# david-andrew/TerminalRayTracer

Measured on AMD Instinct MI355X. Metric: path rays/s (primary+secondary) at 1920x1080, 64 spheres, 8 bounces, higher is better.
Workload: dtype f64

## Files before the change

terminalraytracer_amd/csrc/trt_device.hpp:

```cpp
#pragma once

#include <hip/hip_runtime.h>
#include <stdint.h>

namespace trt
{

struct d3
{
    double x, y, z;
};

#define TRT_DEV __device__ __forceinline__

TRT_DEV d3 make3(double x, double y, double z) { return d3{x, y, z}; }
TRT_DEV d3 load3(const double *p) { return d3{p[0], p[1], p[2]}; }
TRT_DEV double dot(d3 a, d3 b) { return a.x * b.x + a.y * b.y + a.z * b.z; }
TRT_DEV d3 sub(d3 a, d3 b) { return d3{a.x - b.x, a.y - b.y, a.z - b.z}; }
TRT_DEV d3 add(d3 a, d3 b) { return d3{a.x + b.x, a.y + b.y, a.z + b.z}; }
TRT_DEV d3 mulc(d3 a, d3 b) { return d3{a.x * b.x, a.y * b.y, a.z * b.z}; }
TRT_DEV d3 scale(d3 a, double s) { return d3{a.x * s, a.y * s, a.z * s}; }


#define TRT_LIKELY(c) __builtin_expect(!!(c), 1)

TRT_DEV unsigned long long lanes_with(bool p) { return __builtin_amdgcn_ballot_w64(p); }

TRT_DEV unsigned hi32(double x) { return (unsigned)(__builtin_bit_cast(unsigned long long, x) >> 32); }

TRT_DEV bool mid_range(double x) { return hi32(x) - (723u << 20) < (600u << 20); }

TRT_DEV double sqrt_exact(double x)
{
    const double y = __builtin_amdgcn_rsq(x);
    double g = x * y, h = y * 0.5;
    const double r = __builtin_fma(-h, g, 0.5);
    g = __builtin_fma(g, r, g);
    h = __builtin_fma(h, r, h);
    double d = __builtin_fma(-g, g, x);
    g = __builtin_fma(d, h, g);
    d = __builtin_fma(-g, g, x);
    double root = __builtin_fma(d, h, g);
    const bool outside = !mid_range(x);
    if (__builtin_expect(__any(outside), 0))
    {
        const double full = __builtin_sqrt(x);
        root = outside ? full : root;
    }
    return root;
}

TRT_DEV d3 unit(d3 a)
{
    const double len = sqrt_exact(a.x * a.x + a.y * a.y + a.z * a.z);
    const bool longer = len > 0.0001;
    const int ex = __builtin_amdgcn_frexp_exp(a.x), ey = __builtin_amdgcn_frexp_exp(a.y), ez = __builtin_amdgcn_frexp_exp(a.z);
    int lo = ex < ey ? ex : ey;
    lo = lo < ez ? lo : ez;
    const bool ok = len < 0x1p300 && lo > -300;
    if (TRT_LIKELY(!__any(!ok)))
    {
        const double den = longer ? len : 1.0;
        double r = __builtin_amdgcn_rcp(den);
        double e = __builtin_fma(-den, r, 1.0);
        r = __builtin_fma(r, e, r);
        e = __builtin_fma(-den, r, 1.0);
        r = __builtin_fma(r, e, r);
        double q[3] = {a.x, a.y, a.z};
#pragma unroll
        for (int k = 0; k < 3; k++)
        {
            const double num = q[k];
            const double q0 = num * r;
            const double err = __builtin_fma(-den, q0, num);
            const double quo = __builtin_fma(err, r, q0);
            q[k] = __builtin_copysign(quo, num);
        }
        return d3{q[0], q[1], q[2]};
    }
    if (longer)
    {
        a.x /= len;
        a.y /= len;
        a.z /= len;
    }
    return a;
}

TRT_DEV d3 unit_reference(d3 a)
{
    const double len = __builtin_sqrt(a.x * a.x + a.y * a.y + a.z * a.z);
    if (len > 0.0001)
    {
        a.x /= len;
        a.y /= len;
        a.z /= len;
    }
    return a;
}

TRT_DEV double clampd(double v, double lo, double hi) { return v < lo ? lo : (v > hi ? hi : v); }

TRT_DEV d3 reflect(d3 v, d3 n)
{
    double d = dot(v, n);
    return d3{v.x - 2.0 * d * n.x, v.y - 2.0 * d * n.y, v.z - 2.0 * d * n.z};
}

TRT_DEV int d2i(double x)
{
    return __builtin_fabs(x) < 2147483648.0 ? (int)x : (int)0x80000000;
}

TRT_DEV double min1(double x) { return __builtin_fmin(x, 1.0); }

constexpr int kSphereDoubles = 9;
constexpr int kDirLightDoubles = 6;
constexpr int kPointLightDoubles = 7;

struct SceneView
{
    const double *spheres;
    const double *dir_lights;
    const double *point_lights;
    const uint32_t *sky;
    int num_spheres;
    int num_dir;
    int num_point;
    int sky_dim;
    double ground[16];
    double sky_dim_f;
};

struct FrameView
{
    double cam[15];
    const double *jitter;
    const double *col_x;
    const double *row_y;
    double inv_spp;
    unsigned width_magic;
    unsigned spp_magic;
    unsigned tile_magic;
    double *samples;
    double *out;
    const double *ior;
    unsigned long long *counters;
    unsigned int *queue;
    unsigned ring_at;
    unsigned queue_shift;
    unsigned chunk;
    int width, height;
    int tile_rows, tile_first, tile_step;
    int local_rows;
    int bounce_limit, spp;
    const double *image;
};

TRT_DEV int frame_row_of_magic(const FrameView &f, unsigned local_row)
{
    unsigned t = __umulhi(local_row, f.tile_magic);
    int within = (int)(local_row - t * (unsigned)f.tile_rows);
    const int under = within < 0, over = within >= f.tile_rows;
    t += (unsigned)(over - under);
    within += (under - over) * f.tile_rows;
    return (f.tile_first + (int)t * f.tile_step) * f.tile_rows + within;
}

TRT_DEV int frame_row_of(const FrameView &f, int local_row)
{
    int t = local_row / f.tile_rows;
    return (f.tile_first + t * f.tile_step) * f.tile_rows + (local_row - t * f.tile_rows);
}

TRT_DEV bool hit_sphere(d3 o, d3 d, double a, d3 c, double r, d3 &p)
{
    d3 oc = sub(o, c);
    double b = 2.0 * dot(oc, d);
    double cc = dot(oc, oc) - r * r;
    double disc = b * b - 4.0 * a * cc;
    if (disc < 0.0)
        return false;
    double t0 = (-b - __builtin_sqrt(disc)) / (2.0 * a);
    if (!(t0 > 0.0))
        return false;
    p = d3{o.x + t0 * d.x, o.y + t0 * d.y, o.z + t0 * d.z};
    return true;
}

TRT_DEV bool hit_plane(d3 o, d3 d, d3 gp, d3 gn, d3 &p)
{
    double denom = dot(d, gn);
    if (!(__builtin_fabs(denom) > 0.00001))
        return false;
    const double num = dot(sub(gp, o), gn);
    if ((long long)(__builtin_bit_cast(unsigned long long, num) ^ __builtin_bit_cast(unsigned long long, denom)) < 0)
        return false;
    double t = num / denom;
    if (!(t > 0.00001))
        return false;
    p = d3{o.x + t * d.x, o.y + t * d.y, o.z + t * d.z};
    return true;
}

TRT_DEV double dist2(d3 o, d3 p)
{
    d3 b = sub(o, p);
    return dot(b, b);
}

TRT_DEV d3 nudge(d3 o, d3 p) { return add(p, scale(unit(sub(o, p)), 0.000001)); }

TRT_DEV int checker_odd(d3 p) { return d2i(__builtin_floor(p.x) + __builtin_floor(p.z)) & 1; }

TRT_DEV d3 cube_axis(int f)
{
    double s = (f & 1) ? -1.0 : 1.0;
    int a = f >> 1;
    return d3{a == 0 ? s : 0.0, a == 1 ? s : 0.0, a == 2 ? s : 0.0};
}

TRT_DEV uint32_t sky_texel(const uint32_t *sky, int dim, d3 direction)
{
    d3 dir = unit(direction);
    int face = -1;
    double best = -1.0;
#pragma unroll
    for (int f = 0; f < 6; f++)
    {
        double t = dot(dir, cube_axis(f));
        if (t > best)
        {
            best = t;
            face = f;
        }
    }
    if (face < 0)
        face = 0;
    d3 ax = cube_axis(face);
    d3 touching = mulc(dir, ax);
    double scale_by = touching.x + touching.y + touching.z;
    dir = scale(dir, 1.0 / scale_by);
    double along = dot(dir, ax);
    d3 in_plane = scale(sub(dir, scale(ax, along)), 0.5);
    double u = dot(in_plane, cube_axis((face + 2) % 6));
    double v = dot(in_plane, cube_axis((face + 4) % 6));
    if (face & 1)
        u *= -1.0;
    if (face < 2)
    {
        double t = u;
        u = v;
        v = -t;
    }
    else if (face < 4)
    {
        double t = u;
        u = -v;
        v = t;
    }
    else if (face == 4)
    {
        u *= -1.0;
        v *= -1.0;
    }
    u = clampd(u, -0.5, 0.5);
    v = clampd(v, -0.5, 0.5);
    int ui = d2i((u + 0.5) * dim);
    int vi = d2i((v + 0.5) * dim);
    long idx = (long)ui + (long)vi * dim;
    long last = (long)dim * dim - 1;
    if (idx > last)
        idx = last;
    if (idx < 0)
        idx = 0;
    return sky[(long)face * dim * dim + idx];
}

TRT_DEV long sky_index_unit(int dim, d3 dir, double dim_f)
{
    int face = 0;
    double best = -1.0;
    const double t[6] = {dir.x, -dir.x, dir.y, -dir.y, dir.z, -dir.z};
#pragma unroll
    for (int f = 0; f < 6; f++)
        if (t[f] > best)
        {
            best = t[f];
            face = f;
        }
    const double inv = 1.0 / best;
    const d3 ds = scale(dir, inv);
    const int axis = face >> 1;
    const double sgn = (face & 1) ? -0.5 : 0.5;
    const double cu = axis == 0 ? ds.y : (axis == 1 ? ds.z : ds.x);
    const double cv = axis == 0 ? ds.z : (axis == 1 ? ds.x : ds.y);
    double u = sgn * cu, v = sgn * cv;
    if (face & 1)
        u = -u;
    if (face < 2)
    {
        const double w = u;
        u = v;
        v = -w;
    }
    else if (face < 4)
    {
        const double w = u;
        u = -v;
        v = w;
    }
    else if (face == 4)
    {
        u = -u;
        v = -v;
    }
    u = clampd(u, -0.5, 0.5);
    v = clampd(v, -0.5, 0.5);
    const int ui = d2i((u + 0.5) * dim_f);
    const int vi = d2i((v + 0.5) * dim_f);
    long idx = (long)ui + (long)vi * dim;
    const long last = (long)dim * dim - 1;
    idx = idx > last ? last : (idx < 0 ? 0 : idx);
    return (long)face * dim * dim + idx;
}

TRT_DEV uint32_t sky_texel_unit(const uint32_t *sky, int dim, d3 dir, double dim_f) { return sky[sky_index_unit(dim, dir, dim_f)]; }

TRT_DEV uint32_t sky_texel_unit(const uint32_t *sky, int dim, d3 dir)
{
    return sky_texel_unit(sky, dim, dir, (double)dim);
}

TRT_DEV long sky_index_estimate(int dim, float dim_f, d3 dir, bool &ambiguous, unsigned long long &sure_lanes)
{
    const float x = (float)dir.x, y = (float)dir.y, z = (float)dir.z;
    const int face = (int)__builtin_amdgcn_cubeid(x, y, z);
    const float sc = __builtin_amdgcn_cubesc(x, y, z), tc = __builtin_amdgcn_cubetc(x, y, z), ma = __builtin_amdgcn_cubema(x, y, z);
    const float inv = __builtin_amdgcn_rcpf(__builtin_fabsf(ma));
    const unsigned flip = face == 3 ? 0x80000000u : 0u;
    const float un = __builtin_bit_cast(float, __builtin_bit_cast(unsigned, sc) ^ flip ^ 0x80000000u) * inv;
    const float vn = __builtin_bit_cast(float, __builtin_bit_cast(unsigned, tc) ^ flip) * inv;
    const float half = 0.5f * dim_f, e = 0x1p-20f * dim_f;
    const float U = __builtin_fmaf(un, dim_f, half), V = __builtin_fmaf(vn, dim_f, half);
    const float fu = __builtin_amdgcn_fractf(U), fv = __builtin_amdgcn_fractf(V);
    const float lo = __builtin_fminf(__builtin_fminf(U, V), __builtin_fminf(fu, fv)), hi = __builtin_fmaxf(U - dim_f + 1.0f, __builtin_fmaxf(V - dim_f + 1.0f, __builtin_fmaxf(fu, fv)));
    const bool above = lo > e, below = hi < 1.0f - e, ranged = __builtin_fabsf(ma) > 0x1p-100f;
    ambiguous = !(above && below) || !ranged;
    sure_lanes = lanes_with(above) & lanes_with(below) & lanes_with(ranged);
    return ((long)face * dim + (long)(int)V) * dim + (long)(int)U;
}

TRT_DEV long sky_index_estimate(int dim, float dim_f, d3 dir, bool &ambiguous)
{
    unsigned long long sure_lanes;
    return sky_index_estimate(dim, dim_f, dir, ambiguous, sure_lanes);
}

TRT_DEV long sky_index_unit(int dim, d3 dir, double dim_f);
TRT_DEV uint32_t sky_texel_wave(const uint32_t *sky, int dim, d3 dir, double dim_f, bool active, unsigned long long active_lanes)
{
    bool ambiguous;
    unsigned long long sure_lanes;
    long idx = sky_index_estimate(dim, (float)dim_f, dir, ambiguous, sure_lanes);
    if ((active_lanes & ~sure_lanes) != 0)
    {
        const long exact = sky_index_unit(dim, dir, dim_f);
        idx = ambiguous ? exact : idx;
    }
    return active ? sky[idx] : 0u;
}

TRT_DEV d3 texel_color(uint32_t t)
{
    return d3{(double)(t & 0xFF) / 255.0, (double)((t >> 8) & 0xFF) / 255.0, (double)((t >> 16) & 0xFF) / 255.0};
}

TRT_DEV d3 primary_direction(const FrameView &f, int row, int column, int k)
{
    const double sw = f.cam[13], sh = f.cam[14], sd = f.cam[12];
    double sx = (((double)column / (double)f.width) * sw - sw / 2.0);
    double sy = -(((double)row / (double)f.height) * sh - sh / 2.0);
    double sz = -sd;
    sx += f.jitter[k];
    sy += f.jitter[f.spp + k];
    d3 bx = load3(f.cam + 0), by = load3(f.cam + 3), bz = load3(f.cam + 6), eye = load3(f.cam + 9);
    d3 dir = d3{0.0, 0.0, 0.0};
    dir = add(dir, scale(bx, sx));
    dir = add(dir, scale(by, sy));
    dir = add(dir, scale(bz, sz));
    dir = sub(dir, eye);
    return unit(dir);
}

}
```

terminalraytracer_amd/csrc/trt_diag.hip:

```cpp
#define TRT_UNIT_DIAG 1
#include "trt_context.hpp"
#include "trt_simple.hpp"

using namespace trt_impl;

namespace trt_impl
{
void allow_large_lds_diag(const trt_context *ctx)
{
    (void)hipFuncSetAttribute((const void *)trt::probe_rays_kernel, hipFuncAttributeMaxDynamicSharedMemorySize, ctx->lds_limit);
    (void)hipFuncSetAttribute((const void *)trt::probe_rounds_kernel<false>, hipFuncAttributeMaxDynamicSharedMemorySize, ctx->lds_limit);
    (void)hipFuncSetAttribute((const void *)trt::probe_rounds_kernel<true>, hipFuncAttributeMaxDynamicSharedMemorySize, ctx->lds_limit);
}
}

extern "C" int trt_set_list_pool_words(trt_context *ctx, size_t words)
{
    if (!ctx)
        return fail(TRT_ERR_ARGUMENT, "ctx is NULL");
    const int rc = refuse_if_shared(ctx, "trt_set_list_pool_words");
    if (rc)
        return rc;
    ctx->list_pool_cap = words;
    ctx->T->grids_built_for[0] = -1;
    return TRT_OK;
}

extern "C" int trt_read_diagnostics(trt_context *ctx, unsigned long long *wave_loop_trips, unsigned long long *phase2_rounds)
{
    if (!ctx)
        return fail(TRT_ERR_ARGUMENT, "ctx is NULL");
    if (wave_loop_trips)
        *wave_loop_trips = ctx->last_trips;
    if (phase2_rounds)
        *phase2_rounds = ctx->last_phase2;
    return TRT_OK;
}

extern "C" int trt_read_sweep_fallbacks(trt_context *ctx, unsigned long long *swept_traces)
{
    if (!ctx || !swept_traces)
        return fail(TRT_ERR_ARGUMENT, "NULL argument");
    *swept_traces = ctx->last_swept;
    return TRT_OK;
}

extern "C" int trt_read_loop_diagnostics(trt_context *ctx, unsigned long long out[8])
{
    if (!ctx || !out)
        return fail(TRT_ERR_ARGUMENT, "NULL argument");
    memcpy(out, ctx->last_loops, sizeof ctx->last_loops);
    return TRT_OK;
}

extern "C" int trt_read_shading_passes(trt_context *ctx, unsigned long long *passes)
{
    if (!ctx || !passes)
        return fail(TRT_ERR_ARGUMENT, "NULL argument");
    *passes = ctx->last_passes;
    return TRT_OK;
}

extern "C" int trt_path_family_code(trt_context *ctx, int kind, int sphere, const double *parent_origin)
{
    if (!ctx || !ctx->have_scene || !ctx->grids.path_enabled || kind < 0 || kind > 3)
        return -1;
    if (kind < 2)
        return kind;
    const int n = (int)(ctx->T->h_spheres.size() / 9);
    if (sphere < 0 || sphere >= n)
        return -1;
    if (kind == 2)
        return 2 + sphere;
    if (!parent_origin)
        return -1;
    if (!ctx->grids.patch_m)
        return 2 + n + sphere;
    const double *c = ctx->T->h_spheres.data() + 9 * (size_t)sphere;
    const int k = trt_patch_of(ctx->grids.patch_m, parent_origin[0] - c[0], parent_origin[1] - c[1], parent_origin[2] - c[2]);
    return 2 + n + ((sphere << TRT_PATCH_SHIFT) | k);
}

extern "C" long trt_read_path_tables(trt_context *ctx, const Camera *camera, unsigned long long *cells, size_t capacity_cells,
                                     unsigned long long *pool, size_t capacity_pool, long info[8])
{
    if (!ctx || !camera || !cells || !pool || !info)
        return fail(TRT_ERR_ARGUMENT, "NULL argument");
    if (!ctx->have_scene)
        return fail(TRT_ERR_NO_SCENE, "no scene");
    HIP_TRY(hipSetDevice(ctx->device));
    const int rc = ensure_eye_tables(ctx, camera, ctx->stream);
    if (rc)
        return rc;
    HIP_TRY(hipStreamSynchronize(ctx->stream));
    const trt::GridView &g = ctx->grids;
    const int n = (int)(ctx->T->h_spheres.size() / 9);
    unsigned long long used[16 * (1 + kEyeSlots)] = {0};
    HIP_TRY(hipMemcpy(used, ctx->T->d_pool_used.ptr, sizeof used, hipMemcpyDeviceToHost));
    const size_t eye_total = 2 * 6 * (size_t)g.g_eye * g.g_eye, sph_total = 2 * (size_t)n * (size_t)g.patch_count * 6 * (size_t)g.g_sph * g.g_sph;
    const size_t total = g.path_enabled ? eye_total + sph_total : 0;
    const size_t pool_words = ctx->T->pool_scene_words + kEyeSlots * ctx->T->pool_eye_words;
    const size_t eye_from = ctx->T->pool_scene_words + (size_t)ctx->eye_slot * ctx->T->pool_eye_words;
    info[0] = g.path_enabled, info[1] = g.g_eye, info[2] = g.g_sph, info[3] = n, info[4] = (long)total;
    info[5] = (long)std::min<unsigned long long>(used[0], 1ull << 62), info[6] = (long)used[16 * (1 + ctx->eye_slot)] - (long)eye_from, info[7] = (long)pool_words;
    if (!g.path_enabled)
        return 0;
    if (capacity_cells < total || capacity_pool < pool_words)
        return fail(TRT_ERR_CAPACITY, "tables have %zu cells and %zu pool words", total, pool_words);
    HIP_TRY(hipMemcpy(cells, ctx->T->d_path_lists.ptr + g.eye_at, eye_total * sizeof(unsigned long long), hipMemcpyDeviceToHost));
    if (sph_total)
        HIP_TRY(hipMemcpy(cells + eye_total, ctx->T->d_path_lists.ptr + g.sph_at, sph_total * sizeof(unsigned long long), hipMemcpyDeviceToHost));
    HIP_TRY(hipMemcpy(pool, ctx->T->d_pool.ptr, pool_words * sizeof(unsigned long long), hipMemcpyDeviceToHost));
    return (long)total;
}

extern "C" long trt_read_light_grid(trt_context *ctx, int point_light, int index, unsigned long long *masks, size_t capacity_words)
{
    if (!ctx || !masks || index < 0)
        return fail(TRT_ERR_ARGUMENT, "bad argument");
    if (!ctx->have_scene)
        return fail(TRT_ERR_NO_SCENE, "no scene");
    const trt::GridView &g = ctx->grids;
    if (!g.enabled)
        return 0;
    if (index >= (point_light ? ctx->scene.num_point : ctx->scene.num_dir))
        return fail(TRT_ERR_ARGUMENT, "light %d", index);
    const size_t words = (size_t)std::max((ctx->scene.num_spheres + 63) / 64, 1);
    const size_t stride = (point_light ? g.point_stride : g.dir_stride) * words;
    if (capacity_words < stride)
        return fail(TRT_ERR_CAPACITY, "table has %zu words, buffer %zu", stride, capacity_words);
    HIP_TRY(hipSetDevice(ctx->device));
    HIP_TRY(hipStreamSynchronize(ctx->stream));
    HIP_TRY(hipMemcpy(masks, (point_light ? ctx->T->d_point_masks.ptr : ctx->T->d_dir_masks.ptr) + stride * (size_t)index, stride * sizeof(unsigned long long),
                      hipMemcpyDeviceToHost));
    return (long)stride;
}

extern "C" long trt_read_light_lists(trt_context *ctx, int point_light, int index, unsigned long long *cells, size_t capacity_cells,
                                     unsigned long long *pool, size_t capacity_pool, long info[4])
{
    const bool query = !cells && !pool && !capacity_cells && !capacity_pool;
    if (!ctx || !info || index < 0 || (!query && (!cells || !pool)))
        return fail(TRT_ERR_ARGUMENT, "bad argument");
    if (!ctx->have_scene)
        return fail(TRT_ERR_NO_SCENE, "no scene");
    const trt::GridView &g = ctx->grids;
    const size_t stride = point_light ? g.point_stride : g.dir_stride;
    const size_t pool_words = ctx->T->pool_scene_words;
    info[0] = g.enabled ? (long)stride : 0, info[1] = g.list_bits, info[2] = g.enabled ? (long)pool_words : 0, info[3] = g.enabled;
    if (!g.enabled)
        return 0;
    if (index >= (point_light ? ctx->scene.num_point : ctx->scene.num_dir))
        return fail(TRT_ERR_ARGUMENT, "light %d", index);
    if (query)
        return (long)stride;
    if (capacity_cells < stride || capacity_pool < pool_words)
        return fail(TRT_ERR_CAPACITY, "table has %zu cells and %zu pool words", stride, pool_words);
    HIP_TRY(hipSetDevice(ctx->device));
    HIP_TRY(hipStreamSynchronize(ctx->stream));
    HIP_TRY(hipMemcpy(cells, (point_light ? ctx->T->d_point_lists.ptr : ctx->T->d_dir_lists.ptr) + stride * (size_t)index, stride * sizeof(unsigned long long),
                      hipMemcpyDeviceToHost));
    HIP_TRY(hipMemcpy(pool, ctx->T->d_pool.ptr, pool_words * sizeof(unsigned long long), hipMemcpyDeviceToHost));
    return (long)stride;
}

extern "C" int trt_selftest_div_sqrt(trt_context *ctx, const double *a, const double *b, size_t n, double *quot, double *root)
{
    if (!ctx || !a || !b || !quot || !root)
        return fail(TRT_ERR_ARGUMENT, "NULL argument");
    if (n == 0)
        return TRT_OK;
    HIP_TRY(hipSetDevice(ctx->device));
    DeviceBuffer<double> buf;
    HIP_TRY(buf.reserve(4 * n));
    double *da = buf.ptr, *db = buf.ptr + n, *dq = buf.ptr + 2 * n, *dr = buf.ptr + 3 * n;
    HIP_TRY(hipMemcpy(da, a, n * sizeof(double), hipMemcpyHostToDevice));
    HIP_TRY(hipMemcpy(db, b, n * sizeof(double), hipMemcpyHostToDevice));
    hipLaunchKernelGGL(trt::div_sqrt_kernel, dim3((unsigned)((n + 255) / 256)), dim3(256), 0, ctx->stream, da, db, (long)n, dq, dr);
    HIP_TRY(hipGetLastError());
    HIP_TRY(hipStreamSynchronize(ctx->stream));
    HIP_TRY(hipMemcpy(quot, dq, n * sizeof(double), hipMemcpyDeviceToHost));
    HIP_TRY(hipMemcpy(root, dr, n * sizeof(double), hipMemcpyDeviceToHost));
    return TRT_OK;
}

extern "C" int trt_selftest_unit(trt_context *ctx, const double *xyzw, size_t n, double *fast, double *reference)
{
    if (!ctx || !xyzw || !fast || !reference)
        return fail(TRT_ERR_ARGUMENT, "NULL argument");
    if (n == 0)
        return TRT_OK;
    HIP_TRY(hipSetDevice(ctx->device));
    DeviceBuffer<double> buf;
    HIP_TRY(buf.reserve(12 * n));
    double *dv = buf.ptr, *df = buf.ptr + 4 * n, *dr = buf.ptr + 8 * n;
    HIP_TRY(hipMemcpy(dv, xyzw, 4 * n * sizeof(double), hipMemcpyHostToDevice));
    hipLaunchKernelGGL(trt::unit_selftest_kernel, dim3((unsigned)((n + 255) / 256)), dim3(256), 0, ctx->stream, dv, (long)n, df, dr);
    HIP_TRY(hipGetLastError());
    HIP_TRY(hipStreamSynchronize(ctx->stream));
    HIP_TRY(hipMemcpy(fast, df, 4 * n * sizeof(double), hipMemcpyDeviceToHost));
    HIP_TRY(hipMemcpy(reference, dr, 4 * n * sizeof(double), hipMemcpyDeviceToHost));
    return TRT_OK;
}

namespace
{
__global__ void cube_selftest_kernel(const float *xyz, long n, float *out)
{
    const long i = (long)blockIdx.x * blockDim.x + threadIdx.x;
    if (i >= n)
        return;
    int face;
    float sc, tc, ma2;
    trt_cube_lookup(xyz[3 * i], xyz[3 * i + 1], xyz[3 * i + 2], &face, &sc, &tc, &ma2);
    out[4 * i] = (float)face, out[4 * i + 1] = sc, out[4 * i + 2] = tc, out[4 * i + 3] = ma2;
}
}

namespace
{
__global__ void sky_selftest_kernel(const double *dirs, long n, int dim, long *exact, long *estimate, int *ambiguous)
{
    const long i = (long)blockIdx.x * blockDim.x + threadIdx.x;
    if (i >= n)
        return;
    const trt::d3 d = trt::d3{dirs[3 * i], dirs[3 * i + 1], dirs[3 * i + 2]};
    bool amb;
    exact[i] = trt::sky_index_unit(dim, d, (double)dim);
    estimate[i] = trt::sky_index_estimate(dim, (float)dim, d, amb);
    ambiguous[i] = amb;
}
}

extern "C" int trt_selftest_sky(trt_context *ctx, const double *dirs, size_t n, int dim, long long *exact, long long *estimate, int *ambiguous)
{
    if (!ctx || !dirs || !exact || !estimate || !ambiguous || dim < 1)
        return fail(TRT_ERR_ARGUMENT, "bad argument");
    if (n == 0)
        return TRT_OK;
    HIP_TRY(hipSetDevice(ctx->device));
    DeviceBuffer<double> in;
    DeviceBuffer<long> out;
    DeviceBuffer<int> flags;
    HIP_TRY(in.reserve(3 * n));
    HIP_TRY(out.reserve(2 * n));
    HIP_TRY(flags.reserve(n));
    HIP_TRY(hipMemcpy(in.ptr, dirs, 3 * n * sizeof(double), hipMemcpyHostToDevice));
    hipLaunchKernelGGL(sky_selftest_kernel, dim3((unsigned)((n + 255) / 256)), dim3(256), 0, ctx->stream, (const double *)in.ptr, (long)n, dim, out.ptr, out.ptr + n, flags.ptr);
    HIP_TRY(hipGetLastError());
    HIP_TRY(hipStreamSynchronize(ctx->stream));
    HIP_TRY(hipMemcpy(exact, out.ptr, n * sizeof(long), hipMemcpyDeviceToHost));
    HIP_TRY(hipMemcpy(estimate, out.ptr + n, n * sizeof(long), hipMemcpyDeviceToHost));
    HIP_TRY(hipMemcpy(ambiguous, flags.ptr, n * sizeof(int), hipMemcpyDeviceToHost));
    return TRT_OK;
}

extern "C" int trt_selftest_cube(trt_context *ctx, const float *xyz, size_t n, float *device_out, float *host_out)
{
    if (!ctx || !xyz || !device_out || !host_out)
        return fail(TRT_ERR_ARGUMENT, "NULL argument");
    if (n == 0)
        return TRT_OK;
    HIP_TRY(hipSetDevice(ctx->device));
    DeviceBuffer<float> buf;
    HIP_TRY(buf.reserve(7 * n));
    HIP_TRY(hipMemcpy(buf.ptr, xyz, 3 * n * sizeof(float), hipMemcpyHostToDevice));
    hipLaunchKernelGGL(cube_selftest_kernel, dim3((unsigned)((n + 255) / 256)), dim3(256), 0, ctx->stream, (const float *)buf.ptr, (long)n, buf.ptr + 3 * n);
    HIP_TRY(hipGetLastError());
    HIP_TRY(hipStreamSynchronize(ctx->stream));
    HIP_TRY(hipMemcpy(device_out, buf.ptr + 3 * n, 4 * n * sizeof(float), hipMemcpyDeviceToHost));
    for (size_t i = 0; i < n; i++)
    {
        int face;
        float sc, tc, ma2;
        trt_cube_lookup(xyz[3 * i], xyz[3 * i + 1], xyz[3 * i + 2], &face, &sc, &tc, &ma2);
        host_out[4 * i] = (float)face, host_out[4 * i + 1] = sc, host_out[4 * i + 2] = tc, host_out[4 * i + 3] = ma2;
    }
    return TRT_OK;
}

extern "C" int trt_probe_rays(trt_context *ctx, const Ray *rays, size_t n, int *obj, double *point, double *normal,
                              double *material, double *lit)
{
    if (!ctx || !rays || !obj || !point || !normal || !material || !lit)
        return fail(TRT_ERR_ARGUMENT, "NULL argument");
    if (!ctx->have_scene)
        return fail(TRT_ERR_NO_SCENE, "trt_set_scene has not been called");
    if (n == 0)
        return TRT_OK;
    HIP_TRY(hipSetDevice(ctx->device));
    DeviceBuffer<double> buf;
    DeviceBuffer<int> dobj;
    HIP_TRY(buf.reserve(n * (6 + 3 + 3 + 5 + 3)));
    HIP_TRY(dobj.reserve(n));
    double *dr = buf.ptr, *dp = dr + 6 * n, *dn = dp + 3 * n, *dm = dn + 3 * n, *dl = dm + 5 * n;
    HIP_TRY(hipMemcpy(dr, rays, n * sizeof(Ray), hipMemcpyHostToDevice));
    hipLaunchKernelGGL(trt::probe_rays_kernel, dim3((unsigned)((n + 255) / 256)), dim3(256), scene_lds_bytes(ctx->scene), ctx->stream,
                       ctx->scene, dr, (long)n, dobj.ptr, dp, dn, dm, dl);
    HIP_TRY(hipGetLastError());
    HIP_TRY(hipStreamSynchronize(ctx->stream));
    HIP_TRY(hipMemcpy(obj, dobj.ptr, n * sizeof(int), hipMemcpyDeviceToHost));
    HIP_TRY(hipMemcpy(point, dp, 3 * n * sizeof(double), hipMemcpyDeviceToHost));
    HIP_TRY(hipMemcpy(normal, dn, 3 * n * sizeof(double), hipMemcpyDeviceToHost));
    HIP_TRY(hipMemcpy(material, dm, 5 * n * sizeof(double), hipMemcpyDeviceToHost));
    HIP_TRY(hipMemcpy(lit, dl, 3 * n * sizeof(double), hipMemcpyDeviceToHost));
    return TRT_OK;
}

extern "C" int trt_probe_rays_production(trt_context *ctx, const Camera *camera, const Ray *rays, const int *families, size_t n, int *obj,
                                         double *point, double *normal, double *material, double *lit)
{
    if (!ctx || !camera || !rays || !obj || !point || !normal || !material || !lit)
        return fail(TRT_ERR_ARGUMENT, "NULL argument");
    if (!ctx->have_scene)
        return fail(TRT_ERR_NO_SCENE, "trt_set_scene has not been called");
    if (n == 0)
        return TRT_OK;
    HIP_TRY(hipSetDevice(ctx->device));
    const int rc = ensure_eye_tables(ctx, camera, ctx->stream);
    if (rc)
        return rc;
    DeviceBuffer<double> buf;
    DeviceBuffer<int> dobj;
    HIP_TRY(buf.reserve(n * (6 + 3 + 3 + 5 + 3)));
    HIP_TRY(dobj.reserve(2 * n));
    double *dr = buf.ptr, *dp = dr + 6 * n, *dn = dp + 3 * n, *dm = dn + 3 * n, *dl = dm + 5 * n;
    HIP_TRY(hipMemcpy(dr, rays, n * sizeof(Ray), hipMemcpyHostToDevice));
    if (families)
    {
        const int ns = ctx->scene.num_spheres, pm = ctx->grids.path_enabled ? ctx->grids.patch_m : 0, pc = ctx->grids.path_enabled ? ctx->grids.patch_count : 0;
        std::vector<int> codes(families, families + n);
        for (int &c : codes)
        {
            bool ok = c == 0 || c == 1 || (c >= 2 && c < 2 + ns);
            if (!ok && c >= 2 + ns)
            {
                const int rest = c - 2 - ns;
                ok = pm ? ((rest >> TRT_PATCH_SHIFT) < ns && (rest & ((1 << TRT_PATCH_SHIFT) - 1)) < pc) : rest < ns;
            }
            if (!ok)
                c = -1;
        }
        HIP_TRY(hipMemcpy(dobj.ptr + n, codes.data(), n * sizeof(int), hipMemcpyHostToDevice));
    }
    trt::FrameView f{};
    memcpy(f.cam, camera, sizeof(Camera));
    f.jitter = ctx->d_jitter.ptr;
    if (ctx->grids.path_enabled && ctx->grids.patch_m > 0)
        hipLaunchKernelGGL(trt::probe_rounds_kernel<true>, dim3((unsigned)((n + trt::kPersistentBlock - 1) / trt::kPersistentBlock)), dim3(trt::kPersistentBlock),
                           image_lds_bytes(ctx, 0), ctx->stream, ctx->scene, ctx->cull, f, ctx->grids, (const double *)dr,
                           families ? (const int *)(dobj.ptr + n) : (const int *)nullptr, (long)n, dobj.ptr, dp, dn, dm, dl);
    else
        hipLaunchKernelGGL(trt::probe_rounds_kernel<false>, dim3((unsigned)((n + trt::kPersistentBlock - 1) / trt::kPersistentBlock)), dim3(trt::kPersistentBlock),
                           image_lds_bytes(ctx, 0), ctx->stream, ctx->scene, ctx->cull, f, ctx->grids, (const double *)dr,
                           families ? (const int *)(dobj.ptr + n) : (const int *)nullptr, (long)n, dobj.ptr, dp, dn, dm, dl);
    HIP_TRY(hipGetLastError());
    HIP_TRY(hipStreamSynchronize(ctx->stream));
    HIP_TRY(hipMemcpy(obj, dobj.ptr, n * sizeof(int), hipMemcpyDeviceToHost));
    HIP_TRY(hipMemcpy(point, dp, 3 * n * sizeof(double), hipMemcpyDeviceToHost));
    HIP_TRY(hipMemcpy(normal, dn, 3 * n * sizeof(double), hipMemcpyDeviceToHost));
    HIP_TRY(hipMemcpy(material, dm, 5 * n * sizeof(double), hipMemcpyDeviceToHost));
    HIP_TRY(hipMemcpy(lit, dl, 3 * n * sizeof(double), hipMemcpyDeviceToHost));
    return TRT_OK;
}
```

terminalraytracer_amd/csrc/trt_render.hip:

```cpp
#define TRT_UNIT_RENDER 1
#include "trt_context.hpp"
#ifndef TRT_REDUCE_BLOCK
#define TRT_REDUCE_BLOCK 64
#endif
#include "trt_simple.hpp"
#include "trt_ansi.hpp"
#include "trt_ansi_delta.hpp"
#include "trt_ansi_half.hpp"

using namespace trt_impl;

namespace trt_impl
{

enum Variant : int
{
    kPlain, kPlainCount,
    kPatches, kPatchesCount,
    kPatchesBig,
    kDecoupled, kDecoupledCount,
    kRefract, kRefractCount, kRefractPatches, kRefractPatchesCount,
    kPlainImage, kPlainImageCount, kPatchesImage, kPatchesImageCount,
    kReference,
    kReferenceImage,
};

using RoundsKernel = void (*)(trt::SceneView, trt::CullView, trt::FrameView, trt::GridView);
using BatchKernel = void (*)(trt::SceneView, trt::CullView, trt::FrameView, trt::GridView, trt::BatchView);
struct RoundsVariant
{
    RoundsKernel fn;
    int block;
    bool rings;
    bool image;
    BatchKernel batch;
};
static const RoundsVariant kRounds[kReference] = {
    {trt::render_rounds_kernel<false>, trt::kPersistentBlock, false, false, trt::render_rounds_kernel<false, false, false, false, false, false, true, trt::BatchView>},
    {trt::render_rounds_kernel<true>, trt::kPersistentBlock, false},
    {trt::render_rounds_kernel<false, false, false, true>, trt::kPersistentBlock, false, false, trt::render_rounds_kernel<false, false, false, true, false, false, true, trt::BatchView>},
    {trt::render_rounds_kernel<true, false, false, true>, trt::kPersistentBlock, false},
    {trt::render_rounds_kernel<false, false, false, true, true>, trt::kBigBlock, false},
    {trt::render_rounds_kernel<false, false, true>, trt::kCompactBlock, true, false, trt::render_rounds_kernel<false, false, true, false, false, false, true, trt::BatchView>},
    {trt::render_rounds_kernel<true, false, true>, trt::kCompactBlock, true},
    {trt::render_rounds_kernel<false, true>, trt::kPersistentBlock, false},
    {trt::render_rounds_kernel<true, true>, trt::kPersistentBlock, false},
    {trt::render_rounds_kernel<false, true, false, true>, trt::kPersistentBlock, false},
    {trt::render_rounds_kernel<true, true, false, true>, trt::kPersistentBlock, false},
    {trt::render_rounds_kernel<false, false, false, false, false, true>, trt::kPersistentBlock, false, true},
    {trt::render_rounds_kernel<true, false, false, false, false, true>, trt::kPersistentBlock, false, true},
    {trt::render_rounds_kernel<false, false, false, true, false, true>, trt::kPersistentBlock, false, true},
    {trt::render_rounds_kernel<true, false, false, true, false, true>, trt::kPersistentBlock, false, true},
};
static_assert(TRT_BATCH_MAX == kEyeSlots && TRT_BATCH_MAX == trt::kBatchMax, "a frame of a batch has an eye slot of the scene's tables and a place in BatchView");

static BatchKernel batch_form(Variant v)
{
    return v < kReference ? kRounds[v].batch : nullptr;
}

static bool image_in_device_memory(Variant v)
{
    return v == kReferenceImage || (v < kReference && kRounds[v].image);
}

static bool wants_device_image(const trt_context *ctx, int spp)
{
    if (ctx->scene_image >= 0)
        return ctx->scene_image == 1;
    return (ctx->kernel == 1 ? scene_lds_bytes(ctx->scene) : image_lds_bytes(ctx, spp)) > (size_t)ctx->lds_limit;
}

constexpr int kCompactionMinLights = 2;

constexpr long kCompactionMinUnits = 16L << 20;

static bool renders_decoupled(const trt_context *ctx, long units)
{
    if (!ctx->have_scene || ctx->compact_blocks_per_cu <= 0 || ctx->compaction == 0)
        return false;
    const bool pays = ctx->scene.num_dir + ctx->scene.num_point >= kCompactionMinLights && units >= kCompactionMinUnits && ctx->grids.path_enabled &&
                      ctx->compact_blocks_per_cu * trt::kCompactBlock >= ctx->rounds_blocks_per_cu * trt::kPersistentBlock;
    return ctx->compaction > 0 || pays;
}

static bool has_patches(const trt_context *ctx)
{
    return ctx->grids.path_enabled && ctx->grids.patch_m > 0;
}

static Variant choose_variant(const trt_context *ctx, long units, int spp, int frames = 1)
{
    const bool device_image = wants_device_image(ctx, spp);
    if (ctx->kernel == 1)
        return device_image ? kReferenceImage : kReference;
    const bool count = ctx->counters_enabled;
    const bool patches = has_patches(ctx);
    if (ctx->ior_count)
        return patches ? (count ? kRefractPatchesCount : kRefractPatches) : (count ? kRefractCount : kRefract);
    if (device_image)
        return patches ? (count ? kPatchesImageCount : kPatchesImage) : (count ? kPlainImageCount : kPlainImage);
    if (!patches && renders_decoupled(ctx, units) && compact_lds_bytes(ctx, spp, frames) <= (size_t)ctx->lds_limit)
        return count ? kDecoupledCount : kDecoupled;
    if (!patches)
        return count ? kPlainCount : kPlain;
    const bool big = ctx->big_blocks_per_cu * trt::kBigBlock > ctx->rounds_blocks_per_cu * trt::kPersistentBlock;
    return count ? kPatchesCount : big ? kPatchesBig : kPatches;
}

static Variant described_variant(const trt_context *ctx)
{
    return ctx->last_variant >= 0 ? (Variant)ctx->last_variant : choose_variant(ctx, kCompactionMinUnits, 64);
}

static int described_spp(const trt_context *ctx)
{
    return ctx->last_variant >= 0 ? ctx->last_spp : 64;
}

static size_t launch_lds_bytes(const trt_context *ctx, Variant v, int spp, int frames = 1)
{
    const RoundsVariant &k = kRounds[v];
    return k.image ? 0u : k.rings ? compact_lds_bytes(ctx, spp, frames) : image_lds_bytes(ctx, spp, frames);
}

static int blocks_per_cu(trt_context *ctx, Variant v, bool batch, size_t lds, int *blocks)
{
    const RoundsVariant &k = kRounds[v];
    if (!batch)
    {
        *blocks = k.image ? ctx->device_blocks_per_cu : k.rings ? ctx->compact_blocks_per_cu : k.block == trt::kBigBlock ? ctx->big_blocks_per_cu : ctx->rounds_blocks_per_cu;
        return TRT_OK;
    }
    for (const trt_context::BatchOccupancy &o : ctx->batch_occupancy)
        if (o.kernel == (const void *)k.batch && o.lds == lds)
        {
            *blocks = o.blocks;
            return TRT_OK;
        }
    *blocks = 0;
    if (lds <= (size_t)ctx->lds_limit)
        HIP_TRY(hipOccupancyMaxActiveBlocksPerMultiprocessor(blocks, k.batch, k.block, lds));
    if (ctx->batch_occupancy.size() >= 64)
        ctx->batch_occupancy.clear();
    ctx->batch_occupancy.push_back({(const void *)k.batch, lds, *blocks});
    return TRT_OK;
}

struct RenderPlan
{
    Variant variant;
    bool batch;
    unsigned grid, block;
    size_t lds;
    unsigned ring_at;
    unsigned queue_shift, chunk;
    int per_cu;
};

static int plan_render(trt_context *ctx, long units, int spp, int frames, bool batch, RenderPlan *plan)
{
    const Variant v = choose_variant(ctx, units, spp, frames);
    if (v == kReference || v == kReferenceImage)
    {
        *plan = RenderPlan{v, false, (unsigned)((units / spp + 255) / 256), 256u, v == kReference ? scene_lds_bytes(ctx->scene) : 0u};
        return TRT_OK;
    }
    const RoundsVariant &k = kRounds[v];
    RenderPlan p{v, batch, 0u, (unsigned)k.block, launch_lds_bytes(ctx, v, spp, frames), k.rings ? (unsigned)compact_ring_at(ctx, spp, frames) : 0u};
    const int rc = blocks_per_cu(ctx, v, batch, p.lds, &p.per_cu);
    if (rc)
        return rc;
    const long cap = (long)(ctx->compute_units - (ctx->stream == ctx->own_stream ? ctx->reserved_cus : 0)) * std::max(p.per_cu, 1);
    const long want = (units + k.block - 1) / k.block;
    p.grid = (unsigned)std::max(1L, std::min(want, cap));
    const bool per_xcd = !has_patches(ctx) && p.grid >= (1u << trt::kQueueXcdShift);
    p.queue_shift = per_xcd ? (unsigned)trt::kQueueXcdShift : 0u;
    p.chunk = per_xcd ? trt::kQueueChunkSmall : trt::kQueueChunkSamples;
    *plan = p;
    return TRT_OK;
}

static hipError_t occupancy(const trt_context *ctx, Variant v, int *blocks)
{
    return hipOccupancyMaxActiveBlocksPerMultiprocessor(blocks, kRounds[v].fn, kRounds[v].block, launch_lds_bytes(ctx, v, 64));
}

int refresh_occupancy(trt_context *ctx)
{
    const trt::SceneView &v = ctx->scene;
    const size_t lds_need = std::max(scene_lds_bytes(v), image_lds_bytes(ctx, 64));
    if (lds_need > (size_t)ctx->lds_limit && ctx->scene_image == 0)
        return fail(TRT_ERR_CAPACITY, "scene needs %zu B of LDS staging, device offers %d", lds_need, ctx->lds_limit);
    if (ctx->device_blocks_per_cu == 0)
    {
        int blocks = 0;
        HIP_TRY(hipOccupancyMaxActiveBlocksPerMultiprocessor(&blocks, kRounds[kPlainImage].fn, kRounds[kPlainImage].block, 0));
        ctx->device_blocks_per_cu = std::max(blocks, 1);
    }
    if (ctx->occupancy_for_lds != image_lds_bytes(ctx, 64))
    {
        const bool fits = image_lds_bytes(ctx, 64) <= (size_t)ctx->lds_limit;
        int blocks = 0;
        if (fits)
            HIP_TRY(occupancy(ctx, kPlain, &blocks));
        ctx->rounds_blocks_per_cu = std::max(blocks, 1);
        ctx->occupancy_for_lds = image_lds_bytes(ctx, 64);
        ctx->compact_blocks_per_cu = 0;
        if (compact_lds_bytes(ctx, 64) <= (size_t)ctx->lds_limit)
            HIP_TRY(occupancy(ctx, kDecoupled, &ctx->compact_blocks_per_cu));
        ctx->big_blocks_per_cu = 0;
        if (fits && ctx->rounds_blocks_per_cu < 4)
            HIP_TRY(occupancy(ctx, kPatchesBig, &ctx->big_blocks_per_cu));
    }
    return TRT_OK;
}

int prepare_jitter(trt_context *ctx, const Camera *cam, int width, int height, int spp)
{
    const double pw = cam->screen_width / width, ph = cam->screen_height / height;
    if (ctx->jit_spp == spp && ctx->jit_pw == pw && ctx->jit_ph == ph)
        return TRT_OK;
    std::vector<double> j(2 * (size_t)spp);
    for (int k = 0; k < spp; k++)
    {
        j[k] = triangle_wave(2 * kPi * k / spp) / 2 * pw;
        j[spp + k] = triangle_wave(kPi * k / spp) / 2 * ph;
    }
    HIP_TRY(ctx->d_jitter.reserve(j.size()));
    HIP_TRY(hipStreamSynchronize(ctx->stream));
    HIP_TRY(hipMemcpy(ctx->d_jitter.ptr, j.data(), j.size() * sizeof(double), hipMemcpyHostToDevice));
    ctx->jit_spp = spp;
    ctx->jit_pw = pw;
    ctx->jit_ph = ph;
    return TRT_OK;
}

int prepare_axes(trt_context *ctx, const Camera *cam, int width, int height)
{
    const double sw = cam->screen_width, sh = cam->screen_height;
    if (ctx->axes_w == width && ctx->axes_h == height && ctx->axes_sw == sw && ctx->axes_sh == sh)
        return TRT_OK;
    std::vector<double> t((size_t)width + height);
    for (int column = 0; column < width; column++)
        t[column] = (((double)column / (double)width) * sw - sw / 2.0);
    for (int row = 0; row < height; row++)
        t[(size_t)width + row] = -(((double)row / (double)height) * sh - sh / 2.0);
    HIP_TRY(ctx->d_axes.reserve(t.size()));
    HIP_TRY(hipStreamSynchronize(ctx->stream));
    HIP_TRY(hipMemcpy(ctx->d_axes.ptr, t.data(), t.size() * sizeof(double), hipMemcpyHostToDevice));
    ctx->axes_w = width;
    ctx->axes_h = height;
    ctx->axes_sw = sw;
    ctx->axes_sh = sh;
    return TRT_OK;
}

void allow_large_lds_render(const trt_context *ctx)
{
    (void)hipFuncSetAttribute((const void *)trt::render_simple_kernel<false>, hipFuncAttributeMaxDynamicSharedMemorySize, ctx->lds_limit);
    for (const RoundsVariant &k : kRounds)
    {
        if (!k.image)
            (void)hipFuncSetAttribute((const void *)k.fn, hipFuncAttributeMaxDynamicSharedMemorySize, ctx->lds_limit);
        if (k.batch)
            (void)hipFuncSetAttribute((const void *)k.batch, hipFuncAttributeMaxDynamicSharedMemorySize, ctx->lds_limit);
    }
}

constexpr int kImageBlock = 1024;
__global__ __launch_bounds__(kImageBlock) void stage_image_kernel(trt::SceneView s, trt::CullView cull, trt::FrameView f, trt::GridView grids)
{
    trt::fill_image(trt::image_layout(const_cast<double *>(f.image), s.num_spheres, s.num_dir, s.num_point, cull.padded, f.spp), s, cull, f, grids);
}

}

extern "C" int trt_enable_counters(trt_context *ctx, int enable)
{
    if (!ctx)
        return fail(TRT_ERR_ARGUMENT, "ctx is NULL");
    ctx->counters_enabled = enable != 0;
    return TRT_OK;
}

extern "C" int trt_set_scratch_fill(trt_context *ctx, int on)
{
    if (!ctx)
        return fail(TRT_ERR_ARGUMENT, "ctx is NULL");
    ctx->scratch_fill = on != 0;
    return TRT_OK;
}

extern "C" int trt_read_counters(trt_context *ctx, unsigned long long *path_rays, unsigned long long *shadow_rays)
{
    if (!ctx)
        return fail(TRT_ERR_ARGUMENT, "ctx is NULL");
    HIP_TRY(hipSetDevice(ctx->device));
    HIP_TRY(hipStreamSynchronize(ctx->stream));
    unsigned long long c[kCounterSlots];
    HIP_TRY(hipMemcpy(c, ctx->d_counters.ptr, sizeof c, hipMemcpyDeviceToHost));
    ctx->last_trips = c[2];
    ctx->last_phase2 = c[3];
    ctx->last_swept = c[28];
    ctx->last_passes = c[29];
    for (int k = 0; k < 7; k++)
        ctx->last_loops[k] = c[30 + k];
#if defined(TRT_MARKS) && TRT_MARKS == 2
    if (getenv("TRT_PRINT_PROFILE"))
        for (int k = 0; k < trt::kProfileKinds; k++)
            for (int s = 0; s < 64; s++)
                if (c[trt::kProfileAt + 64 * k + s])
                    fprintf(stderr, "profile %d %d %llu\n", k, s, c[trt::kProfileAt + 64 * k + s]);
#endif
    if (path_rays)
        *path_rays = c[0];
    if (shadow_rays)
        *shadow_rays = c[1];
    return TRT_OK;
}


enum Output : int { kDoubles, kBytes, kText, kHalfText };

static bool is_text(Output kind) { return kind == kText || kind == kHalfText; }

static size_t frame_bytes(Output kind, int width, int rows)
{
    if (kind == kText)
        return (size_t)trt_ansi_text_bytes(width, rows);
    if (kind == kHalfText)
        return (size_t)trt_ansi_half_text_bytes(width, rows);
    return (size_t)rows * width * 3 * (kind == kBytes ? 1u : sizeof(double));
}

static int check_render_arguments(const trt_context *ctx, const Camera *cameras, int frames, const trt_rowset *rows, int bounce_limit, int rays_per_pixel,
                                  const void *d_pixels, size_t capacity_bytes, Output kind = kDoubles)
{
    if (!ctx || !cameras || !d_pixels)
        return fail(TRT_ERR_ARGUMENT, "NULL argument");
    if (frames < 1 || frames > TRT_BATCH_MAX)
        return fail(TRT_ERR_ARGUMENT, "a batch has 1 to %d cameras, %d given", TRT_BATCH_MAX, frames);
    if (!rowset_valid(rows))
        return fail(TRT_ERR_ARGUMENT, "invalid rowset");
    if (bounce_limit < 1 || rays_per_pixel < 1)
        return fail(TRT_ERR_ARGUMENT, "bounce_limit %d / rays_per_pixel %d", bounce_limit, rays_per_pixel);
    for (int b = 1; b < frames; b++)
        if (cameras[b].screen_width != cameras[0].screen_width || cameras[b].screen_height != cameras[0].screen_height ||
            cameras[b].screen_distance != cameras[0].screen_distance)
            return fail(TRT_ERR_ARGUMENT, "camera %d of the batch has another screen_width / screen_height / screen_distance than camera 0", b);
    if (!ctx->have_scene)
        return fail(TRT_ERR_NO_SCENE, "trt_set_scene has not been called");
    const int local_rows = trt_rowset_rows(rows);
    const size_t need = frame_bytes(kind, rows->width, local_rows) * frames;
    if (capacity_bytes < need)
        return fail(TRT_ERR_CAPACITY, "framebuffer of %d frame(s) needs %zu B, %zu given", frames, need, capacity_bytes);
    if ((unsigned long long)local_rows * rows->width >= 0x7fffffffull)
        return fail(TRT_ERR_ARGUMENT, "%d x %d pixels exceed the 2^31 pixel index range", local_rows, rows->width);
    const unsigned long long units = (unsigned long long)local_rows * rows->width * rays_per_pixel * frames;
    if (ctx->kernel == 0 && units >= 0x7fffffffull)
        return fail(TRT_ERR_ARGUMENT, "%llu work units in %d frame(s) exceed the 2^31 index range", units, frames);
    return TRT_OK;
}

static unsigned division_magic(unsigned long long d)
{
    return (unsigned)std::min<unsigned long long>((0x100000000ull + d - 1) / d, 0xffffffffull);
}

static trt::FrameView frame_view(const trt_context *ctx, const Camera *camera, const trt_rowset *rows, int bounce_limit, int rays_per_pixel, void *d_pixels,
                                 int lane_set)
{
    trt::FrameView f{};
    memcpy(f.cam, camera, sizeof(Camera));
    f.jitter = ctx->d_jitter.ptr;
    f.col_x = ctx->d_axes.ptr;
    f.row_y = ctx->d_axes.ptr + rows->width;
    f.inv_spp = 1.0 / rays_per_pixel;
    f.width_magic = division_magic((unsigned)rows->width);
    f.spp_magic = division_magic((unsigned)rays_per_pixel);
    f.tile_magic = division_magic((unsigned)rows->tile_rows);
    f.out = (double *)d_pixels;
    f.counters = ctx->counters_enabled ? ctx->d_counters.ptr : nullptr;
#if defined(TRT_MARKS) && TRT_MARKS == 2
    f.counters = ctx->d_counters.ptr;
#endif
    f.queue = ctx->d_queue.ptr + trt::kQueueLaneWords * lane_set;
    f.width = rows->width;
    f.height = rows->height;
    f.tile_rows = rows->tile_rows;
    f.tile_first = rows->tile_first;
    f.tile_step = rows->tile_step;
    f.local_rows = trt_rowset_rows(rows);
    f.bounce_limit = bounce_limit;
    f.spp = rays_per_pixel;
    return f;
}

static void launch_ansi_from_rgb8(hipStream_t stream, const unsigned char *d_rgb8, int width, int rows, void *d_text)
{
    const unsigned long long bytes = trt_ansi_text_bytes(width, rows), waves = trt_ansi_waves(trt_ansi_split_of((unsigned long long)d_text, bytes).words);
    hipLaunchKernelGGL(trt::ansi_from_rgb8_kernel, dim3((unsigned)((waves * 64 + TRT_REDUCE_BLOCK - 1) / TRT_REDUCE_BLOCK)), dim3(TRT_REDUCE_BLOCK), 0, stream, d_rgb8,
                       (unsigned char *)d_text, width, rows, trt_ansi_row_magic(width));
}

static void launch_ansi_half_from_rgb8(hipStream_t stream, const unsigned char *d_rgb8, int width, int rows, void *d_text)
{
    const unsigned long long bytes = trt_ansi_half_text_bytes(width, rows),
                             waves = trt_ansi_half_waves(trt_ansi_half_split_of((unsigned long long)d_text, bytes).words);
    hipLaunchKernelGGL(trt::ansi_half_from_rgb8_kernel, dim3((unsigned)((waves * 64 + TRT_REDUCE_BLOCK - 1) / TRT_REDUCE_BLOCK)), dim3(TRT_REDUCE_BLOCK), 0, stream, d_rgb8,
                       (unsigned char *)d_text, width, rows, trt_ansi_half_row_magic(width), trt_ansi_half_width_magic(width));
}

enum : int { kEntryOpens = 1, kEntryCloses = 2, kEntryWhole = kEntryOpens | kEntryCloses };

static int launch_reference(trt_context *ctx, const RenderPlan &plan, trt::FrameView f, void *out, Output kind, long pixels, hipStream_t stream, int entry)
{
    const int slot = (int)(ctx->launches % kEventRing);
    if (kind != kDoubles)
    {
        if (ctx->d_fb.capacity < (size_t)pixels * 3 || (is_text(kind) && ctx->d_text_rgb8.capacity < (size_t)pixels * 3))
            HIP_TRY(hipStreamSynchronize(stream));
        HIP_TRY(ctx->d_fb.reserve((size_t)pixels * 3));
        if (is_text(kind))
            HIP_TRY(ctx->d_text_rgb8.reserve((size_t)pixels * 3));
        f.out = ctx->d_fb.ptr;
    }
    if (ctx->scratch_fill)
    {
        HIP_TRY(hipMemsetAsync(f.out, 0xFF, (size_t)pixels * 3 * sizeof(double), stream));
        if (kind != kDoubles)
            HIP_TRY(hipMemsetAsync(out, 0xFF, frame_bytes(kind, f.width, f.local_rows), stream));
    }
    if (entry & kEntryOpens)
        HIP_TRY(hipEventRecord(ctx->ev_start[slot], stream));
    if (plan.variant == kReference)
        hipLaunchKernelGGL(trt::render_simple_kernel<false>, dim3(plan.grid), dim3(plan.block), plan.lds, stream, ctx->scene, f);
    else
        hipLaunchKernelGGL(trt::render_simple_kernel<true>, dim3(plan.grid), dim3(plan.block), 0, stream, ctx->scene, f);
    if (entry & kEntryCloses)
        HIP_TRY(hipEventRecord(ctx->ev_mid[slot], stream));
    if (kind != kDoubles)
        hipLaunchKernelGGL(trt::quantize_kernel, dim3((unsigned)((pixels * 3 + 255) / 256)), dim3(256), 0, stream, (const double *)f.out, pixels * 3,
                           is_text(kind) ? ctx->d_text_rgb8.ptr : (unsigned char *)out);
    if (kind == kText)
        launch_ansi_from_rgb8(stream, ctx->d_text_rgb8.ptr, f.width, f.local_rows, out);
    if (kind == kHalfText)
        launch_ansi_half_from_rgb8(stream, ctx->d_text_rgb8.ptr, f.width, f.local_rows, out);
    if (entry & kEntryCloses)
        HIP_TRY(hipEventRecord(ctx->ev_stop[slot], stream));
    HIP_TRY(hipGetLastError());
    return TRT_OK;
}

static void launch_ordered_mean(hipStream_t stream, const RenderPlan &plan, const trt::FrameView &f, const double *samples, void *out, Output kind, long pixels,
                                unsigned frames)
{
    const long values = pixels * 3;
    const dim3 block(TRT_REDUCE_BLOCK);
    const auto blocks = [&](unsigned long long lanes) { return dim3((unsigned)((lanes + TRT_REDUCE_BLOCK - 1) / TRT_REDUCE_BLOCK), frames); };
    switch (kind)
    {
    case kDoubles:
        hipLaunchKernelGGL(trt::reduce_samples_kernel, blocks((unsigned long long)trt_mean_lanes(values)), block, 0, stream, samples, (double *)out, values, f.spp, f.inv_spp, f.queue, plan.grid,
                           plan.block / 64, f.queue_shift);
        break;
    case kBytes:
        hipLaunchKernelGGL(trt::reduce_samples_rgb8_kernel,
                           blocks(frames > 1 ? values / trt::kRgb8Group + 6 : trt::rgb8_lanes(values, trt::rgb8_head((const unsigned char *)out, values))), block, 0,
                           stream, samples, (unsigned char *)out, values, f.spp, f.inv_spp, f.queue, plan.grid, plan.block / 64, f.queue_shift);
        break;
    case kText:
    {
        const unsigned long long bytes = trt_ansi_text_bytes(f.width, f.local_rows);
        const unsigned long long waves = trt_ansi_waves(frames > 1 ? bytes / 4 : trt_ansi_split_of((unsigned long long)out, bytes).words);
        hipLaunchKernelGGL(trt::reduce_samples_ansi_kernel, blocks(waves * 64), block, 0, stream, samples, (unsigned char *)out, f.width, f.local_rows,
                           trt_ansi_row_magic(f.width), f.spp, f.inv_spp, f.queue, plan.grid, plan.block / 64, f.queue_shift);
        break;
    }
    case kHalfText:
    {
        const unsigned long long bytes = trt_ansi_half_text_bytes(f.width, f.local_rows);
        const unsigned long long waves = trt_ansi_half_waves(frames > 1 ? bytes / 4 : trt_ansi_half_split_of((unsigned long long)out, bytes).words);
        hipLaunchKernelGGL(trt::reduce_samples_ansi_half_kernel, blocks(waves * 64), block, 0, stream, samples, (unsigned char *)out, f.width, f.local_rows,
                           trt_ansi_half_row_magic(f.width), trt_ansi_half_width_magic(f.width), f.spp, f.inv_spp, f.queue, plan.grid, plan.block / 64,
                           f.queue_shift);
        break;
    }
    }
}

static int launch_production(trt_context *ctx, const RenderPlan &plan, trt::FrameView f, const trt::GridView &grids, const trt::BatchView *batch, void *out,
                             Output kind, long pixels, int lane_set, int entry)
{
    const hipStream_t stream = lane_set ? ctx->alt_stream : ctx->stream;
    const int slot = (int)(ctx->launches % kEventRing);
    const dim3 grid(plan.grid), block(plan.block);
    unsigned *const ready = ctx->queue_ready[lane_set];
    const RoundsVariant &k = kRounds[plan.variant];
    const unsigned frames = batch ? batch->frames : 1u;
    DeviceBuffer<double> &scratch = lane_set ? ctx->d_samples_alt : ctx->d_samples;
    const size_t samples = (size_t)pixels * f.spp * frames * 3;
    if (scratch.capacity < samples)
        HIP_TRY(hipStreamSynchronize(stream));
    HIP_TRY(scratch.reserve(samples));
    f.samples = scratch.ptr;
    if (k.image)
    {
        DeviceBuffer<double> &image = lane_set ? ctx->d_image_alt : ctx->d_image;
        const size_t doubles = image_lds_bytes(ctx, f.spp) / sizeof(double);
        if (image.capacity < doubles)
            HIP_TRY(hipStreamSynchronize(stream));
        HIP_TRY(image.reserve(doubles));
        f.image = image.ptr;
    }
    if (ctx->ior_count && ctx->ior_count != ctx->scene.num_spheres)
        return fail(TRT_ERR_ARGUMENT, "trt_set_refraction was given %d indices, the scene has %d spheres", ctx->ior_count, ctx->scene.num_spheres);
    if (ctx->ior_count)
        f.ior = ctx->d_ior.ptr;
    f.ring_at = plan.ring_at;
    f.queue_shift = plan.queue_shift;
    f.chunk = plan.chunk;
    if (ctx->scratch_fill)
    {
        HIP_TRY(hipMemsetAsync(scratch.ptr, 0xFF, samples * sizeof(double), stream));
        HIP_TRY(hipMemsetAsync(out, 0xFF, frame_bytes(kind, f.width, f.local_rows) * frames, stream));
    }
    const bool left_ready = ready[0] == plan.grid && ready[1] == plan.block / 64 && ready[2] == f.queue_shift;
    ready[0] = 0;
    if (!left_ready)
        hipLaunchKernelGGL(trt::start_queue_kernel, dim3(1), dim3(64), 0, stream, f.queue, plan.grid, plan.block / 64, f.queue_shift);
    if (entry & kEntryOpens)
        HIP_TRY(hipEventRecord(ctx->ev_start[slot], stream));
    if (k.image)
        hipLaunchKernelGGL(stage_image_kernel, dim3(1), dim3(kImageBlock), 0, stream, ctx->scene, ctx->cull, f, grids);
    if (batch)
        hipLaunchKernelGGL(k.batch, grid, block, plan.lds, stream, ctx->scene, ctx->cull, f, grids, *batch);
    else
        hipLaunchKernelGGL(k.fn, grid, block, plan.lds, stream, ctx->scene, ctx->cull, f, grids);
    if (entry & kEntryCloses)
        HIP_TRY(hipEventRecord(ctx->ev_mid[slot], stream));
#if !TRT_AB_SKIP_REDUCE
    launch_ordered_mean(stream, plan, f, scratch.ptr, out, kind, pixels, frames);
#endif
    if (entry & kEntryCloses)
        HIP_TRY(hipEventRecord(ctx->ev_stop[slot], stream));
    HIP_TRY(hipGetLastError());
#if !TRT_AB_SKIP_REDUCE
    ready[0] = plan.grid, ready[1] = plan.block / 64, ready[2] = f.queue_shift;
#endif
    return TRT_OK;
}

static int launch_render(trt_context *ctx, const RenderPlan &plan, const trt::FrameView &f, const trt::GridView &grids, const trt::BatchView *batch, void *out,
                         Output kind, long pixels, int lane_set, int entry)
{
    const hipStream_t stream = lane_set ? ctx->alt_stream : ctx->stream;
    const bool reference = plan.variant == kReference || plan.variant == kReferenceImage;
    if (plan.lds > (size_t)ctx->lds_limit)
        return fail(TRT_ERR_CAPACITY, "%s and %d rays per pixel need %zu B of LDS staging, device offers %d%s", plan.variant == kReference ? "scene" : "scene image",
                    f.spp, plan.lds, ctx->lds_limit, ctx->ior_count && plan.variant != kReference ? " (the refraction extension stages it in LDS only)" : "");
#if defined(TRT_MARKS) && TRT_MARKS == 2
    HIP_TRY(hipMemsetAsync(ctx->d_counters.ptr, 0, kCounterSlots * sizeof(unsigned long long), stream));
#endif
    const int rc = reference ? launch_reference(ctx, plan, f, out, kind, pixels, stream, entry)
                             : launch_production(ctx, plan, f, grids, batch, out, kind, pixels, lane_set, entry);
    if (rc)
        return rc;
    ctx->last_variant = plan.variant;
    ctx->last_spp = f.spp;
    if (entry & kEntryCloses)
        ctx->launches++;
    return TRT_OK;
}

static int render_device_on(trt_context *ctx, const Camera *camera, const trt_rowset *rows, int bounce_limit, int rays_per_pixel, void *d_pixels,
                            size_t capacity_bytes, int lane_set, int entry = kEntryWhole, Output kind = kDoubles)
{
    int rc = check_render_arguments(ctx, camera, 1, rows, bounce_limit, rays_per_pixel, d_pixels, capacity_bytes, kind);
    if (rc)
        return rc;
    const long pixels = (long)trt_rowset_rows(rows) * rows->width;
    if (pixels == 0)
        return TRT_OK;
    HIP_TRY(hipSetDevice(ctx->device));
    const hipStream_t stream = lane_set ? ctx->alt_stream : ctx->stream;
    rc = prepare_jitter(ctx, camera, rows->width, rows->height, rays_per_pixel);
    if (rc)
        return rc;
    rc = prepare_axes(ctx, camera, rows->width, rows->height);
    if (rc)
        return rc;
    rc = ensure_eye_tables(ctx, camera, stream);
    if (rc)
        return rc;
    if (ctx->counters_enabled && (entry & kEntryOpens))
        HIP_TRY(hipMemsetAsync(ctx->d_counters.ptr, 0, kCounterSlots * sizeof(unsigned long long), stream));
    RenderPlan plan;
    rc = plan_render(ctx, pixels * rays_per_pixel, rays_per_pixel, 1, false, &plan);
    if (rc)
        return rc;
    return launch_render(ctx, plan, frame_view(ctx, camera, rows, bounce_limit, rays_per_pixel, kind == kDoubles ? d_pixels : nullptr, lane_set), ctx->grids, nullptr,
                         d_pixels, kind, pixels, lane_set, entry);
}

extern "C" int trt_render_device(trt_context *ctx, const Camera *camera, const trt_rowset *rows, int bounce_limit,
                                 int rays_per_pixel, void *d_pixels, size_t capacity_bytes)
{
    return render_device_on(ctx, camera, rows, bounce_limit, rays_per_pixel, d_pixels, capacity_bytes, 0);
}

extern "C" int trt_render_device_rgb8(trt_context *ctx, const Camera *camera, const trt_rowset *rows, int bounce_limit, int rays_per_pixel, void *d_rgb8,
                                      size_t capacity_bytes)
{
    return render_device_on(ctx, camera, rows, bounce_limit, rays_per_pixel, d_rgb8, capacity_bytes, 0, kEntryWhole, kBytes);
}

extern "C" size_t trt_ansi_bytes(int width, int rows)
{
    return (size_t)trt_ansi_text_bytes(width, rows);
}

extern "C" int trt_render_device_ansi(trt_context *ctx, const Camera *camera, const trt_rowset *rows, int bounce_limit, int rays_per_pixel, void *d_text,
                                      size_t capacity_bytes)
{
    return render_device_on(ctx, camera, rows, bounce_limit, rays_per_pixel, d_text, capacity_bytes, 0, kEntryWhole, kText);
}

extern "C" size_t trt_ansi_half_bytes(int width, int rows)
{
    return (size_t)trt_ansi_half_text_bytes(width, rows);
}

extern "C" int trt_render_device_ansi_half(trt_context *ctx, const Camera *camera, const trt_rowset *rows, int bounce_limit, int rays_per_pixel, void *d_text,
                                           size_t capacity_bytes)
{
    return render_device_on(ctx, camera, rows, bounce_limit, rays_per_pixel, d_text, capacity_bytes, 0, kEntryWhole, kHalfText);
}

extern "C" int trt_ansi_half_from_rgb8_device(trt_context *ctx, const void *d_rgb8, int width, int rows, void *d_text)
{
    if (!ctx || !d_rgb8 || !d_text)
        return fail(TRT_ERR_ARGUMENT, "NULL argument");
    if (width <= 0 || rows <= 0 || (unsigned long long)width * rows >= 0x7fffffffull)
        return fail(TRT_ERR_ARGUMENT, "screen %d x %d", width, rows);
    HIP_TRY(hipSetDevice(ctx->device));
    launch_ansi_half_from_rgb8(ctx->stream, (const unsigned char *)d_rgb8, width, rows, d_text);
    HIP_TRY(hipGetLastError());
    return TRT_OK;
}

extern "C" int trt_ansi_from_rgb8_device(trt_context *ctx, const void *d_rgb8, int width, int rows, void *d_text)
{
    if (!ctx || !d_rgb8 || !d_text)
        return fail(TRT_ERR_ARGUMENT, "NULL argument");
    if (width <= 0 || rows <= 0 || (unsigned long long)width * rows >= 0x7fffffffull)
        return fail(TRT_ERR_ARGUMENT, "screen %d x %d", width, rows);
    HIP_TRY(hipSetDevice(ctx->device));
    launch_ansi_from_rgb8(ctx->stream, (const unsigned char *)d_rgb8, width, rows, d_text);
    HIP_TRY(hipGetLastError());
    return TRT_OK;
}

extern "C" int trt_quantize_device(trt_context *ctx, const void *d_pixels, size_t num_pixels, void *d_rgb8)
{
    if (!ctx || !d_pixels || !d_rgb8)
        return fail(TRT_ERR_ARGUMENT, "NULL argument");
    if (num_pixels == 0)
        return TRT_OK;
    HIP_TRY(hipSetDevice(ctx->device));
    const long n = (long)num_pixels * 3;
    hipLaunchKernelGGL(trt::quantize_kernel, dim3((unsigned)((n + 255) / 256)), dim3(256), 0, ctx->stream, (const double *)d_pixels,
                       n, (unsigned char *)d_rgb8);
    HIP_TRY(hipGetLastError());
    return TRT_OK;
}

extern "C" int trt_synchronize(trt_context *ctx)
{
    if (!ctx)
        return fail(TRT_ERR_ARGUMENT, "ctx is NULL");
    HIP_TRY(hipSetDevice(ctx->device));
    HIP_TRY(hipStreamSynchronize(ctx->stream));
    return TRT_OK;
}

extern "C" int trt_render_host(trt_context *ctx, const Camera *camera, const trt_rowset *rows, int bounce_limit,
                               int rays_per_pixel, Vector *pixels)
{
    if (!ctx || !pixels)
        return fail(TRT_ERR_ARGUMENT, "NULL argument");
    if (!rowset_valid(rows))
        return fail(TRT_ERR_ARGUMENT, "invalid rowset");
    HIP_TRY(hipSetDevice(ctx->device));
    const size_t count = (size_t)trt_rowset_rows(rows) * rows->width;
    const size_t bytes = count * sizeof(Vector);
    HIP_TRY(ctx->d_fb.reserve(count * 3));
    HIP_TRY(ctx->h_staging.reserve(bytes));
    const double t_begin = host_now_ms();
    const int local_rows = trt_rowset_rows(rows);
    const bool whole = rows->tile_first == 0 && rows->tile_step == 1 && rows->tile_rows >= rows->height;
    static const int band_count = getenv("TRT_HOST_BANDS") ? std::min(8, std::max(1, atoi(getenv("TRT_HOST_BANDS")))) : 4;
#if defined(TRT_MARKS) && TRT_MARKS == 2
    const int bands = 1;
#else
    const int bands = whole && !ctx->counters_enabled && local_rows >= 256 && bytes >= (32u << 20) ? band_count : 1;
#endif
    const int band_rows = (local_rows + bands - 1) / bands;
    const size_t row_bytes = (size_t)rows->width * sizeof(Vector);
    const int chunks_per_band = (int)std::min<size_t>(16 / bands, std::max<size_t>(1, (size_t)band_rows * row_bytes / (4u << 20)));
    int chunks = 0;
    size_t chunk_at[16], chunk_len[16];
    if (bands > 1 && !ctx->copy_stream)
    {
        HIP_TRY(ctx->copy_stream.create());
        HIP_TRY(ctx->alt_stream.create());
    }
    const hipStream_t copy_stream = bands > 1 ? ctx->copy_stream : ctx->stream;
    if (ctx->have_scene && camera)
    {
        const int rc = ensure_eye_tables(ctx, camera, ctx->stream);
        if (rc)
            return rc;
    }
    if (bands > 1)
    {
        HIP_TRY(hipEventRecord(ctx->ev_fork, ctx->stream));
        HIP_TRY(hipStreamWaitEvent(ctx->alt_stream, ctx->ev_fork, 0));
    }
    for (int b = 0; b < bands; b++)
    {
        trt_rowset band = *rows;
        if (bands > 1)
            band = trt_rowset{rows->width, rows->height, band_rows, b, bands};
        const int rows_here = trt_rowset_rows(&band);
        const size_t at = (size_t)b * band_rows * row_bytes, len = (size_t)rows_here * row_bytes;
        const int set = bands > 1 ? (b & 1) : 0;
        int rc = render_device_on(ctx, camera, &band, bounce_limit, rays_per_pixel, (char *)ctx->d_fb.ptr + at, len, set);
        if (rc)
            return rc;
        if (bands > 1)
        {
            HIP_TRY(hipEventRecord(ctx->ev_band[b], set ? ctx->alt_stream : ctx->stream));
            HIP_TRY(hipStreamWaitEvent(copy_stream, ctx->ev_band[b], 0));
        }
        const size_t per = ((len + chunks_per_band - 1) / chunks_per_band + 63) / 64 * 64;
        for (int i = 0; i < chunks_per_band; i++, chunks++)
        {
            chunk_at[chunks] = at + (size_t)i * per;
            chunk_len[chunks] = (size_t)i * per < len ? std::min(per, len - (size_t)i * per) : 0;
            if (chunk_len[chunks])
                HIP_TRY(hipMemcpyAsync((char *)ctx->h_staging.ptr + chunk_at[chunks], (const char *)ctx->d_fb.ptr + chunk_at[chunks], chunk_len[chunks],
                                       hipMemcpyDeviceToHost, copy_stream));
            HIP_TRY(hipEventRecord(ctx->ev_chunk[chunks], copy_stream));
        }
    }
    const double t_enqueued = host_now_ms();
    const int workers = chunks >= 4 ? 4 : 1;
    hipError_t worker_error[4] = {hipSuccess, hipSuccess, hipSuccess, hipSuccess};
    auto drain = [&](int w) {
        (void)hipSetDevice(ctx->device);
        for (int i = w; i < chunks; i += workers)
        {
            const hipError_t e = hipEventSynchronize(ctx->ev_chunk[i]);
            if (e != hipSuccess)
            {
                worker_error[w] = e;
                return;
            }
            memcpy((char *)pixels + chunk_at[i], (const char *)ctx->h_staging.ptr + chunk_at[i], chunk_len[i]);
        }
    };
    if (workers == 1)
        drain(0);
    else
    {
        std::thread pool[3];
        for (int w = 1; w < workers; w++)
            pool[w - 1] = std::thread(drain, w);
        drain(0);
        for (int w = 1; w < workers; w++)
            pool[w - 1].join();
    }
    for (int w = 0; w < workers; w++)
        HIP_TRY(worker_error[w]);
    if (bands > 1)
    {
        HIP_TRY(hipStreamSynchronize(ctx->copy_stream));
        HIP_TRY(hipStreamSynchronize(ctx->alt_stream));
    }
    HIP_TRY(hipStreamSynchronize(ctx->stream));
    if (print_host_times())
        fprintf(stderr, "trt_render_host: %d band(s), enqueue %.3f ms, render + copy-out of %zu bytes %.3f ms\n", bands, t_enqueued - t_begin, bytes,
                host_now_ms() - t_enqueued);
    return TRT_OK;
}


static int fit_batch(trt_context *ctx, long units_per_frame, int spp, int remaining, RenderPlan *plan)
{
    for (int t = remaining;; t--)
    {
        int rc = plan_render(ctx, units_per_frame * t, spp, t, true, plan), alone = 0;
        if (!rc)
            rc = blocks_per_cu(ctx, plan->variant, true, launch_lds_bytes(ctx, plan->variant, spp), &alone);
        if (rc)
            return rc;
        if (t == 1 || (plan->per_cu > 0 && plan->per_cu >= alone))
            return t;
    }
}

static int render_device_batch(trt_context *ctx, const Camera *cameras, int n, const trt_rowset *rows, int bounce_limit, int rays_per_pixel, void *d_pixels,
                               size_t capacity_bytes, Output kind)
{
    int rc = check_render_arguments(ctx, cameras, n, rows, bounce_limit, rays_per_pixel, d_pixels, capacity_bytes, kind);
    if (rc)
        return rc;
    const long pixels = (long)trt_rowset_rows(rows) * rows->width, units = pixels * rays_per_pixel;
    const size_t each = frame_bytes(kind, rows->width, trt_rowset_rows(rows));
    const bool shared = ctx->T.use_count() > 1;
    if (n > 1 && shared)
        return fail(TRT_ERR_CAPACITY, "this context's scene tables are shared with %ld other context(s) (trt_share_scene): their eye slots are the sharers', "
                                      "a batch of %d cameras has none to build its tables in (one camera per call works)", ctx->T.use_count() - 1, n);
    ctx->batch_frames = n;
    ctx->batch_launches = 0;
    if (pixels == 0)
        return TRT_OK;
    HIP_TRY(hipSetDevice(ctx->device));
    const hipStream_t stream = ctx->stream;
    if (shared || bounce_limit > trt::kBatchBounceMask || !batch_form(choose_variant(ctx, units * n, rays_per_pixel, n)))
    {
        for (int b = 0; b < n; b++)
        {
            rc = render_device_on(ctx, &cameras[b], rows, bounce_limit, rays_per_pixel, (char *)d_pixels + (size_t)b * each, each, 0, (b == 0 ? kEntryOpens : 0) | (b == n - 1 ? kEntryCloses : 0), kind);
            if (rc)
                return rc;
            ctx->batch_launches++;
        }
        return TRT_OK;
    }
    rc = prepare_jitter(ctx, &cameras[0], rows->width, rows->height, rays_per_pixel);
    if (rc)
        return rc;
    rc = prepare_axes(ctx, &cameras[0], rows->width, rows->height);
    if (rc)
        return rc;
    for (int b = 0; b < n; b++)
    {
        rc = ensure_eye_tables(ctx, &cameras[b], stream, b);
        if (rc)
            return rc;
    }
    RenderPlan plan;
    int m = n;
    for (int first = 0; first < n; first += m)
    {
        m = fit_batch(ctx, units, rays_per_pixel, std::min(m, n - first), &plan);
        if (m < 0)
            return m;
        trt::GridView g = ctx->grids;
        g.eye_at = (unsigned)((size_t)first * 2 * 6 * (size_t)g.g_eye * (size_t)g.g_eye);
        trt::BatchView batch{};
        for (int b = 0; b < m; b++)
        {
            memcpy(batch.cam[b], &cameras[first + b], sizeof(Camera));
            batch.eye[b][0] = ctx->eye_slots[first + b].families[0], batch.eye[b][1] = ctx->eye_slots[first + b].families[1];
        }
        g.eye[0] = batch.eye[0][0], g.eye[1] = batch.eye[0][1];
        batch.frames = (unsigned)m;
        batch.units_per_frame = (unsigned)units;
        batch.frame_magic = division_magic((unsigned long long)units);
        rc = launch_render(ctx, plan, frame_view(ctx, &cameras[first], rows, bounce_limit, rays_per_pixel, kind == kDoubles ? d_pixels : nullptr, 0), g, &batch,
                           (char *)d_pixels + (size_t)first * each, kind, pixels, 0,
                           (first == 0 ? kEntryOpens : 0) | (first + m == n ? kEntryCloses : 0));
        if (rc)
            return rc;
        ctx->batch_launches++;
    }
    return TRT_OK;
}

extern "C" int trt_render_device_batch(trt_context *ctx, const Camera *cameras, int n, const trt_rowset *rows, int bounce_limit, int rays_per_pixel,
                                       void *d_pixels, size_t capacity_bytes)
{
    return render_device_batch(ctx, cameras, n, rows, bounce_limit, rays_per_pixel, d_pixels, capacity_bytes, kDoubles);
}

extern "C" int trt_render_device_batch_rgb8(trt_context *ctx, const Camera *cameras, int n, const trt_rowset *rows, int bounce_limit, int rays_per_pixel,
                                            void *d_rgb8, size_t capacity_bytes)
{
    return render_device_batch(ctx, cameras, n, rows, bounce_limit, rays_per_pixel, d_rgb8, capacity_bytes, kBytes);
}

extern "C" int trt_render_device_batch_ansi(trt_context *ctx, const Camera *cameras, int n, const trt_rowset *rows, int bounce_limit, int rays_per_pixel,
                                            void *d_text, size_t capacity_bytes)
{
    return render_device_batch(ctx, cameras, n, rows, bounce_limit, rays_per_pixel, d_text, capacity_bytes, kText);
}

static int render_host_as(trt_context *ctx, const Camera *cameras, int n, bool batch, const trt_rowset *rows, int bounce_limit, int rays_per_pixel, void *host,
                          Output kind, const char *name = nullptr)
{
    if (!ctx || !host)
        return fail(TRT_ERR_ARGUMENT, "NULL argument");
    if (batch && (n < 1 || n > TRT_BATCH_MAX))
        return fail(TRT_ERR_ARGUMENT, "a batch has 1 to %d cameras, %d given", TRT_BATCH_MAX, n);
    if (!rowset_valid(rows))
        return fail(TRT_ERR_ARGUMENT, "invalid rowset");
    HIP_TRY(hipSetDevice(ctx->device));
    const size_t bytes = (size_t)n * frame_bytes(kind, rows->width, trt_rowset_rows(rows));
    if (!batch && bytes == 0)
        return TRT_OK;
    const size_t room = std::max<size_t>(bytes, 1);
    if (kind == kDoubles)
        HIP_TRY(ctx->d_fb.reserve((room + sizeof(double) - 1) / sizeof(double)));
    else
        HIP_TRY((kind == kBytes ? ctx->d_rgb8 : ctx->d_text).reserve(room));
    void *const d_out = kind == kDoubles ? (void *)ctx->d_fb.ptr : kind == kBytes ? (void *)ctx->d_rgb8.ptr : (void *)ctx->d_text.ptr;
    HIP_TRY(ctx->h_staging.reserve(room));
    const double t_begin = host_now_ms();
    const int rc = batch ? render_device_batch(ctx, cameras, n, rows, bounce_limit, rays_per_pixel, d_out, bytes, kind)
                         : render_device_on(ctx, cameras, rows, bounce_limit, rays_per_pixel, d_out, bytes, 0, kEntryWhole, kind);
    if (rc || bytes == 0)
        return rc;
    HIP_TRY(hipMemcpyAsync(ctx->h_staging.ptr, d_out, bytes, hipMemcpyDeviceToHost, ctx->stream));
    HIP_TRY(hipStreamSynchronize(ctx->stream));
    memcpy(host, ctx->h_staging.ptr, bytes);
    if (name && print_host_times())
        fprintf(stderr, kind == kBytes ? "%s: %.3f ms for %zu pixels\n" : "%s: %.3f ms for %zu bytes of text\n", name, host_now_ms() - t_begin,
                kind == kBytes ? bytes / 3 : bytes);
    return TRT_OK;
}

extern "C" int trt_render_host_rgb8(trt_context *ctx, const Camera *camera, const trt_rowset *rows, int bounce_limit, int rays_per_pixel,
                                    unsigned char *rgb)
{
    return render_host_as(ctx, camera, 1, false, rows, bounce_limit, rays_per_pixel, rgb, kBytes, "trt_render_host_rgb8");
}

extern "C" int trt_render_host_ansi(trt_context *ctx, const Camera *camera, const trt_rowset *rows, int bounce_limit, int rays_per_pixel, char *text)
{
    return render_host_as(ctx, camera, 1, false, rows, bounce_limit, rays_per_pixel, text, kText, "trt_render_host_ansi");
}

extern "C" int trt_render_host_batch(trt_context *ctx, const Camera *cameras, int n, const trt_rowset *rows, int bounce_limit, int rays_per_pixel,
                                     Vector *pixels)
{
    return render_host_as(ctx, cameras, n, true, rows, bounce_limit, rays_per_pixel, pixels, kDoubles);
}

extern "C" int trt_render_host_batch_rgb8(trt_context *ctx, const Camera *cameras, int n, const trt_rowset *rows, int bounce_limit, int rays_per_pixel,
                                          unsigned char *rgb)
{
    return render_host_as(ctx, cameras, n, true, rows, bounce_limit, rays_per_pixel, rgb, kBytes);
}

extern "C" int trt_render_host_batch_ansi(trt_context *ctx, const Camera *cameras, int n, const trt_rowset *rows, int bounce_limit, int rays_per_pixel, char *text)
{
    return render_host_as(ctx, cameras, n, true, rows, bounce_limit, rays_per_pixel, text, kText);
}

extern "C" int trt_render_device_batch_ansi_half(trt_context *ctx, const Camera *cameras, int n, const trt_rowset *rows, int bounce_limit, int rays_per_pixel,
                                                 void *d_text, size_t capacity_bytes)
{
    return render_device_batch(ctx, cameras, n, rows, bounce_limit, rays_per_pixel, d_text, capacity_bytes, kHalfText);
}

extern "C" int trt_render_host_ansi_half(trt_context *ctx, const Camera *camera, const trt_rowset *rows, int bounce_limit, int rays_per_pixel, char *text)
{
    return render_host_as(ctx, camera, 1, false, rows, bounce_limit, rays_per_pixel, text, kHalfText, "trt_render_host_ansi_half");
}

extern "C" int trt_render_host_batch_ansi_half(trt_context *ctx, const Camera *cameras, int n, const trt_rowset *rows, int bounce_limit, int rays_per_pixel,
                                               char *text)
{
    return render_host_as(ctx, cameras, n, true, rows, bounce_limit, rays_per_pixel, text, kHalfText);
}

extern "C" int trt_batch_info(trt_context *ctx, int *frames, int *render_launches)
{
    if (!ctx)
        return fail(TRT_ERR_ARGUMENT, "ctx is NULL");
    if (frames)
        *frames = ctx->batch_frames;
    if (render_launches)
        *render_launches = ctx->batch_launches;
    return TRT_OK;
}

template <class Each>
static int for_last_launches(trt_context *ctx, int max, Each each)
{
    HIP_TRY(hipSetDevice(ctx->device));
    HIP_TRY(hipStreamSynchronize(ctx->stream));
    const long n = std::min<long>(std::min<long>(ctx->launches, kEventRing), max);
    for (long i = 0; i < n; i++)
    {
        const int rc = each(i, (int)((ctx->launches - n + i) % kEventRing));
        if (rc)
            return rc;
    }
    return (int)n;
}

extern "C" int trt_kernel_times(trt_context *ctx, float *ms, int max)
{
    if (!ctx || !ms || max < 0)
        return fail(TRT_ERR_ARGUMENT, "bad argument");
    return for_last_launches(ctx, max, [&](long i, int slot) -> int {
        HIP_TRY(hipEventElapsedTime(&ms[i], ctx->ev_start[slot], ctx->ev_stop[slot]));
        return TRT_OK;
    });
}

extern "C" int trt_render_kernel_times(trt_context *ctx, float *render_ms, float *reduce_ms, int max)
{
    if (!ctx || !render_ms || max < 0)
        return fail(TRT_ERR_ARGUMENT, "bad argument");
    return for_last_launches(ctx, max, [&](long i, int slot) -> int {
        HIP_TRY(hipEventElapsedTime(&render_ms[i], ctx->ev_start[slot], ctx->ev_mid[slot]));
        if (reduce_ms)
            HIP_TRY(hipEventElapsedTime(&reduce_ms[i], ctx->ev_mid[slot], ctx->ev_stop[slot]));
        return TRT_OK;
    });
}

extern "C" long trt_launch_count(trt_context *ctx) { return ctx ? ctx->launches : -1; }

extern "C" int trt_launch_span_ms(trt_context *first, long first_launch, trt_context *last, long last_launch, float *ms)
{
    if (!first || !last || !ms || first->device != last->device)
        return fail(TRT_ERR_ARGUMENT, "bad argument");
    if (first_launch < 0 || first_launch >= first->launches || first->launches - first_launch > kEventRing || last_launch < 0 ||
        last_launch >= last->launches || last->launches - last_launch > kEventRing)
        return fail(TRT_ERR_ARGUMENT, "launches %ld / %ld are not among the last %d of their contexts (%ld / %ld launched)", first_launch, last_launch,
                    kEventRing, first->launches, last->launches);
    HIP_TRY(hipSetDevice(first->device));
    HIP_TRY(hipStreamSynchronize(first->stream));
    HIP_TRY(hipStreamSynchronize(last->stream));
    HIP_TRY(hipEventElapsedTime(ms, first->ev_start[first_launch % kEventRing], last->ev_stop[last_launch % kEventRing]));
    return TRT_OK;
}

extern "C" int trt_render_variant(trt_context *ctx, int *decoupled, int *workgroup_threads)
{
    if (!ctx)
        return fail(TRT_ERR_ARGUMENT, "ctx is NULL");
    const Variant v = described_variant(ctx);
    if (decoupled)
        *decoupled = v < kReference && kRounds[v].rings ? 1 : 0;
    if (workgroup_threads)
        *workgroup_threads = v >= kReference ? 256 : kRounds[v].block;
    return TRT_OK;
}

extern "C" int trt_set_scene_image(trt_context *ctx, int mode)
{
    if (!ctx || mode < -1 || mode > 1)
        return fail(TRT_ERR_ARGUMENT, "scene image mode %d", mode);
    ctx->scene_image = mode;
    return ctx->have_scene && mode != 0 ? refresh_occupancy(ctx) : TRT_OK;
}

extern "C" int trt_render_image(trt_context *ctx, int *in_device_memory, unsigned long long *image_bytes)
{
    if (!ctx)
        return fail(TRT_ERR_ARGUMENT, "ctx is NULL");
    const Variant v = described_variant(ctx);
    if (in_device_memory)
        *in_device_memory = image_in_device_memory(v) ? 1 : 0;
    if (image_bytes)
        *image_bytes = !ctx->have_scene ? 0ull : v >= kReference ? scene_lds_bytes(ctx->scene) : image_lds_bytes(ctx, described_spp(ctx));
    return TRT_OK;
}

extern "C" int trt_kernel_info(trt_context *ctx, int *vgprs, int *sgprs, int *static_lds_bytes, int *max_blocks_per_cu,
                               int *compute_units)
{
    if (!ctx)
        return fail(TRT_ERR_ARGUMENT, "ctx is NULL");
    HIP_TRY(hipSetDevice(ctx->device));
    const Variant v = described_variant(ctx);
    hipFuncAttributes attr;
    HIP_TRY(hipFuncGetAttributes(&attr, v == kReference ? (const void *)trt::render_simple_kernel<false>
                                      : v == kReferenceImage ? (const void *)trt::render_simple_kernel<true> : (const void *)kRounds[v].fn));
    if (vgprs)
        *vgprs = attr.numRegs;
    if (sgprs)
        *sgprs = 0;
    if (static_lds_bytes)
        *static_lds_bytes = (int)attr.sharedSizeBytes;
    if (max_blocks_per_cu)
    {
        int blocks = 0;
        if (v == kReference)
            HIP_TRY(hipOccupancyMaxActiveBlocksPerMultiprocessor(&blocks, trt::render_simple_kernel<false>, 256, ctx->have_scene ? scene_lds_bytes(ctx->scene) : 0));
        else if (v == kReferenceImage)
            HIP_TRY(hipOccupancyMaxActiveBlocksPerMultiprocessor(&blocks, trt::render_simple_kernel<true>, 256, 0));
        else if (!ctx->have_scene)
            HIP_TRY(hipOccupancyMaxActiveBlocksPerMultiprocessor(&blocks, kRounds[kPlain].fn, trt::kPersistentBlock, 0));
        else
            (void)blocks_per_cu(ctx, v, false, 0, &blocks);
        *max_blocks_per_cu = blocks;
    }
    if (compute_units)
        *compute_units = ctx->compute_units;
    return TRT_OK;
}


extern "C" size_t trt_ansi_delta_capacity(int width, int rows)
{
    if (!trt_delta_size_ok(width, rows))
        return 0;
    return (size_t)std::max(trt_ansi_text_bytes(width, rows), trt_delta_bound(width, rows));
}

static int launch_ansi_delta(trt_context *ctx, hipStream_t stream, const unsigned char *d_shown, const unsigned char *d_next, int width, int rows, void *d_text,
                             size_t capacity_bytes, unsigned long long *d_bytes, const Event *marks = nullptr)
{
    const unsigned long long cells = (unsigned long long)width * (unsigned long long)rows, tiles = trt_delta_tiles(cells);
    if (ctx->d_delta_tile_bytes.capacity < tiles || ctx->d_delta_tile_at.capacity < tiles)
        HIP_TRY(hipStreamSynchronize(stream));
    HIP_TRY(ctx->d_delta_tile_bytes.reserve((size_t)tiles));
    HIP_TRY(ctx->d_delta_tile_at.reserve((size_t)tiles));
    if (marks)
        HIP_TRY(hipEventRecord(marks[0], stream));
    hipLaunchKernelGGL(trt::ansi_delta_measure_kernel, dim3((unsigned)tiles), dim3(TRT_DELTA_BLOCK), 0, stream, d_shown, d_next, width, cells, ctx->d_delta_tile_bytes.ptr);
    if (marks)
        HIP_TRY(hipEventRecord(marks[1], stream));
    hipLaunchKernelGGL(trt::ansi_delta_offsets_kernel, dim3(1), dim3(TRT_DELTA_SCAN_BLOCK), 0, stream, (const unsigned *)ctx->d_delta_tile_bytes.ptr, tiles,
                       ctx->d_delta_tile_at.ptr, d_bytes);
    if (marks)
        HIP_TRY(hipEventRecord(marks[2], stream));
    hipLaunchKernelGGL(trt::ansi_delta_write_kernel, dim3((unsigned)tiles), dim3(TRT_DELTA_BLOCK), 0, stream, d_shown, d_next, width, cells,
                       (const unsigned long long *)ctx->d_delta_tile_at.ptr, (unsigned char *)d_text, (unsigned long long)capacity_bytes);
    if (marks)
        HIP_TRY(hipEventRecord(marks[3], stream));
    HIP_TRY(hipGetLastError());
    return TRT_OK;
}

static int check_delta_from_rgb8(const trt_context *ctx, const void *d_shown_rgb8, const void *d_next_rgb8, int width, int rows, const void *d_text, size_t capacity_bytes,
                                 const unsigned long long *d_bytes)
{
    if (!ctx || !d_shown_rgb8 || !d_next_rgb8 || !d_text || !d_bytes)
        return fail(TRT_ERR_ARGUMENT, "NULL argument");
    if (!trt_delta_size_ok(width, rows))
        return fail(TRT_ERR_ARGUMENT, "screen %d x %d: a delta text has 1 to %d cells per row and 1 to %d rows", width, rows, TRT_DELTA_MAX_WIDTH, TRT_DELTA_MAX_ROWS);
    if (capacity_bytes < trt_ansi_delta_capacity(width, rows))
        return fail(TRT_ERR_CAPACITY, "the delta text of %d x %d needs room for %zu B, %zu given", width, rows, trt_ansi_delta_capacity(width, rows), capacity_bytes);
    return TRT_OK;
}

extern "C" int trt_ansi_delta_from_rgb8_device(trt_context *ctx, const void *d_shown_rgb8, const void *d_next_rgb8, int width, int rows, void *d_text,
                                               size_t capacity_bytes, unsigned long long *d_bytes)
{
    const int rc = check_delta_from_rgb8(ctx, d_shown_rgb8, d_next_rgb8, width, rows, d_text, capacity_bytes, d_bytes);
    if (rc)
        return rc;
    HIP_TRY(hipSetDevice(ctx->device));
    return launch_ansi_delta(ctx, ctx->stream, (const unsigned char *)d_shown_rgb8, (const unsigned char *)d_next_rgb8, width, rows, d_text, capacity_bytes, d_bytes);
}

extern "C" int trt_ansi_delta_kernel_times(trt_context *ctx, const void *d_shown_rgb8, const void *d_next_rgb8, int width, int rows, void *d_text,
                                           size_t capacity_bytes, unsigned long long *d_bytes, float *ms)
{
    if (!ms)
        return fail(TRT_ERR_ARGUMENT, "NULL argument");
    int rc = check_delta_from_rgb8(ctx, d_shown_rgb8, d_next_rgb8, width, rows, d_text, capacity_bytes, d_bytes);
    if (rc)
        return rc;
    HIP_TRY(hipSetDevice(ctx->device));
    Event marks[4];
    for (Event &e : marks)
        HIP_TRY(e.create());
    rc = launch_ansi_delta(ctx, ctx->stream, (const unsigned char *)d_shown_rgb8, (const unsigned char *)d_next_rgb8, width, rows, d_text, capacity_bytes, d_bytes, marks);
    HIP_TRY(hipStreamSynchronize(ctx->stream));
    if (rc)
        return rc;
    for (int k = 0; k < 3; k++)
        HIP_TRY(hipEventElapsedTime(&ms[k], marks[k], marks[k + 1]));
    return TRT_OK;
}

extern "C" int trt_ansi_delta_reset(trt_context *ctx)
{
    if (!ctx)
        return fail(TRT_ERR_ARGUMENT, "ctx is NULL");
    ctx->shown_valid = false;
    return TRT_OK;
}

static int check_render_delta(const trt_context *ctx, const Camera *camera, const trt_rowset *rows, int bounce_limit, int rays_per_pixel, const void *text,
                              size_t capacity_bytes, const void *bytes)
{
    if (!bytes)
        return fail(TRT_ERR_ARGUMENT, "NULL argument");
    if (rowset_valid(rows) && !trt_delta_size_ok(rows->width, trt_rowset_rows(rows)))
        return fail(TRT_ERR_ARGUMENT, "%d x %d owned rows: a delta text has 1 to %d cells per row and 1 to %d rows", rows->width, trt_rowset_rows(rows), TRT_DELTA_MAX_WIDTH,
                    TRT_DELTA_MAX_ROWS);
    const int rc = check_render_arguments(ctx, camera, 1, rows, bounce_limit, rays_per_pixel, text, (size_t)-1, kBytes);
    if (rc)
        return rc;
    const size_t need = trt_ansi_delta_capacity(rows->width, trt_rowset_rows(rows));
    if (capacity_bytes < need)
        return fail(TRT_ERR_CAPACITY, "the text of %d x %d owned rows needs room for %zu B, %zu given", rows->width, trt_rowset_rows(rows), need, capacity_bytes);
    return TRT_OK;
}

static bool same_rowset(const trt_rowset &a, const trt_rowset &b)
{
    return a.width == b.width && a.height == b.height && a.tile_rows == b.tile_rows && a.tile_first == b.tile_first && a.tile_step == b.tile_step;
}

extern "C" int trt_render_device_ansi_delta(trt_context *ctx, const Camera *camera, const trt_rowset *rows, int bounce_limit, int rays_per_pixel, void *d_text,
                                            size_t capacity_bytes, unsigned long long *d_bytes)
{
    int rc = check_render_delta(ctx, camera, rows, bounce_limit, rays_per_pixel, d_text, capacity_bytes, d_bytes);
    if (rc)
        return rc;
    HIP_TRY(hipSetDevice(ctx->device));
    const int width = rows->width, owned = trt_rowset_rows(rows);
    const size_t frame = (size_t)owned * width * 3;
    const bool keyframe = !(ctx->shown_valid && same_rowset(ctx->shown_rows, *rows));
    const int into = ctx->shown_at ^ 1;
    if (ctx->d_shown[0].capacity < frame || ctx->d_shown[1].capacity < frame)
    {
        HIP_TRY(hipStreamSynchronize(ctx->stream));
        HIP_TRY(ctx->d_shown[0].reserve(frame));
        HIP_TRY(ctx->d_shown[1].reserve(frame));
    }
    ctx->shown_valid = false;
    rc = render_device_on(ctx, camera, rows, bounce_limit, rays_per_pixel, ctx->d_shown[into].ptr, frame, 0, kEntryWhole, kBytes);
    if (rc)
        return rc;
    if (keyframe)
    {
        launch_ansi_from_rgb8(ctx->stream, ctx->d_shown[into].ptr, width, owned, d_text);
        hipLaunchKernelGGL(trt::ansi_delta_keyframe_bytes_kernel, dim3(1), dim3(1), 0, ctx->stream, d_bytes, trt_ansi_text_bytes(width, owned));
        HIP_TRY(hipGetLastError());
    }
    else
    {
        rc = launch_ansi_delta(ctx, ctx->stream, ctx->d_shown[ctx->shown_at].ptr, ctx->d_shown[into].ptr, width, owned, d_text, capacity_bytes, d_bytes);
        if (rc)
            return rc;
    }
    ctx->shown_at = into;
    ctx->shown_rows = *rows;
    ctx->shown_valid = true;
    return TRT_OK;
}

extern "C" int trt_render_host_ansi_delta(trt_context *ctx, const Camera *camera, const trt_rowset *rows, int bounce_limit, int rays_per_pixel, char *text,
                                          size_t capacity_bytes, size_t *bytes)
{
    int rc = check_render_delta(ctx, camera, rows, bounce_limit, rays_per_pixel, text, capacity_bytes, bytes);
    if (rc)
        return rc;
    HIP_TRY(hipSetDevice(ctx->device));
    const size_t room = trt_ansi_delta_capacity(rows->width, trt_rowset_rows(rows));
    if (ctx->d_text.capacity < room)
        HIP_TRY(hipStreamSynchronize(ctx->stream));
    HIP_TRY(ctx->d_text.reserve(room));
    HIP_TRY(ctx->d_delta_bytes.reserve(1));
    HIP_TRY(ctx->h_staging.reserve(room));
    const double t_begin = host_now_ms();
    rc = trt_render_device_ansi_delta(ctx, camera, rows, bounce_limit, rays_per_pixel, ctx->d_text.ptr, room, ctx->d_delta_bytes.ptr);
    if (rc)
        return rc;
    unsigned long long length = 0;
    rc = [&]() -> int {
        HIP_TRY(hipMemcpyAsync(ctx->h_staging.ptr, ctx->d_delta_bytes.ptr, sizeof length, hipMemcpyDeviceToHost, ctx->stream));
        HIP_TRY(hipStreamSynchronize(ctx->stream));
        memcpy(&length, ctx->h_staging.ptr, sizeof length);
        if (length > room)
            return fail(TRT_ERR_CAPACITY, "a text of %llu B where %zu are the most", length, room);
        if (length)
        {
            HIP_TRY(hipMemcpyAsync(ctx->h_staging.ptr, ctx->d_text.ptr, (size_t)length, hipMemcpyDeviceToHost, ctx->stream));
            HIP_TRY(hipStreamSynchronize(ctx->stream));
            memcpy(text, ctx->h_staging.ptr, (size_t)length);
        }
        return TRT_OK;
    }();
    if (rc)
    {
        ctx->shown_valid = false;
        return rc;
    }
    *bytes = (size_t)length;
    if (print_host_times())
        fprintf(stderr, "trt_render_host_ansi_delta: %.3f ms for %llu bytes of text\n", host_now_ms() - t_begin, length);
    return TRT_OK;
}
```

terminalraytracer_amd/csrc/trt_rounds.hpp:

```cpp
#pragma once

#include "trt_device.hpp"
#include "trt_filter.h"
#include "trt_lightgrid.h"
#include "trt_raygrid.h"
#include "trt_common.hpp"

#define TRT_EXPECT_LIST(c) __builtin_expect(!!(c), 1)
#define TRT_EXPECT_RARE(c) __builtin_expect(!!(c), 0)

namespace trt
{


#define CONSTANT_AS __attribute__((address_space(4)))
template <class T>
TRT_DEV T load_kernel_argument(const char CONSTANT_AS *at)
{
    static_assert(sizeof(T) % 8 == 0 && alignof(T) == 8, "argument structs are whole 64-bit words");
    T out;
    const unsigned long long CONSTANT_AS *src = (const unsigned long long CONSTANT_AS *)at;
    unsigned long long *dst = (unsigned long long *)&out;
#pragma unroll
    for (size_t i = 0; i < sizeof(T) / 8; i++)
        dst[i] = src[i];
    return out;
}

struct GridView
{
    const trt_dirgrid *dir;
    const trt_pointgrid *point;
    const unsigned long long *dir_lists, *point_lists;
    unsigned dir_stride, point_stride;
    int enabled;
    int list_bits;
    int path_enabled;
    int g_eye, g_sph;
    int patch_m, patch_count;
    unsigned eye_at, sph_at;
    const unsigned long long *path_lists;
    const unsigned long long *pool;
    const double *sphere_fam;
    const double *patch_rec;
    double rg2_sph;
    double slack0;
    trt_rayfamily eye[2];
};

static_assert(sizeof(trt_rayfamily) == 8 * TRT_RAYFAMILY_DOUBLES, "families of the eye in the LDS image");
static_assert(sizeof(trt_dirgrid) == 8 * kDirGridDoubles && sizeof(trt_pointgrid) == 8 * kPointGridDoubles, "light-table headers in the LDS image");

constexpr int kDirRecord = 8;

struct LdsImage
{
    const float4 *cull;
    const float4 *cull_dir;
    const double *sph;
    const double *mat;
    const double *dir;
    const double *pt;
    const double *b255;
    const double *cam;
    const double *jit;
    const trt_dirgrid *dirgrid;
    const trt_pointgrid *pointgrid;
    const double *fam;
    const double *eye;
    const double *patch;
};

inline size_t rounds_lds_bytes(const SceneView &s, int spp, int patches, int frames = 1)
{
    const size_t padded = ((size_t)s.num_spheres + kCullGroup - 1) / kCullGroup * kCullGroup;
    return sizeof(double) * (padded * 2 + (size_t)s.num_spheres * 4 + ((size_t)s.num_spheres + 2) * 5 + (size_t)s.num_dir * kDirRecord +
                             (size_t)s.num_point * 7 + 256 + kLdsCameraDoubles + 2 * (size_t)spp + 1  +
                             (size_t)s.num_dir * padded * 2 + (size_t)s.num_dir * kDirGridDoubles + (size_t)s.num_point * kPointGridDoubles +
                             (size_t)s.num_spheres * 4 + 2 * TRT_RAYFAMILY_DOUBLES + (size_t)patches * TRT_PATCH_RECORD +
                             (size_t)(frames - 1) * (kLdsCameraDoubles + 2 * TRT_RAYFAMILY_DOUBLES));
}

struct ImageParts
{
    float4 *cull, *cull_dir;
    double *sph, *mat, *dir, *pt, *b255, *cam, *jit, *dirgrid, *pointgrid, *fam, *eye, *patch;
};

TRT_DEV ImageParts image_layout(double *base, int n, int nd, int np, int padded, int spp, int frames = 1)
{
    ImageParts p;
    p.cull = (float4 *)base;
    p.sph = base + padded * 2;
    p.mat = p.sph + 4 * n;
    p.dir = p.mat + (n + 2) * 5;
    p.pt = p.dir + nd * kDirRecord;
    p.b255 = p.pt + np * 7;
    p.cam = p.b255 + 256;
    p.jit = p.cam + frames * kLdsCameraDoubles;
    p.cull_dir = (float4 *)(base + (((p.jit + 2 * spp) - base + 1) & ~1L));
    p.dirgrid = (double *)(p.cull_dir + nd * padded);
    p.pointgrid = p.dirgrid + nd * kDirGridDoubles;
    p.fam = p.pointgrid + np * kPointGridDoubles;
    p.eye = p.fam + 4 * n;
    p.patch = p.eye + frames * 2 * TRT_RAYFAMILY_DOUBLES;
    return p;
}

TRT_DEV LdsImage image_view(const ImageParts &p)
{
    return LdsImage{p.cull, p.cull_dir, p.sph, p.mat, p.dir, p.pt, p.b255, p.cam, p.jit,
                    (const trt_dirgrid *)p.dirgrid, (const trt_pointgrid *)p.pointgrid, p.fam, p.eye, p.patch};
}

TRT_DEV void fill_image(const ImageParts &p, const SceneView &s, const CullView &cull, const FrameView &f, const GridView &grids)
{
    const int n = s.num_spheres, nd = s.num_dir, np = s.num_point;
    for (int i = threadIdx.x; i < cull.padded; i += blockDim.x)
        p.cull[i] = ((const float4 *)cull.table)[i];
    for (int i = threadIdx.x; i < n; i += blockDim.x)
    {
        const double *sp = s.spheres + (long)i * kSphereDoubles;
        p.sph[4 * i + 0] = sp[0];
        p.sph[4 * i + 1] = sp[1];
        p.sph[4 * i + 2] = sp[2];
        p.sph[4 * i + 3] = sp[3] * sp[3];
        for (int j = 0; j < 5; j++)
            p.mat[i * 5 + j] = sp[4 + j];
    }
    for (int i = threadIdx.x; i < 10; i += blockDim.x)
        p.mat[n * 5 + i] = s.ground[6 + i];
    for (int i = threadIdx.x; i < nd; i += blockDim.x)
    {
        const double *li = s.dir_lights + i * kDirLightDoubles;
        const d3 tl = unit(scale(load3(li), -1.0));
        p.dir[i * kDirRecord + 0] = tl.x, p.dir[i * kDirRecord + 1] = tl.y, p.dir[i * kDirRecord + 2] = tl.z;
        p.dir[i * kDirRecord + 3] = li[3], p.dir[i * kDirRecord + 4] = li[4], p.dir[i * kDirRecord + 5] = li[5];
        p.dir[i * kDirRecord + 6] = dot(tl, tl);
        p.dir[i * kDirRecord + 7] = dot(tl, load3(s.ground + 3));
    }
    for (int i = threadIdx.x; i < np * 7; i += blockDim.x)
        p.pt[i] = s.point_lights[i];
    for (int i = threadIdx.x; i < 256; i += blockDim.x)
        p.b255[i] = (double)i / 255.0;
    for (int i = threadIdx.x; i < 12; i += blockDim.x)
        p.cam[i] = f.cam[i];
    if (threadIdx.x < 3)
        p.cam[13 + threadIdx.x] = f.cam[6 + threadIdx.x] * -f.cam[12];
    if (threadIdx.x == 0)
        p.cam[12] = -f.cam[12];
    for (int i = threadIdx.x; i < 2 * f.spp; i += blockDim.x)
        p.jit[i] = f.jitter[i];
    __syncthreads();
    for (int i = threadIdx.x; i < nd * cull.padded; i += blockDim.x)
    {
        const int li = i / cull.padded, j = i - li * cull.padded;
        const float4 e = p.cull[j];
        const float dx = (float)p.dir[li * kDirRecord + 0], dy = (float)p.dir[li * kDirRecord + 1], dz = (float)p.dir[li * kDirRecord + 2];
        p.cull_dir[i] = float4{e.x, e.y, e.z, trt_filter_fixed_dir_kk(e.x, e.y, e.z, e.w, dx, dy, dz)};
    }
    if (grids.enabled)
    {
        for (int i = threadIdx.x; i < nd * kDirGridDoubles; i += blockDim.x)
            p.dirgrid[i] = ((const double *)grids.dir)[i];
        for (int i = threadIdx.x; i < np * kPointGridDoubles; i += blockDim.x)
            p.pointgrid[i] = ((const double *)grids.point)[i];
    }
    if (grids.path_enabled)
    {
        for (int i = threadIdx.x; i < n * 4; i += blockDim.x)
            p.fam[i] = grids.sphere_fam[i];
        for (int i = threadIdx.x; i < 2 * TRT_RAYFAMILY_DOUBLES; i += blockDim.x)
            p.eye[i] = ((const double *)grids.eye)[i];
        for (int i = threadIdx.x; i < grids.patch_count * TRT_PATCH_RECORD; i += blockDim.x)
            p.patch[i] = grids.patch_rec[i];
    }
    __syncthreads();
    if (grids.enabled)
    {
        for (int i = threadIdx.x; i < nd; i += blockDim.x)
        {
            const d3 sd = load3(p.dir + i * kDirRecord);
            if (!(__builtin_fabs(dot(sd, sd) - 1.0) <= 9.094947017729282e-13))
                ((trt_dirgrid *)p.dirgrid)[i].rg2 = -1.0f;
        }
        __syncthreads();
    }
}

TRT_DEV LdsImage stage_lds_image(double *lds, const SceneView &s, const CullView &cull, const FrameView &f, const GridView &grids)
{
    const ImageParts p = image_layout(lds, s.num_spheres, s.num_dir, s.num_point, cull.padded, f.spp);
    fill_image(p, s, cull, f, grids);
    return image_view(p);
}

struct Hit
{
    double d2;
    d3 p;
    int i;
    double t;
};


template <bool ANY_HIT, bool REFRACT = false, bool UNIT_A = false>
TRT_DEV bool exact_step(const LdsImage &L, d3 o, d3 d, double a, int i, bool valid, Hit &best, int inside = -1)
{
    static_assert(!(ANY_HIT && REFRACT), "shadow rays are the reference's");
    const double2 c01 = ((const double2 *)L.sph)[2 * i], c23 = ((const double2 *)L.sph)[2 * i + 1];
    const d3 c = d3{c01.x, c01.y, c23.x};
    const d3 oc = sub(o, c);
    const double b = 2.0 * dot(oc, d);
    const double cc = dot(oc, oc) - c23.y;
    const double disc = b * b - 4.0 * a * cc;
    const bool far_root = REFRACT && i == inside;
    bool done = false;
    if (valid && !(disc < 0.0) && (b < 0.0 || far_root))
    {
        const double root = sqrt_exact(disc);
        if (ANY_HIT)
        {
            const double q = -b - root;
            bool hit = UNIT_A ? q > TRT_SHADOW_QMIN : q / (2.0 * a) > 0.0;
            if (UNIT_A && q > 0.0 && !hit)
                hit = q / (2.0 * a) > 0.0;
            best.i = hit ? i : best.i;
            done = hit;
        }
        else
        {
            const double t0 = (far_root ? -b + root : -b - root) / (2.0 * a);
            const bool hit = t0 > 0.0;
            const d3 p = d3{o.x + t0 * d.x, o.y + t0 * d.y, o.z + t0 * d.z};
            const double d2 = dist2(o, p);
            const bool closer = hit && d2 < best.d2;
            best.d2 = closer ? d2 : best.d2;
            best.t = closer ? t0 : best.t;
            best.i = closer ? i : best.i;
        }
    }
    return done;
}

constexpr int kListPrefilter = 12;


template <bool ANY_HIT, bool REFRACT = false, int MARK_BASE = 0>
TRT_DEV Hit trace(const LdsImage &L, const CullView &cull, int n, d3 o, d3 d, bool active, unsigned long long active_lanes, d3 gp, d3 gn, unsigned &phase2_rounds, unsigned &lane_tests,
                  const float4 *fixed, bool use_list, unsigned long long cell, const unsigned long long *pool, int list_bits, int inside = -1,
                  const double *shared_ad = nullptr)
{
#define TRT_TRACE_MARK(k) TRT_MARK_AT(MARK_BASE + (k))
    (void)fixed;
    Hit best;
    best.d2 = __builtin_inf();
    best.p = o;
    best.i = -1;
    best.t = 0.0;
    const double a = shared_ad ? shared_ad[0] : dot(d, d);
    if (TRT_EXPECT_LIST(use_list))
    {
        const unsigned ctl = (unsigned)(cell >> 56);
        bool pooled = (ctl & TRT_LIST_POOLED) != 0;
        int count = active ? (pooled ? (int)((cell >> 32) & 0xffffu) : (int)ctl) : 0;
        const unsigned at = (unsigned)cell;
        const unsigned entry_mask = (1u << list_bits) - 1u;
        const int per_shift = list_bits == 8 ? 3 : 2, per_mask = (1 << per_shift) - 1;
        int fetch_at = lanes_with(pooled) != 0 ? 0 : per_mask + 1;
        asm("" : "+s"(fetch_at));
        unsigned long long cur = cell;
        int k = 0;
        TRT_TRACE_MARK(0);
        if (__any(count > kListPrefilter))
        {
            trt_ray_filter flt;
            trt_filter_setup(&flt, o.x, o.y, o.z, d.x, d.y, d.z, a, cull.c0x, cull.c0y, cull.c0z, cull.cn, cull.rm);
            unsigned long long kept = 0, word = cell;
            int nk = 0;
            bool over = false;
            for (int j = 0; __any(j < count); j++)
            {
                const bool valid = j < count;
                if ((j & per_mask) == fetch_at)
                    if (__any(valid && pooled))
                        if (valid && pooled)
                            word = pool[at + ((unsigned)j >> per_shift)];
                const unsigned i = valid ? (unsigned)word & entry_mask : 0u;
                word >>= list_bits;
                unsigned sign;
                if (ANY_HIT && fixed)
                {
                    const float4 e = fixed[i];
                    sign = trt_filter_sign_fixed_dir(&flt, e.x, e.y, e.z, e.w);
                }
                else
                {
                    const float4 e = L.cull[i];
                    sign = trt_filter_sign(&flt, e.x, e.y, e.z, e.w);
                }
                if (valid && (!flt.ok || !(sign >> 31)))
                {
                    over = over || nk > per_mask;
                    kept |= nk <= per_mask ? (unsigned long long)i << (list_bits * nk) : 0ull;
                    nk++;
                }
            }
            if (!__any(over))
            {
                cur = kept;
                count = nk;
                pooled = false;
                fetch_at = per_mask + 1;
            }
        }
        TRT_TRACE_MARK(1);
        while (__any(k < count))
        {
            phase2_rounds++;
            const bool valid = k < count;
            lane_tests += valid;
            if ((k & per_mask) == fetch_at)
                if (__any(valid && pooled))
                    if (valid && pooled)
                        cur = pool[at + ((unsigned)k >> per_shift)];
            const int i = valid ? (int)((unsigned)cur & entry_mask) : 0;
            cur >>= list_bits;
            k++;
            if (exact_step<ANY_HIT, REFRACT, ANY_HIT>(L, o, d, a, i, valid, best, inside))
                count = 0;
        }
    }
    else
    {
        trt_ray_filter flt;
        trt_filter_setup(&flt, o.x, o.y, o.z, d.x, d.y, d.z, a, cull.c0x, cull.c0y, cull.c0z, cull.cn, cull.rm);
        TRT_TRACE_MARK(0);
        for (int base = 0; base < cull.padded; base += 64)
        {
            const int chunk = (cull.padded - base) < 64 ? (cull.padded - base) : 64;
            unsigned word[2];
#pragma unroll
            for (int h = 0; h < 2; h++)
            {
                const int first = base + 32 * h, count = (chunk - 32 * h) < 32 ? (chunk - 32 * h) : 32;
                unsigned bits = ~0u;
                for (int g = 0; g < count; g += kCullGroup)
                {
#pragma unroll
                    for (int j = 0; j < kCullGroup; j++)
                    {
                        if (ANY_HIT && fixed)
                        {
                            const float4 e = fixed[first + g + j];
                            bits = __builtin_amdgcn_alignbit(bits, trt_filter_sign_fixed_dir(&flt, e.x, e.y, e.z, e.w), 31);
                        }
                        else
                        {
                            const float4 e = L.cull[first + g + j];
                            bits = __builtin_amdgcn_alignbit(bits, trt_filter_sign(&flt, e.x, e.y, e.z, e.w), 31);
                        }
                    }
                }
                word[h] = count > 0 ? ~(bits << (32 - count)) & (count == 32 ? ~0u : ~((1u << (32 - count)) - 1u)) : 0u;
            }
            unsigned long long cand = ((unsigned long long)word[0] << 32) | word[1];
            if (!flt.ok)
                cand = chunk == 64 ? ~0ull : ~((1ull << (64 - chunk)) - 1ull);
            if (!active)
                cand = 0;
            TRT_TRACE_MARK(1);
            while (__any(cand != 0))
            {
                phase2_rounds++;
                const int lead = __builtin_clzll(cand | 1ull);
                const bool valid = cand != 0 && base + lead < n;
                lane_tests += valid;
                const int i = valid ? base + lead : 0;
                cand &= ~(0x8000000000000000ull >> lead);
                if (exact_step<ANY_HIT, REFRACT>(L, o, d, a, i, valid, best, inside))
                    cand = 0ull;
            }
        }
    }
    if (!ANY_HIT && best.i >= 0)
        best.p = d3{o.x + best.t * d.x, o.y + best.t * d.y, o.z + best.t * d.z};
    TRT_TRACE_MARK(2);
    {
        const double denom = shared_ad ? shared_ad[1] : dot(d, gn), num = dot(sub(gp, o), gn);
        const bool steep = __builtin_fabs(denom) > 0.00001;
        const bool same_sign = (long long)(__builtin_bit_cast(unsigned long long, num) ^ __builtin_bit_cast(unsigned long long, denom)) >= 0;
        const bool maybe = active && !(ANY_HIT && best.i >= 0) && steep && same_sign;
        unsigned long long maybe_lanes = active_lanes & lanes_with(steep) & lanes_with(same_sign);
        if (ANY_HIT)
            maybe_lanes &= ~lanes_with(best.i >= 0);
        if (maybe_lanes != 0)
        {
            const double t = num / denom;
            const bool hit = maybe && t > 0.00001;
            if (ANY_HIT)
                best.i = hit ? n : best.i;
            else
            {
                const d3 p = d3{o.x + t * d.x, o.y + t * d.y, o.z + t * d.z};
                const double d2 = dist2(o, p);
                const bool closer = hit && d2 < best.d2;
                best.d2 = closer ? d2 : best.d2;
                best.p.x = closer ? p.x : best.p.x;
                best.p.y = closer ? p.y : best.p.y;
                best.p.z = closer ? p.z : best.p.z;
                best.i = closer ? n : best.i;
            }
        }
    }
    TRT_TRACE_MARK(3);
#undef TRT_TRACE_MARK
    return best;
}

TRT_DEV void point_light_search(const LdsImage &L, int n, d3 o, d3 d, bool active, unsigned long long active_lanes, d3 gp, d3 gn, unsigned &rounds, unsigned &lane_tests,
                                unsigned long long cell, const unsigned long long *pool, int list_bits, double lo, double hi, bool &dark, bool &unsure)
{
    (void)n;
    const double a = dot(d, d);
    const unsigned ctl = (unsigned)(cell >> 56);
    const bool pooled = (ctl & TRT_LIST_POOLED) != 0;
    int count = active ? (pooled ? (int)((cell >> 32) & 0xffffu) : (int)ctl) : 0;
    const unsigned at = (unsigned)cell;
    const unsigned entry_mask = (1u << list_bits) - 1u;
    const int per_shift = list_bits == 8 ? 3 : 2, per_mask = (1 << per_shift) - 1;
    int fetch_at = lanes_with(pooled) != 0 ? 0 : per_mask + 1;
    asm("" : "+s"(fetch_at));
    unsigned long long cur = cell;
    int k = 0;
    dark = false, unsure = false;
    while (__any(k < count))
    {
        rounds++;
        const bool valid = k < count;
        lane_tests += valid;
        if ((k & per_mask) == fetch_at)
            if (__any(valid && pooled))
                if (valid && pooled)
                    cur = pool[at + ((unsigned)k >> per_shift)];
        const int i = valid ? (int)((unsigned)cur & entry_mask) : 0;
        cur >>= list_bits;
        k++;
        const double2 c01 = ((const double2 *)L.sph)[2 * i], c23 = ((const double2 *)L.sph)[2 * i + 1];
        const d3 oc = sub(o, d3{c01.x, c01.y, c23.x});
        const double b = 2.0 * dot(oc, d);
        const double cc = dot(oc, oc) - c23.y;
        const double disc = b * b - 4.0 * a * cc;
        if (valid && !(disc < 0.0) && b < 0.0)
        {
            const double q = -b - sqrt_exact(disc), qq = q * q;
            const bool blocks = q > TRT_SHADOW_QMIN && qq * TRT_SHADOW_K1 <= lo;
            unsure = unsure || (q > 0.0 && !blocks && !(qq >= hi));
            dark = dark || blocks;
            count = blocks ? 0 : count;
        }
    }
    {
        const double denom = dot(d, gn), num = dot(sub(gp, o), gn);
        const bool steep = __builtin_fabs(denom) > 0.00001;
        const bool same_sign = (long long)(__builtin_bit_cast(unsigned long long, num) ^ __builtin_bit_cast(unsigned long long, denom)) >= 0;
        const bool maybe = active && !dark && steep && same_sign;
        if (__any(maybe))
        {
            const double t = num / denom;
            const bool hit = maybe && t > 0.00001;
            const double qq = (t * t) * (4.0 * a) * a;
            const bool blocks = hit && qq * TRT_SHADOW_K1 <= lo;
            dark = dark || blocks;
            unsure = unsure || (hit && !blocks && !(qq >= hi));
        }
    }
    unsure = unsure && !dark;
}

template <bool BATCH = false>
TRT_DEV unsigned long long path_cell(const LdsImage &L, const GridView &G, int n, int fam, d3 o, d3 d, bool active, unsigned long long active_lanes,
                                     unsigned long long &fallback_lanes, int frame = 0)
{
    const bool in_family = fam >= 0;
    const unsigned long long family_lanes = lanes_with(in_family);
    const bool has = active && in_family;
    const int f = has ? fam : 0;
    const int s = f >= 2 ? f - 2 : 0, i = s >= n ? s - n : s;
    const bool of_eye = f < 2, mirrored = s >= n;
    const double *rec = L.fam + 4 * i;
    d3 apex = mirrored ? load3(rec) : load3(L.sph + 4 * i);
    double r_chk = mirrored ? rec[3] + TRT_FAMILY_SLACK : rec[3];
    const double *E = BATCH ? L.eye + frame * (2 * TRT_RAYFAMILY_DOUBLES) + TRT_RAYFAMILY_DOUBLES * (f & 1) : L.eye + TRT_RAYFAMILY_DOUBLES * (f & 1);
    const double rg2_eye = E[5];
    if (of_eye)
    {
        apex = load3(E);
        r_chk = E[3];
    }
    const double rg2 = of_eye ? rg2_eye : G.rg2_sph;
    const d3 w = sub(o, apex);
    const d3 c = d3{w.y * d.z - w.z * d.y, w.z * d.x - w.x * d.z, w.x * d.y - w.y * d.x};
    const bool near_line = dot(c, c) <= r_chk * r_chk, ahead = dot(w, d) >= -r_chk, in_range = dot(w, w) <= rg2;
    const bool unit_dir = __builtin_fabs(dot(d, d) - 1.0) <= 9.094947017729282e-13;
    const bool member = near_line & ahead & in_range & unit_dir;
    const unsigned long long member_lanes = family_lanes & lanes_with(near_line) & lanes_with(ahead) & lanes_with(in_range) & lanes_with(unit_dir);
    const int g = of_eye ? G.g_eye : G.g_sph;
    const int at = trt_cubemap_cell((float)d.x, (float)d.y, (float)d.z, 0.5f * (float)g, (float)(g - 1), g);
    const unsigned eye_cells = 6u * (unsigned)G.g_eye * (unsigned)G.g_eye, sph_cells = 6u * (unsigned)G.g_sph * (unsigned)G.g_sph;
    const unsigned base = of_eye ? G.eye_at + (BATCH ? 2u * (unsigned)frame + (unsigned)f : (unsigned)f) * eye_cells : G.sph_at + (unsigned)s * sph_cells;
    unsigned long long cell = 0;
    if (has && member)
        cell = G.path_lists[base + (unsigned)at];
    fallback_lanes = active_lanes & (~member_lanes | lanes_with((unsigned)(cell >> 56) == TRT_LIST_NONE));
    return cell;
}

template <bool BATCH = false>
TRT_DEV unsigned long long path_cell_patches(const LdsImage &L, const GridView &G, int n, int &fam, d3 o, d3 d, bool active, unsigned long long active_lanes,
                                             unsigned long long &fallback_lanes, int frame = 0)
{
    const bool in_family = fam >= 0;
    const unsigned long long family_lanes = lanes_with(in_family);
    const bool has = active && in_family;
    const int f = has ? fam : 0;
    const bool of_eye = f < 2, mirrored = f >= 2 + n;
    const int code = f - 2 - n;
    const int i = mirrored ? code >> TRT_PATCH_SHIFT : (of_eye ? 0 : f - 2);
    const double *at_sphere = L.sph + 4 * i, *at_mirror = L.fam + 4 * i;
    const double *src = of_eye ? L.eye + (BATCH ? frame * (2 * TRT_RAYFAMILY_DOUBLES) : 0) + TRT_RAYFAMILY_DOUBLES * (f & 1) : (mirrored ? at_mirror : at_sphere);
    const d3 base_at = load3(src);
    const int here = trt_cubemap_cell((float)(o.x - base_at.x), (float)(o.y - base_at.y), (float)(o.z - base_at.z), 0.5f * (float)G.patch_m,
                                      (float)(G.patch_m - 1), G.patch_m);
    const int k = mirrored ? code & ((1 << TRT_PATCH_SHIFT) - 1) : (of_eye ? 0 : here);
    fam = !has ? -1 : (f == 0 ? 1 : (!of_eye && !mirrored ? 2 + n + (((f - 2) << TRT_PATCH_SHIFT) | k) : -1));
    const double r_abs = of_eye ? 0.0 : at_mirror[3];
    const double *pr = L.patch + TRT_PATCH_RECORD * k + (mirrored ? 4 : 0);
    const d3 apex = d3{TRT_PATCH_APEX(base_at.x, r_abs, pr[0]), TRT_PATCH_APEX(base_at.y, r_abs, pr[1]), TRT_PATCH_APEX(base_at.z, r_abs, pr[2])};
    const double rho = pr[3];
    double rchk_eye = src[3], rg2_eye = src[5];
    asm("" : "+v"(rchk_eye), "+v"(rg2_eye));
    double r_chk = TRT_PATCH_RCHK(r_abs, rho, G.slack0), rg2 = G.rg2_sph;
    r_chk = mirrored ? r_chk + TRT_FAMILY_SLACK : r_chk;
    r_chk = of_eye ? rchk_eye : r_chk;
    rg2 = of_eye ? rg2_eye : rg2;
    const d3 w = sub(o, apex);
    const d3 c = d3{w.y * d.z - w.z * d.y, w.z * d.x - w.x * d.z, w.x * d.y - w.y * d.x};
    const bool near_line = dot(c, c) <= r_chk * r_chk, ahead = dot(w, d) >= -r_chk, in_range = dot(w, w) <= rg2;
    const bool unit_dir = __builtin_fabs(dot(d, d) - 1.0) <= 9.094947017729282e-13;
    const bool member = near_line & ahead & in_range & unit_dir;
    const unsigned long long member_lanes = family_lanes & lanes_with(near_line) & lanes_with(ahead) & lanes_with(in_range) & lanes_with(unit_dir);
    const int g = of_eye ? G.g_eye : G.g_sph;
    const int at = trt_cubemap_cell((float)d.x, (float)d.y, (float)d.z, 0.5f * (float)g, (float)(g - 1), g);
    const unsigned eye_cells = 6u * (unsigned)G.g_eye * (unsigned)G.g_eye, sph_cells = 6u * (unsigned)G.g_sph * (unsigned)G.g_sph;
    const unsigned table = ((mirrored ? (unsigned)n : 0u) + (unsigned)i) * (unsigned)G.patch_count + (unsigned)k;
    const unsigned base = of_eye ? G.eye_at + (BATCH ? 2u * (unsigned)frame + (unsigned)f : (unsigned)f) * eye_cells : G.sph_at + table * sph_cells;
    unsigned long long cell = 0;
    if (has && member)
        cell = G.path_lists[base + (unsigned)at];
    fallback_lanes = active_lanes & (~member_lanes | lanes_with((unsigned)(cell >> 56) == TRT_LIST_NONE));
    return cell;
}

TRT_DEV unsigned lanes_below(unsigned long long mask)
{
    return __builtin_amdgcn_mbcnt_hi((unsigned)(mask >> 32), __builtin_amdgcn_mbcnt_lo((unsigned)mask, 0u));
}

struct Tally
{
    unsigned path = 0, shadow = 0, rounds = 0, swept = 0, passes = 0;
    unsigned iters[3] = {0, 0, 0};
    unsigned tests[3] = {0, 0, 0};
    unsigned full = 0;
};

struct PathHit
{
    Hit ph;
    bool hit;
    bool sky;
    unsigned long long hit_lanes, sky_lanes;
    d3 back;
    d3 normal;
    int mat;
};

template <bool COUNT, bool REFRACT = false, bool PATCHES = false, bool BATCH = false>
TRT_DEV PathHit path_stage(const LdsImage &L, const CullView &cull, const GridView &grids, int n, d3 o, d3 d, int &fam, bool alive, unsigned long long alive_lanes,
                           d3 gp, d3 gn, Tally &tally, int inside = -1, int frame = 0)
{
    bool p_list = false;
    unsigned long long p_cell = 0;
    if (grids.path_enabled)
    {
        unsigned long long fallback_lanes;
        if constexpr (PATCHES)
            p_cell = path_cell_patches<BATCH>(L, grids, n, fam, o, d, alive, alive_lanes, fallback_lanes, frame);
        else
            p_cell = path_cell<BATCH>(L, grids, n, fam, o, d, alive, alive_lanes, fallback_lanes, frame);
        p_list = fallback_lanes == 0;
    }
    if (COUNT && !p_list)
        tally.swept++;
    PathHit r;
    r.ph = trace<false, REFRACT, 2>(L, cull, n, o, d, alive, alive_lanes, gp, gn, tally.iters[0], tally.tests[0], nullptr, p_list, p_cell, grids.pool, grids.list_bits, inside);
    r.hit = alive && r.ph.i >= 0;
    r.sky = alive && r.ph.i < 0;
    r.hit_lanes = alive_lanes & lanes_with(r.ph.i >= 0);
    r.sky_lanes = alive_lanes & ~r.hit_lanes;
    if (r.hit)
        fam = r.ph.i < n ? 2 + r.ph.i : (PATCHES ? fam : (fam == 0 ? 1 : (fam >= 2 && fam < 2 + n ? fam + n : -1)));
    r.back = unit(r.hit ? sub(o, r.ph.p) : d);
    r.normal = d;
    r.mat = 0;
    if (r.hit_lanes != 0)
    {
        d3 raw = gn;
        r.mat = n + checker_odd(r.ph.p);
        if (r.ph.i >= 0 && r.ph.i < n)
        {
            raw = sub(r.ph.p, load3(L.sph + 4 * r.ph.i));
            r.mat = r.ph.i;
        }
        r.normal = unit(raw);
    }
    TRT_MARK_AT(6);
    return r;
}

template <bool COUNT>
TRT_DEV d3 shadow_stage(const LdsImage &L, const CullView &cull, const GridView &grids, int n, int nd, int nl, d3 o, d3 normal, int mat,
                        bool lit_lanes, unsigned long long lit_word, d3 gp, d3 gn, Tally &tally)
{
    d3 lit = d3{0.0, 0.0, 0.0};
    if (lit_word == 0)
        return lit;
    for (int li = 0; li < nl; li++)
    {
        if (COUNT && lit_lanes)
            tally.shadow++;
        d3 sd, lcolor;
        bool is_lit;
        double factor;
        if (li < nd)
        {
            TRT_MARK_AT(24);
            sd = load3(L.dir + li * kDirRecord);
            lcolor = load3(L.dir + li * kDirRecord + 3);
            bool use_list = false;
            unsigned long long cell = 0;
            if (grids.enabled)
            {
                const trt_dirgrid *G = L.dirgrid + li;
                int far;
                const int c = trt_dirgrid_cell(G, o.x, o.y, o.z, &far);
                if (lit_lanes && !far)
                    cell = grids.dir_lists[(size_t)li * grids.dir_stride + (unsigned)c];
                use_list = (lit_word & (lanes_with(far != 0) | lanes_with((unsigned)(cell >> 56) == TRT_LIST_NONE))) == 0;
            }
            if (COUNT && !use_list)
                tally.swept++;
            TRT_MARK_AT(8);
            const Hit sh = trace<true, false, 9>(L, cull, n, o, sd, lit_lanes, lit_word, gp, gn, tally.iters[1], tally.tests[1], L.cull_dir + li * cull.padded, use_list, cell, grids.pool, grids.list_bits,
                                                 -1, L.dir + li * kDirRecord + 6);
            is_lit = sh.i < 0;
            factor = min1(dot(normal, sd));
            TRT_MARK_AT(13);
        }
        else
        {
            TRT_MARK_AT(25);
            const double *pl = L.pt + (li - nd) * 7;
            const d3 to_light = sub(load3(pl), o);
            const double light_d2 = dot(to_light, to_light);
            const double strength = clampd(pl[6] / light_d2, 0.0, 1.0);
            sd = unit(to_light);
            lcolor = load3(pl + 3);
            bool use_list = false;
            unsigned long long cell = 0;
            if (grids.enabled)
            {
                const trt_pointgrid *G = L.pointgrid + (li - nd);
                int far;
                const int c = trt_pointgrid_cell(G, o.x, o.y, o.z, &far);
                far |= !(__builtin_fabs(dot(sd, sd) - 1.0) <= 9.094947017729282e-13);
                if (lit_lanes && !far)
                    cell = grids.point_lists[(size_t)(li - nd) * grids.point_stride + (unsigned)c];
                use_list = (lit_word & (lanes_with(far != 0) | lanes_with((unsigned)(cell >> 56) == TRT_LIST_NONE))) == 0;
            }
            if (COUNT && !use_list)
                tally.swept++;
            TRT_MARK_AT(14);
            bool full = !use_list;
            is_lit = true;
            if (use_list)
            {
                const trt_pointgrid *G = L.pointgrid + (li - nd);
                double lo, hi;
                trt_point_shadow_bounds(G, light_d2, dot(sd, sd), &lo, &hi);
                bool dark, unsure;
                point_light_search(L, n, o, sd, lit_lanes, lit_word, gp, gn, tally.iters[2], tally.tests[2], cell, grids.pool, grids.list_bits, lo, hi, dark, unsure);
                is_lit = !dark;
                full = __any(lit_lanes && unsure);
                TRT_MARK_AT(17);
            }
            if (TRT_EXPECT_RARE(full))
            {
                if (COUNT)
                    tally.full++;
                const Hit sh = trace<false, false, 26>(L, cull, n, o, sd, lit_lanes, lit_word, gp, gn, tally.iters[2], tally.tests[2], nullptr, use_list, cell, grids.pool, grids.list_bits);
                is_lit = sh.i < 0;
                const bool surely_lit = light_d2 < sh.d2 * (1.0 - 1.01e-6) - 1.01e-6;
                const bool surely_dark = sh.d2 > 1e-10 && light_d2 >= sh.d2;
                if (sh.i >= 0)
                    is_lit = surely_lit;
                if (__any(lit_lanes && sh.i >= 0 && !surely_lit && !surely_dark))
                {
                    const d3 to_blocker = sub(add(sh.p, scale(unit(sub(o, sh.p)), 0.000001)), o);
                    if (sh.i >= 0 && !surely_lit && !surely_dark)
                        is_lit = light_d2 < dot(to_blocker, to_blocker);
                }
            }
            factor = strength * min1(dot(normal, sd));
            TRT_MARK_AT(19);
        }
        if (lit_lanes && is_lit)
            lit = add(lit, mulc(scale(lcolor, factor), load3(L.mat + mat * 5)));
    }
    return lit;
}

#ifndef TRT_ROUNDS_WAVES
#if TRT_BLOCK > 768
#define TRT_ROUNDS_WAVES 4
#else
#define TRT_ROUNDS_WAVES 3
#endif
#endif

constexpr int kRingTasks = 128;
constexpr int kRingDoubles = 7 * kRingTasks + kRingTasks / 4 + 3 * 64;

constexpr size_t kArgScene = 0;
constexpr size_t kArgCull = (kArgScene + sizeof(SceneView) + alignof(CullView) - 1) / alignof(CullView) * alignof(CullView);
constexpr size_t kArgFrame = (kArgCull + sizeof(CullView) + alignof(FrameView) - 1) / alignof(FrameView) * alignof(FrameView);
constexpr size_t kArgGrids = (kArgFrame + sizeof(FrameView) + alignof(GridView) - 1) / alignof(GridView) * alignof(GridView);
struct RenderKernelArguments
{
    SceneView s;
    CullView cull;
    FrameView f;
    GridView grids;
};
static_assert(offsetof(RenderKernelArguments, cull) == kArgCull && offsetof(RenderKernelArguments, f) == kArgFrame &&
                  offsetof(RenderKernelArguments, grids) == kArgGrids,
              "TRT_FRESH_ARGS reads the kernel's arguments at these offsets");

constexpr int kBatchMax = 8;
struct BatchView
{
    double cam[kBatchMax][15];
    trt_rayfamily eye[kBatchMax][2];
    unsigned frames, units_per_frame;
    unsigned frame_magic, reserved;
};
constexpr size_t kArgBatch = (kArgGrids + sizeof(GridView) + alignof(BatchView) - 1) / alignof(BatchView) * alignof(BatchView);
static_assert(kArgBatch + sizeof(BatchView) <= 4096, "the arguments of a BATCH launch fit the 4 KB kernarg segment");
static_assert(sizeof(BatchView::cam) % 8 == 0 && offsetof(BatchView, eye) == sizeof(BatchView::cam) && offsetof(BatchView, frames) % 8 == 0,
              "BatchView is read as whole 64-bit words");
constexpr int kBatchFrameShift = 28;
constexpr int kBatchBounceMask = (1 << kBatchFrameShift) - 1;
static_assert(kBatchMax <= 8, "three bits of `bounces` hold the frame");
template <class T>
TRT_DEV T *in_device_memory(T *p)
{
    T __attribute__((address_space(1))) *g = (T __attribute__((address_space(1))) *)p;
    asm("" : "+s"(g));
    return (T *)g;
}
TRT_DEV SceneView in_device_memory(SceneView v)
{
    v.spheres = in_device_memory(v.spheres), v.dir_lights = in_device_memory(v.dir_lights), v.point_lights = in_device_memory(v.point_lights);
    v.sky = in_device_memory(v.sky);
    return v;
}
TRT_DEV CullView in_device_memory(CullView v)
{
    v.table = in_device_memory(v.table);
    return v;
}
TRT_DEV FrameView in_device_memory(FrameView v)
{
    v.jitter = in_device_memory(v.jitter), v.col_x = in_device_memory(v.col_x), v.row_y = in_device_memory(v.row_y);
    v.samples = in_device_memory(v.samples), v.out = in_device_memory(v.out), v.ior = in_device_memory(v.ior);
    v.counters = in_device_memory(v.counters), v.queue = in_device_memory(v.queue);
    return v;
}
TRT_DEV GridView in_device_memory(GridView v)
{
    v.dir = in_device_memory(v.dir), v.point = in_device_memory(v.point);
    v.dir_lists = in_device_memory(v.dir_lists), v.point_lists = in_device_memory(v.point_lists);
    v.path_lists = in_device_memory(v.path_lists), v.pool = in_device_memory(v.pool), v.sphere_fam = in_device_memory(v.sphere_fam);
    v.patch_rec = in_device_memory(v.patch_rec);
    return v;
}
#define TRT_FRESH_ARGS                                                                             \
    const char CONSTANT_AS *fresh_ = (const char CONSTANT_AS *)__builtin_amdgcn_kernarg_segment_ptr(); \
    asm volatile("" : "+s"(fresh_));                                                               \
    const SceneView s = in_device_memory(load_kernel_argument<SceneView>(fresh_ + kArgScene));     \
    const CullView cull = in_device_memory(load_kernel_argument<CullView>(fresh_ + kArgCull));     \
    const FrameView f = in_device_memory(load_kernel_argument<FrameView>(fresh_ + kArgFrame));     \
    const GridView grids = in_device_memory(load_kernel_argument<GridView>(fresh_ + kArgGrids));   \
    const int n = s.num_spheres, nd = s.num_dir, nl = s.num_dir + s.num_point;                     \
    const unsigned pixels_here = (unsigned)f.local_rows * (unsigned)f.width;                       \
    const unsigned total = pixels_here * (unsigned)f.spp;                                          \
    const d3 gp = load3(s.ground), gn = load3(s.ground + 3);                                       \
    (void)n, (void)nd, (void)nl, (void)total, (void)pixels_here, (void)gp, (void)gn, (void)cull, (void)grids

struct alignas(8) BatchShape
{
    unsigned frames, units_per_frame, frame_magic, reserved;
};
TRT_DEV BatchShape load_batch_shape()
{
    const char CONSTANT_AS *args = (const char CONSTANT_AS *)__builtin_amdgcn_kernarg_segment_ptr();
    asm volatile("" : "+s"(args));
    return load_kernel_argument<BatchShape>(args + kArgBatch + offsetof(BatchView, frames));
}

TRT_DEV LdsImage stage_lds_image_batch(double *lds, const SceneView &s, const CullView &cull, const FrameView &f, const GridView &grids)
{
    const int frames = (int)load_batch_shape().frames;
    const ImageParts p = image_layout(lds, s.num_spheres, s.num_dir, s.num_point, cull.padded, f.spp, frames);
    fill_image(p, s, cull, f, grids);
    const double CONSTANT_AS *cams = (const double CONSTANT_AS *)((const char CONSTANT_AS *)__builtin_amdgcn_kernarg_segment_ptr() + kArgBatch);
    const double CONSTANT_AS *eyes = cams + sizeof(BatchView::cam) / sizeof(double);
    for (int i = threadIdx.x; i < frames * kLdsCameraDoubles; i += blockDim.x)
    {
        const int b = i / kLdsCameraDoubles, j = i - b * kLdsCameraDoubles;
        const double CONSTANT_AS *c = cams + b * 15;
        p.cam[i] = j < 12 ? c[j] : (j == 12 ? -c[12] : c[6 + (j - 13)] * -c[12]);
    }
    if (grids.path_enabled)
        for (int i = threadIdx.x; i < frames * 2 * TRT_RAYFAMILY_DOUBLES; i += blockDim.x)
            p.eye[i] = eyes[i];
    __syncthreads();
    return image_view(p);
}

#ifndef TRT_COMPACT_BLOCK
#define TRT_COMPACT_BLOCK 1024
#endif
constexpr int kCompactBlock = TRT_COMPACT_BLOCK;
constexpr int kBigBlock = 1024;

template <bool COUNT, bool REFRACT = false, bool COMPACT = false, bool PATCHES = false, bool BIG = false, bool DEVICE_IMAGE = false, bool BATCH = false,
          class... BatchArgument>
__global__ __launch_bounds__(BIG ? kBigBlock : COMPACT ? kCompactBlock : kPersistentBlock, ((COMPACT && !COUNT) || BIG) ? 4 : TRT_ROUNDS_WAVES) void render_rounds_kernel(SceneView s, CullView cull, FrameView f, GridView grids, BatchArgument... batch)
{
    static_assert(sizeof...(BatchArgument) == (BATCH ? 1 : 0), "a BATCH launch has one more argument, a BatchView; the others none");
    static_assert(!BATCH || (!COUNT && !REFRACT && !BIG && !DEVICE_IMAGE), "several frames per launch: the plain, patch and decoupled rounds");
    static_assert(!(REFRACT && COMPACT), "the refraction extension runs on the plain rounds");
    static_assert(!(PATCHES && COMPACT), "scenes with patches run the plain rounds");
    static_assert(!BIG || (PATCHES && !COUNT && !REFRACT && !COMPACT), "1024-thread workgroups: the shipping patch instantiation only");
    static_assert(!DEVICE_IMAGE || (!REFRACT && !COMPACT && !BIG), "the device-memory image: the plain rounds only");
    extern __shared__ __attribute__((aligned(16))) double lds[];
    const LdsImage L = BATCH ? stage_lds_image_batch(lds, s, cull, f, grids)
                       : DEVICE_IMAGE ? image_view(image_layout(const_cast<double *>(f.image), s.num_spheres, s.num_dir, s.num_point, cull.padded, f.spp))
                                      : stage_lds_image(lds, s, cull, f, grids);
    const int n = s.num_spheres, nd = s.num_dir, nl = s.num_dir + s.num_point;
    const int lane = threadIdx.x & 63;
    const unsigned pixels_here = (unsigned)f.local_rows * (unsigned)f.width;
    const unsigned total = pixels_here * (unsigned)f.spp;
    (void)total;
    const d3 gp = load3(s.ground), gn = load3(s.ground + 3);

    bool alive = true;
    bool want_unit = true;
    unsigned slot_id = 0;
    d3 sample = d3{0.0, 0.0, 0.0};
    double weight = 1.0, weight_sum = 0.0;
    int bounces = 0;
    d3 o = d3{0.0, 0.0, 0.0}, d = d3{0.0, 0.0, -1.0};
    d3 next_dir = d;
    int fam = 0;
    int inside = -1;
    Tally tally;
    unsigned pool_next = 0, pool_end = 0;
    {
        const unsigned group = blockIdx.x, waves = blockDim.x >> 6, wave = (unsigned)__builtin_amdgcn_readfirstlane((int)(threadIdx.x >> 6));
        const unsigned j = (group >> f.queue_shift) * waves + wave;
        pool_next = ((j << f.queue_shift) + (group & ((1u << f.queue_shift) - 1u))) * f.chunk;
        pool_end = pool_next + f.chunk;
    }
    double *const ring = lds + f.ring_at + (unsigned)__builtin_amdgcn_readfirstlane((int)(threadIdx.x >> 6)) * kRingDoubles;
    unsigned short *const ring_mat = (unsigned short *)(ring + 7 * kRingTasks);
    double *const parked = ring + 7 * kRingTasks + kRingTasks / 4;
    if (COMPACT)
    {
        for (int i = lane; i < kRingDoubles; i += 64)
            ring[i] = 0.0;
        __builtin_amdgcn_fence(__ATOMIC_SEQ_CST, "wavefront");
    }
    unsigned q_head = 0, q_tail = 0, q_old = 0;
    unsigned my_task = 0, old_slot = 0;
    bool my_open = false, old_open = false;
    bool waiting = false;
    for (;;)
    {
        TRT_MARK_AT(22);
        {
            TRT_FRESH_ARGS;
            const unsigned long long need = __ballot(want_unit);
            if (need)
            {
                const unsigned wanted = (unsigned)__builtin_popcountll(need);
                const unsigned rank = lanes_below(need);
                unsigned mine = pool_next + rank;
                if (pool_end - pool_next < wanted)
                {
                    const unsigned left = pool_end - pool_next;
                    unsigned fresh = 0;
                    const int leader = __builtin_ctzll(need);
                    const unsigned word = blockIdx.x & ((1u << f.queue_shift) - 1u);
                    if (lane == leader)
                        fresh = atomicAdd(f.queue + word * kQueueStride, 1u);
                    fresh = (unsigned)__builtin_amdgcn_readlane((int)fresh, leader);
                    fresh = ((fresh << f.queue_shift) + word) * f.chunk;
                    if (rank >= left)
                        mine = fresh + (rank - left);
                    pool_next = fresh + (wanted - left);
                    pool_end = fresh + f.chunk;
                }
                else
                    pool_next += wanted;
                BatchShape shape{};
                if constexpr (BATCH)
                    shape = load_batch_shape();
                if (want_unit)
                {
                    alive = mine < (BATCH ? shape.frames * total : total);
                    if (alive)
                    {
                        unsigned frame = 0;
                        if constexpr (BATCH)
                        {
                            frame = __umulhi(mine, shape.frame_magic);
                            const int within = (int)(mine - frame * total);
                            const int under = within < 0, over = within >= (int)total;
                            frame += (unsigned)(over - under);
                            mine = (unsigned)(within + (under - over) * (int)total);
                        }
                        const double *const cam = L.cam + (BATCH ? frame * (unsigned)kLdsCameraDoubles : 0u);
                        unsigned pixel = __umulhi(mine, f.spp_magic);
                        int k = (int)(mine - pixel * (unsigned)f.spp);
                        {
                            const int under = k < 0, over = k >= f.spp;
                            pixel += (unsigned)(over - under);
                            k += (under - over) * f.spp;
                        }
                        slot_id = (unsigned)k * pixels_here + pixel;
                        unsigned row = __umulhi(pixel, f.width_magic);
                        int col = (int)(pixel - row * (unsigned)f.width);
                        {
                            const int under = col < 0, over = col >= f.width;
                            row += (unsigned)(over - under);
                            col += (under - over) * f.width;
                        }
                        const double sx = f.col_x[col] + L.jit[k];
                        const double sy = f.row_y[f.tile_first == 0 && f.tile_step == 1 ? (int)row : frame_row_of_magic(f, row)] + L.jit[f.spp + k];
                        d3 dir = d3{0.0, 0.0, 0.0};
                        dir = add(dir, scale(load3(cam + 0), sx));
                        dir = add(dir, scale(load3(cam + 3), sy));
                        dir = add(dir, load3(cam + 13));
                        next_dir = sub(dir, load3(cam + 9));
                        o = load3(cam + 9);
                        fam = 0;
                        inside = -1;
                        sample = d3{0.0, 0.0, 0.0};
                        weight = 1.0;
                        weight_sum = 0.0;
                        bounces = BATCH ? (int)(frame << kBatchFrameShift) : 0;
                    }
                    want_unit = false;
                }
            }
        }
        const unsigned long long alive_lanes = lanes_with(alive);
        if ((COMPACT ? alive_lanes | lanes_with(waiting) : alive_lanes) == 0)
            break;
        if (COUNT)
            tally.rounds++;
        TRT_MARK_AT(0);
        d = unit(next_dir);

        if (COUNT && alive)
            tally.path++;
        TRT_MARK_AT(1);
        PathHit hit;
        {
            TRT_FRESH_ARGS;
            hit = path_stage<COUNT, REFRACT, PATCHES, BATCH>(L, cull, grids, n, o, d, fam, alive, alive_lanes, gp, gn, tally, inside, BATCH ? bounces >> kBatchFrameShift : 0);
        }
        if constexpr (COMPACT)
        {
            const bool path_hit = hit.hit, path_sky = hit.sky;
            bool end_sample = path_sky;
            uint32_t sky_t = 0;
            const double weight_before = weight;
            {
            TRT_FRESH_ARGS;
            if (hit.sky_lanes != 0)
                sky_t = sky_texel_wave(s.sky, s.sky_dim, hit.back, s.sky_dim_f, path_sky, hit.sky_lanes);
            const unsigned long long hits = hit.hit_lanes;
            if (hits)
            {
                if (path_hit)
                {
                    my_task = q_tail + lanes_below(hits);
                    my_open = true;
                    const unsigned at = my_task & (kRingTasks - 1);
                    const d3 so = add(hit.ph.p, scale(hit.back, 0.000001));
                    ring[0 * kRingTasks + at] = so.x, ring[1 * kRingTasks + at] = so.y, ring[2 * kRingTasks + at] = so.z;
                    ring[3 * kRingTasks + at] = hit.normal.x, ring[4 * kRingTasks + at] = hit.normal.y, ring[5 * kRingTasks + at] = hit.normal.z;
                    ring[6 * kRingTasks + at] = weight;
                    ring_mat[at] = (unsigned short)hit.mat;
                    const d3 nd3 = reflect(d, hit.normal);
                    parked[lane] = nd3.x, parked[64 + lane] = nd3.y, parked[128 + lane] = nd3.z;
                    weight *= L.mat[hit.mat * 5 + 3];
                    bounces++;
                    end_sample = !((BATCH ? bounces & kBatchBounceMask : bounces) < f.bounce_limit && weight > 0.00001);
                }
                q_tail += (unsigned)__builtin_popcountll(hits);
            }
            }
            if (alive)
                weight_sum += weight_before;
            __builtin_amdgcn_fence(__ATOMIC_SEQ_CST, "wavefront");
            TRT_MARK_AT(7);
            if (q_head != q_tail && ((int)(q_old - q_head) > 0 || q_tail - q_head >= 64u))
            {
                TRT_FRESH_ARGS;
                const unsigned take = q_tail - q_head < 64u ? q_tail - q_head : 64u;
                const bool has = (unsigned)lane < take;
                const unsigned at = (q_head + (unsigned)lane) & (kRingTasks - 1);
                const d3 so = d3{ring[0 * kRingTasks + at], ring[1 * kRingTasks + at], ring[2 * kRingTasks + at]};
                const d3 sn = d3{ring[3 * kRingTasks + at], ring[4 * kRingTasks + at], ring[5 * kRingTasks + at]};
                const int sm = ring_mat[at];
                if (COUNT)
                    tally.passes++;
                const d3 lit = shadow_stage<COUNT>(L, cull, grids, n, nd, nl, so, sn, sm, has, lanes_with(has), gp, gn, tally);
                d3 color = d3{clampd(lit.x, 0.0, 1.0), clampd(lit.y, 0.0, 1.0), clampd(lit.z, 0.0, 1.0)};
                color = scale(color, ring[6 * kRingTasks + at]);
                if (has)
                    ring[3 * kRingTasks + at] = color.x, ring[4 * kRingTasks + at] = color.y, ring[5 * kRingTasks + at] = color.z;
                q_head += take;
            }
            q_old = q_tail;
            __builtin_amdgcn_fence(__ATOMIC_SEQ_CST, "wavefront");
            TRT_MARK_AT(20);
            if (old_open)
            {
                const unsigned at = old_slot;
                sample = add(sample, d3{ring[3 * kRingTasks + at], ring[4 * kRingTasks + at], ring[5 * kRingTasks + at]});
            }
            if (my_open && (int)(q_head - my_task) > 0)
            {
                const unsigned at = my_task & (kRingTasks - 1);
                sample = add(sample, d3{ring[3 * kRingTasks + at], ring[4 * kRingTasks + at], ring[5 * kRingTasks + at]});
                my_open = false;
            }
            if (path_hit)
            {
                o = d3{ring[0 * kRingTasks + (my_task & (kRingTasks - 1))], ring[1 * kRingTasks + (my_task & (kRingTasks - 1))],
                       ring[2 * kRingTasks + (my_task & (kRingTasks - 1))]};
                next_dir = d3{parked[lane], parked[64 + lane], parked[128 + lane]};
            }
            bool finish = end_sample;
            if (waiting)
                finish = true, waiting = false;
            else if (end_sample && my_open)
                finish = false, waiting = true, alive = false;
            old_slot = my_task & (kRingTasks - 1), old_open = my_open, my_open = false;
            if (path_sky)
            {
                const d3 color = d3{L.b255[sky_t & 0xFF], L.b255[(sky_t >> 8) & 0xFF], L.b255[(sky_t >> 16) & 0xFF]};
                sample = add(sample, scale(color, weight));
            }
            if (__any(finish))
            {
                const double q = 1.0 / weight_sum;
                if (finish)
                {
                    TRT_FRESH_ARGS;
                    unsigned slot = slot_id;
                    asm volatile("" : "+v"(slot));
                    double *out = f.samples + (size_t)slot * 3;
                    if constexpr (BATCH)
                        out += (size_t)(unsigned)(bounces >> kBatchFrameShift) * total * 3;
                    out[0] = sample.x * q;
                    out[1] = sample.y * q;
                    out[2] = sample.z * q;
                    want_unit = true;
                }
            }
        }
        else
        {
        const bool leaving = REFRACT && hit.hit && hit.ph.i == inside;
        const bool path_hit = hit.hit && !leaving, path_sky = hit.sky;
        const d3 h_normal = hit.normal;
        const int h_mat = hit.mat;
        bool end_sample = false;
        double weight_sum_new = weight_sum + weight;
        uint32_t sky_t = 0;
        if (hit.sky_lanes != 0)
        {
            TRT_FRESH_ARGS;
            sky_t = sky_texel_wave(s.sky, s.sky_dim, hit.back, s.sky_dim_f, path_sky, hit.sky_lanes);
            end_sample = path_sky;
        }
        d3 lit;
        if (!REFRACT)
        {
            if (path_hit)
            {
                next_dir = reflect(d, h_normal);
                o = add(hit.ph.p, scale(hit.back, 0.000001));
            }
            TRT_MARK_AT(7);
            if (COUNT && hit.hit_lanes != 0)
                tally.passes++;
            {
                TRT_FRESH_ARGS;
                lit = shadow_stage<COUNT>(L, cull, grids, n, nd, nl, o, h_normal, h_mat, path_hit, hit.hit_lanes, gp, gn, tally);
            }
        }
        else
        {
            const d3 shade_at = add(hit.ph.p, scale(hit.back, 0.000001));
            if (hit.hit)
            {
                bool bent = false;
                if (hit.ph.i < n)
                {
                    const double ior = f.ior[hit.ph.i];
                    if (ior > 0.0)
                    {
                        const d3 nn = leaving ? scale(h_normal, -1.0) : h_normal;
                        const double cosi = -dot(nn, d);
                        const double eta = leaving ? ior : 1.0 / ior;
                        const double kk = 1.0 - (eta * eta) * (1.0 - cosi * cosi);
                        bent = true;
                        if (!(kk < 0.0))
                        {
                            const double fac = eta * cosi - __builtin_sqrt(kk);
                            next_dir = d3{eta * d.x + fac * nn.x, eta * d.y + fac * nn.y, eta * d.z + fac * nn.z};
                            o = sub(hit.ph.p, scale(hit.back, 0.000001));
                            inside = leaving ? -1 : hit.ph.i;
                        }
                        else
                        {
                            next_dir = reflect(d, nn);
                            o = shade_at;
                        }
                    }
                }
                if (!bent)
                {
                    next_dir = reflect(d, h_normal);
                    o = shade_at;
                }
            }
            lit = shadow_stage<COUNT>(L, cull, grids, n, nd, nl, shade_at, h_normal, h_mat, path_hit, lanes_with(path_hit), gp, gn, tally);
        }

        TRT_MARK_AT(20);
        if (path_hit)
        {
            TRT_FRESH_ARGS;
            d3 color = d3{clampd(lit.x, 0.0, 1.0), clampd(lit.y, 0.0, 1.0), clampd(lit.z, 0.0, 1.0)};
            color = scale(color, weight);
            weight *= L.mat[h_mat * 5 + 3];
            bounces++;
            sample = add(sample, color);
            if ((BATCH ? bounces & kBatchBounceMask : bounces) < f.bounce_limit && weight > 0.00001)
                weight_sum = weight_sum_new;
            else
                end_sample = true;
        }
        if (REFRACT && leaving)
        {
            bounces++;
            weight_sum_new = weight_sum;
            if (!(bounces < f.bounce_limit))
                end_sample = true;
        }
        if (path_sky)
        {
            const d3 color = d3{L.b255[sky_t & 0xFF], L.b255[(sky_t >> 8) & 0xFF], L.b255[(sky_t >> 16) & 0xFF]};
            sample = add(sample, scale(color, weight));
        }
        if (__any(end_sample))
        {
            const double q = 1.0 / weight_sum_new;
            if (end_sample)
            {
                TRT_FRESH_ARGS;
                double *out = f.samples + (size_t)slot_id * 3;
                if constexpr (BATCH)
                    out += (size_t)(unsigned)(bounces >> kBatchFrameShift) * total * 3;
                out[0] = sample.x * q;
                out[1] = sample.y * q;
                out[2] = sample.z * q;
                want_unit = true;
            }
        }
        }
        TRT_MARK_AT(21);
    }

#if defined(TRT_MARKS) && TRT_MARKS == 2
    if (!COUNT && f.counters)
    {
#define TRT_PROFILE_DUMP(kind)                                                         \
    {                                                                                  \
        unsigned x_;                                                                   \
        asm volatile("v_mov_b32 %0, v" #kind : "=v"(x_));                              \
        atomicAdd(&f.counters[kProfileAt + 64 * ((kind) - 240) + lane], (unsigned long long)x_); \
    }
        TRT_PROFILE_DUMP(240) TRT_PROFILE_DUMP(241) TRT_PROFILE_DUMP(242) TRT_PROFILE_DUMP(243) TRT_PROFILE_DUMP(244) TRT_PROFILE_DUMP(245)
        TRT_PROFILE_DUMP(246) TRT_PROFILE_DUMP(247) TRT_PROFILE_DUMP(248) TRT_PROFILE_DUMP(249) TRT_PROFILE_DUMP(250)
#undef TRT_PROFILE_DUMP
    }
#endif
    if (COUNT && f.counters)
    {
        atomicAdd(&f.counters[0], (unsigned long long)tally.path);
        atomicAdd(&f.counters[1], (unsigned long long)tally.shadow);
        for (int k = 0; k < 3; k++)
            atomicAdd(&f.counters[33 + k], (unsigned long long)tally.tests[k]);
        if (lane == 0)
        {
            atomicAdd(&f.counters[2], (unsigned long long)tally.rounds);
            atomicAdd(&f.counters[3], (unsigned long long)tally.iters[0] + tally.iters[1] + tally.iters[2]);
            atomicAdd(&f.counters[28], (unsigned long long)tally.swept);
            atomicAdd(&f.counters[29], (unsigned long long)tally.passes);
            for (int k = 0; k < 3; k++)
                atomicAdd(&f.counters[30 + k], (unsigned long long)tally.iters[k]);
            atomicAdd(&f.counters[36], (unsigned long long)tally.full);
        }
    }
}

template <bool PATCHES>
__global__ __launch_bounds__(kPersistentBlock) void probe_rounds_kernel(SceneView s, CullView cull, FrameView f, GridView grids, const double *rays,
                                                                        const int *families, long count, int *obj, double *point, double *normal,
                                                                        double *material, double *lit_out)
{
    extern __shared__ __attribute__((aligned(16))) double lds[];
    const LdsImage L = stage_lds_image(lds, s, cull, f, grids);
    const int n = s.num_spheres, nd = s.num_dir, nl = s.num_dir + s.num_point;
    const d3 gp = load3(s.ground), gn = load3(s.ground + 3);
    const long i = (long)blockIdx.x * blockDim.x + threadIdx.x;
    const bool alive = i < count;
    const long at = alive ? i : 0;
    const d3 o = load3(rays + 6 * at), d = load3(rays + 6 * at + 3);
    int fam = families ? families[at] : -1;
    Tally tally;
    const PathHit hit = path_stage<false, false, PATCHES>(L, cull, grids, n, o, d, fam, alive, lanes_with(alive), gp, gn, tally);
    const d3 surface = hit.hit ? add(hit.ph.p, scale(hit.back, 0.000001)) : o;
    const d3 lit = shadow_stage<false>(L, cull, grids, n, nd, nl, surface, hit.normal, hit.mat, hit.hit, hit.hit_lanes, gp, gn, tally);
    const uint32_t sky_t = sky_texel_wave(s.sky, s.sky_dim, hit.back, s.sky_dim_f, alive && !hit.hit, hit.sky_lanes);
    if (!alive)
        return;
    d3 color = d3{0.0, 0.0, 0.0};
    double refl = 0.0, spec = 0.0;
    d3 nrm = hit.back;
    if (hit.hit)
    {
        color = load3(L.mat + hit.mat * 5);
        refl = L.mat[hit.mat * 5 + 3];
        spec = L.mat[hit.mat * 5 + 4];
        nrm = hit.normal;
    }
    else
    {
        const uint32_t t = sky_t;
        color = d3{L.b255[t & 0xFF], L.b255[(t >> 8) & 0xFF], L.b255[(t >> 16) & 0xFF]};
    }
    obj[i] = hit.hit ? (hit.ph.i < n ? 1 : 2) : 0;
    point[3 * i + 0] = surface.x, point[3 * i + 1] = surface.y, point[3 * i + 2] = surface.z;
    normal[3 * i + 0] = nrm.x, normal[3 * i + 1] = nrm.y, normal[3 * i + 2] = nrm.z;
    material[5 * i + 0] = color.x, material[5 * i + 1] = color.y, material[5 * i + 2] = color.z;
    material[5 * i + 3] = refl, material[5 * i + 4] = spec;
    const d3 c = hit.hit ? d3{clampd(lit.x, 0.0, 1.0), clampd(lit.y, 0.0, 1.0), clampd(lit.z, 0.0, 1.0)} : d3{0.0, 0.0, 0.0};
    lit_out[3 * i + 0] = c.x, lit_out[3 * i + 1] = c.y, lit_out[3 * i + 2] = c.z;
}

}
```

Before: 37.39 billion.

## Compact LDS image view to base plus host-computed offsets, interleave jitter

New measurement: 37.67 billion, median of 6. No clear change (+0.8%).

```diff
diff --git a/terminalraytracer_amd/csrc/trt_device.hpp b/terminalraytracer_amd/csrc/trt_device.hpp
--- a/terminalraytracer_amd/csrc/trt_device.hpp
+++ b/terminalraytracer_amd/csrc/trt_device.hpp
@@ -2,6 +2,8 @@
 
 #include <hip/hip_runtime.h>
 #include <stdint.h>
+
+#include "trt_image_layout.h"
 
 namespace trt
 {
@@ -155,6 +157,7 @@
     int local_rows;
     int bounce_limit, spp;
     const double *image;
+    trt_image_at at;
 };
 
 TRT_DEV int frame_row_of_magic(const FrameView &f, unsigned local_row)
diff --git a/terminalraytracer_amd/csrc/trt_diag.hip b/terminalraytracer_amd/csrc/trt_diag.hip
--- a/terminalraytracer_amd/csrc/trt_diag.hip
+++ b/terminalraytracer_amd/csrc/trt_diag.hip
@@ -346,6 +346,7 @@
     trt::FrameView f{};
     memcpy(f.cam, camera, sizeof(Camera));
     f.jitter = ctx->d_jitter.ptr;
+    f.at = trt_image_offsets(trt::image_dims(ctx->scene, ctx->cull, 0, ctx->grids));
     if (ctx->grids.path_enabled && ctx->grids.patch_m > 0)
         hipLaunchKernelGGL(trt::probe_rounds_kernel<true>, dim3((unsigned)((n + trt::kPersistentBlock - 1) / trt::kPersistentBlock)), dim3(trt::kPersistentBlock),
                            image_lds_bytes(ctx, 0), ctx->stream, ctx->scene, ctx->cull, f, ctx->grids, (const double *)dr,
diff --git a/terminalraytracer_amd/csrc/trt_image_layout.h b/terminalraytracer_amd/csrc/trt_image_layout.h
--- /dev/null
+++ b/terminalraytracer_amd/csrc/trt_image_layout.h
@@ -0,0 +1,84 @@
+#ifndef TRT_IMAGE_LAYOUT_H
+#define TRT_IMAGE_LAYOUT_H
+
+#if defined(__HIPCC__) || defined(__HIP__)
+#define TRT_IMAGE_HD __host__ __device__ __forceinline__
+#else
+#define TRT_IMAGE_HD static inline
+#endif
+
+#define TRT_IMAGE_CAMERA_DOUBLES 16
+#define TRT_IMAGE_EYE_DOUBLES 12
+#define TRT_IMAGE_FRAME_DOUBLES (TRT_IMAGE_CAMERA_DOUBLES + TRT_IMAGE_EYE_DOUBLES)
+#define TRT_IMAGE_DIR_RECORD 8
+#define TRT_IMAGE_POINT_RECORD 7
+#define TRT_IMAGE_DIRGRID_DOUBLES 14
+#define TRT_IMAGE_POINTGRID_DOUBLES 9
+#define TRT_IMAGE_PATCH_RECORD 8
+#define TRT_IMAGE_CULL_GROUP 8
+
+#define TRT_IMAGE_FRAME0 0
+#define TRT_IMAGE_CAM TRT_IMAGE_FRAME0
+#define TRT_IMAGE_EYE (TRT_IMAGE_CAM + TRT_IMAGE_CAMERA_DOUBLES)
+#define TRT_IMAGE_B255 (TRT_IMAGE_FRAME0 + TRT_IMAGE_FRAME_DOUBLES)
+#define TRT_IMAGE_FIXED_END (TRT_IMAGE_B255 + 256)
+#define TRT_IMAGE_FIXED_DOUBLES ((TRT_IMAGE_FIXED_END + 1) / 2 * 2)
+
+typedef struct trt_image_dims
+{
+    int n, nd, np;
+    int padded;
+    int spp;
+    int patches;
+} trt_image_dims;
+
+TRT_IMAGE_HD int trt_image_padded(int n) { return (n + TRT_IMAGE_CULL_GROUP - 1) / TRT_IMAGE_CULL_GROUP * TRT_IMAGE_CULL_GROUP; }
+
+TRT_IMAGE_HD trt_image_dims trt_image_dims_of(int n, int nd, int np, int spp, int patches)
+{
+    trt_image_dims d;
+    d.n = n, d.nd = nd, d.np = np, d.padded = trt_image_padded(n), d.spp = spp, d.patches = patches;
+    return d;
+}
+
+TRT_IMAGE_HD int trt_image_cull(void) { return TRT_IMAGE_FIXED_DOUBLES; }
+TRT_IMAGE_HD int trt_image_sph(trt_image_dims d) { return TRT_IMAGE_FIXED_DOUBLES + 2 * d.padded; }
+TRT_IMAGE_HD int trt_image_fam(trt_image_dims d) { return trt_image_sph(d) + 4 * d.n; }
+TRT_IMAGE_HD int trt_image_mat(trt_image_dims d) { return trt_image_sph(d) + 8 * d.n; }
+TRT_IMAGE_HD int trt_image_cull_dir(trt_image_dims d) { return (trt_image_mat(d) + 5 * (d.n + 2) + 1) & ~1; }
+TRT_IMAGE_HD int trt_image_patch(trt_image_dims d) { return trt_image_cull_dir(d) + 2 * d.nd * d.padded; }
+
+TRT_IMAGE_HD int trt_image_jit(trt_image_dims d) { return trt_image_patch(d) + TRT_IMAGE_PATCH_RECORD * d.patches; }
+TRT_IMAGE_HD int trt_image_dir(trt_image_dims d) { return trt_image_jit(d) + 2 * d.spp; }
+TRT_IMAGE_HD int trt_image_dirgrid(trt_image_dims d) { return trt_image_dir(d) + d.nd * TRT_IMAGE_DIR_RECORD; }
+TRT_IMAGE_HD int trt_image_pt(trt_image_dims d) { return trt_image_dirgrid(d) + d.nd * TRT_IMAGE_DIRGRID_DOUBLES; }
+TRT_IMAGE_HD int trt_image_pointgrid(trt_image_dims d) { return trt_image_pt(d) + d.np * TRT_IMAGE_POINT_RECORD; }
+
+typedef struct trt_image_at
+{
+    unsigned sph, fam, mat, cull_dir, patch, jit, dir, pt, dirgrid, pointgrid, frames, reserved;
+} trt_image_at;
+
+TRT_IMAGE_HD int trt_image_frames(trt_image_dims d) { return trt_image_pointgrid(d) + d.np * TRT_IMAGE_POINTGRID_DOUBLES; }
+TRT_IMAGE_HD int trt_image_frame(trt_image_dims d, int b)
+{
+    return b == 0 ? TRT_IMAGE_FRAME0 : trt_image_frames(d) + (b - 1) * TRT_IMAGE_FRAME_DOUBLES;
+}
+
+TRT_IMAGE_HD trt_image_at trt_image_offsets(trt_image_dims d)
+{
+    trt_image_at a;
+    a.sph = (unsigned)trt_image_sph(d), a.fam = (unsigned)trt_image_fam(d), a.mat = (unsigned)trt_image_mat(d);
+    a.cull_dir = (unsigned)trt_image_cull_dir(d), a.patch = (unsigned)trt_image_patch(d), a.jit = (unsigned)trt_image_jit(d);
+    a.dir = (unsigned)trt_image_dir(d), a.pt = (unsigned)trt_image_pt(d), a.dirgrid = (unsigned)trt_image_dirgrid(d);
+    a.pointgrid = (unsigned)trt_image_pointgrid(d), a.frames = (unsigned)trt_image_frames(d), a.reserved = 0;
+    return a;
+}
+
+TRT_IMAGE_HD long long trt_image_doubles(trt_image_dims d, int frames)
+{
+    return (long long)trt_image_frames(d) + (long long)(frames - 1) * TRT_IMAGE_FRAME_DOUBLES;
+}
+TRT_IMAGE_HD long long trt_image_bytes(trt_image_dims d, int frames) { return 8 * trt_image_doubles(d, frames); }
+
+#endif
diff --git a/terminalraytracer_amd/csrc/trt_render.hip b/terminalraytracer_amd/csrc/trt_render.hip
--- a/terminalraytracer_amd/csrc/trt_render.hip
+++ b/terminalraytracer_amd/csrc/trt_render.hip
@@ -271,7 +271,7 @@
 constexpr int kImageBlock = 1024;
 __global__ __launch_bounds__(kImageBlock) void stage_image_kernel(trt::SceneView s, trt::CullView cull, trt::FrameView f, trt::GridView grids)
 {
-    trt::fill_image(trt::image_layout(const_cast<double *>(f.image), s.num_spheres, s.num_dir, s.num_point, cull.padded, f.spp), s, cull, f, grids);
+    trt::fill_image(trt::image_layout(const_cast<double *>(f.image), trt::image_dims(s, cull, f.spp, grids)), s, cull, f, grids);
 }
 
 }
@@ -519,6 +519,7 @@
     if (ctx->ior_count)
         f.ior = ctx->d_ior.ptr;
     f.ring_at = plan.ring_at;
+    f.at = trt_image_offsets(trt::image_dims(ctx->scene, ctx->cull, f.spp, grids));
     f.queue_shift = plan.queue_shift;
     f.chunk = plan.chunk;
     if (ctx->scratch_fill)
diff --git a/terminalraytracer_amd/csrc/trt_rounds.hpp b/terminalraytracer_amd/csrc/trt_rounds.hpp
--- a/terminalraytracer_amd/csrc/trt_rounds.hpp
+++ b/terminalraytracer_amd/csrc/trt_rounds.hpp
@@ -2,6 +2,7 @@
 
 #include "trt_device.hpp"
 #include "trt_filter.h"
+#include "trt_image_layout.h"
 #include "trt_lightgrid.h"
 #include "trt_raygrid.h"
 #include "trt_common.hpp"
@@ -51,34 +52,51 @@
 static_assert(sizeof(trt_rayfamily) == 8 * TRT_RAYFAMILY_DOUBLES, "families of the eye in the LDS image");
 static_assert(sizeof(trt_dirgrid) == 8 * kDirGridDoubles && sizeof(trt_pointgrid) == 8 * kPointGridDoubles, "light-table headers in the LDS image");
 
-constexpr int kDirRecord = 8;
+constexpr int kDirRecord = TRT_IMAGE_DIR_RECORD;
+
+static_assert(kLdsCameraDoubles == TRT_IMAGE_CAMERA_DOUBLES && 2 * TRT_RAYFAMILY_DOUBLES == TRT_IMAGE_EYE_DOUBLES && kPointLightDoubles == TRT_IMAGE_POINT_RECORD &&
+                  kDirGridDoubles == TRT_IMAGE_DIRGRID_DOUBLES && kPointGridDoubles == TRT_IMAGE_POINTGRID_DOUBLES && TRT_PATCH_RECORD == TRT_IMAGE_PATCH_RECORD &&
+                  kCullGroup == TRT_IMAGE_CULL_GROUP,
+              "trt_image_layout.h lays out these records");
+static_assert(TRT_IMAGE_FIXED_DOUBLES % 2 == 0, "the culling table and the sphere records behind it are 16-byte aligned");
 
 struct LdsImage
 {
-    const float4 *cull;
-    const float4 *cull_dir;
-    const double *sph;
-    const double *mat;
-    const double *dir;
-    const double *pt;
-    const double *b255;
-    const double *cam;
-    const double *jit;
-    const trt_dirgrid *dirgrid;
-    const trt_pointgrid *pointgrid;
-    const double *fam;
-    const double *eye;
-    const double *patch;
+    const double *base;
+    trt_image_at at;
+    TRT_DEV const float4 *cull() const { return (const float4 *)(base + trt_image_cull()); }
+    TRT_DEV const float4 *cull_dir() const { return (const float4 *)(base + at.cull_dir); }
+    TRT_DEV const double *sph() const { return base + at.sph; }
+    TRT_DEV const double *mat() const { return base + at.mat; }
+    TRT_DEV const double *dir() const { return base + at.dir; }
+    TRT_DEV const double *pt() const { return base + at.pt; }
+    TRT_DEV const double *b255() const { return base + TRT_IMAGE_B255; }
+    TRT_DEV const double *cam() const { return base + TRT_IMAGE_CAM; }
+    TRT_DEV const double *eye() const { return base + TRT_IMAGE_EYE; }
+    TRT_DEV const double *frame(int b) const { return base + (b == 0 ? (unsigned)TRT_IMAGE_FRAME0 : at.frames + (unsigned)(b - 1) * TRT_IMAGE_FRAME_DOUBLES); }
+    TRT_DEV const double *jit() const { return base + at.jit; }
+    TRT_DEV const trt_dirgrid *dirgrid() const { return (const trt_dirgrid *)(base + at.dirgrid); }
+    TRT_DEV const trt_pointgrid *pointgrid() const { return (const trt_pointgrid *)(base + at.pointgrid); }
+    TRT_DEV const double *fam() const { return base + at.fam; }
+    TRT_DEV const double *patch() const { return base + at.patch; }
 };
 
+__host__ __device__ inline trt_image_dims image_dims(const SceneView &s, const CullView &cull, int spp, const GridView &grids)
+{
+    trt_image_dims d;
+    d.n = s.num_spheres, d.nd = s.num_dir, d.np = s.num_point, d.padded = cull.padded, d.spp = spp;
+    d.patches = grids.path_enabled ? grids.patch_count : 0;
+    return d;
+}
+
+TRT_DEV LdsImage image_view(const double *base, const FrameView &f)
+{
+    return LdsImage{base, f.at};
+}
+
 inline size_t rounds_lds_bytes(const SceneView &s, int spp, int patches, int frames = 1)
 {
-    const size_t padded = ((size_t)s.num_spheres + kCullGroup - 1) / kCullGroup * kCullGroup;
-    return sizeof(double) * (padded * 2 + (size_t)s.num_spheres * 4 + ((size_t)s.num_spheres + 2) * 5 + (size_t)s.num_dir * kDirRecord +
-                             (size_t)s.num_point * 7 + 256 + kLdsCameraDoubles + 2 * (size_t)spp + 1  +
-                             (size_t)s.num_dir * padded * 2 + (size_t)s.num_dir * kDirGridDoubles + (size_t)s.num_point * kPointGridDoubles +
-                             (size_t)s.num_spheres * 4 + 2 * TRT_RAYFAMILY_DOUBLES + (size_t)patches * TRT_PATCH_RECORD +
-                             (size_t)(frames - 1) * (kLdsCameraDoubles + 2 * TRT_RAYFAMILY_DOUBLES));
+    return (size_t)trt_image_bytes(trt_image_dims_of(s.num_spheres, s.num_dir, s.num_point, spp, patches), frames);
 }
 
 struct ImageParts
@@ -87,30 +105,24 @@
     double *sph, *mat, *dir, *pt, *b255, *cam, *jit, *dirgrid, *pointgrid, *fam, *eye, *patch;
 };
 
-TRT_DEV ImageParts image_layout(double *base, int n, int nd, int np, int padded, int spp, int frames = 1)
+TRT_DEV ImageParts image_layout(double *base, const trt_image_dims &d)
 {
     ImageParts p;
-    p.cull = (float4 *)base;
-    p.sph = base + padded * 2;
-    p.mat = p.sph + 4 * n;
-    p.dir = p.mat + (n + 2) * 5;
-    p.pt = p.dir + nd * kDirRecord;
-    p.b255 = p.pt + np * 7;
-    p.cam = p.b255 + 256;
-    p.jit = p.cam + frames * kLdsCameraDoubles;
-    p.cull_dir = (float4 *)(base + (((p.jit + 2 * spp) - base + 1) & ~1L));
-    p.dirgrid = (double *)(p.cull_dir + nd * padded);
-    p.pointgrid = p.dirgrid + nd * kDirGridDoubles;
-    p.fam = p.pointgrid + np * kPointGridDoubles;
-    p.eye = p.fam + 4 * n;
-    p.patch = p.eye + frames * 2 * TRT_RAYFAMILY_DOUBLES;
+    p.cull = (float4 *)(base + trt_image_cull());
+    p.cull_dir = (float4 *)(base + trt_image_cull_dir(d));
+    p.sph = base + trt_image_sph(d);
+    p.mat = base + trt_image_mat(d);
+    p.dir = base + trt_image_dir(d);
+    p.pt = base + trt_image_pt(d);
+    p.b255 = base + TRT_IMAGE_B255;
+    p.cam = base + TRT_IMAGE_CAM;
+    p.jit = base + trt_image_jit(d);
+    p.dirgrid = base + trt_image_dirgrid(d);
+    p.pointgrid = base + trt_image_pointgrid(d);
+    p.fam = base + trt_image_fam(d);
+    p.eye = base + TRT_IMAGE_EYE;
+    p.patch = base + trt_image_patch(d);
     return p;
-}
-
-TRT_DEV LdsImage image_view(const ImageParts &p)
-{
-    return LdsImage{p.cull, p.cull_dir, p.sph, p.mat, p.dir, p.pt, p.b255, p.cam, p.jit,
-                    (const trt_dirgrid *)p.dirgrid, (const trt_pointgrid *)p.pointgrid, p.fam, p.eye, p.patch};
 }
 
 TRT_DEV void fill_image(const ImageParts &p, const SceneView &s, const CullView &cull, const FrameView &f, const GridView &grids)
@@ -150,7 +162,7 @@
     if (threadIdx.x == 0)
         p.cam[12] = -f.cam[12];
     for (int i = threadIdx.x; i < 2 * f.spp; i += blockDim.x)
-        p.jit[i] = f.jitter[i];
+        p.jit[i] = f.jitter[(i & 1) * f.spp + (i >> 1)];
     __syncthreads();
     for (int i = threadIdx.x; i < nd * cull.padded; i += blockDim.x)
     {
@@ -190,9 +202,8 @@
 
 TRT_DEV LdsImage stage_lds_image(double *lds, const SceneView &s, const CullView &cull, const FrameView &f, const GridView &grids)
 {
-    const ImageParts p = image_layout(lds, s.num_spheres, s.num_dir, s.num_point, cull.padded, f.spp);
-    fill_image(p, s, cull, f, grids);
-    return image_view(p);
+    fill_image(image_layout(lds, image_dims(s, cull, f.spp, grids)), s, cull, f, grids);
+    return image_view(lds, f);
 }
 
 struct Hit
@@ -208,7 +219,7 @@
 TRT_DEV bool exact_step(const LdsImage &L, d3 o, d3 d, double a, int i, bool valid, Hit &best, int inside = -1)
 {
     static_assert(!(ANY_HIT && REFRACT), "shadow rays are the reference's");
-    const double2 c01 = ((const double2 *)L.sph)[2 * i], c23 = ((const double2 *)L.sph)[2 * i + 1];
+    const double2 c01 = ((const double2 *)L.sph())[2 * i], c23 = ((const double2 *)L.sph())[2 * i + 1];
     const d3 c = d3{c01.x, c01.y, c23.x};
     const d3 oc = sub(o, c);
     const double b = 2.0 * dot(oc, d);
@@ -296,7 +307,7 @@
                 }
                 else
                 {
-                    const float4 e = L.cull[i];
+                    const float4 e = L.cull()[i];
                     sign = trt_filter_sign(&flt, e.x, e.y, e.z, e.w);
                 }
                 if (valid && (!flt.ok || !(sign >> 31)))
@@ -357,7 +368,7 @@
                         }
                         else
                         {
-                            const float4 e = L.cull[first + g + j];
+                            const float4 e = L.cull()[first + g + j];
                             bits = __builtin_amdgcn_alignbit(bits, trt_filter_sign(&flt, e.x, e.y, e.z, e.w), 31);
                         }
                     }
@@ -446,7 +457,7 @@
         const int i = valid ? (int)((unsigned)cur & entry_mask) : 0;
         cur >>= list_bits;
         k++;
-        const double2 c01 = ((const double2 *)L.sph)[2 * i], c23 = ((const double2 *)L.sph)[2 * i + 1];
+        const double2 c01 = ((const double2 *)L.sph())[2 * i], c23 = ((const double2 *)L.sph())[2 * i + 1];
         const d3 oc = sub(o, d3{c01.x, c01.y, c23.x});
         const double b = 2.0 * dot(oc, d);
         const double cc = dot(oc, oc) - c23.y;
@@ -488,10 +499,10 @@
     const int f = has ? fam : 0;
     const int s = f >= 2 ? f - 2 : 0, i = s >= n ? s - n : s;
     const bool of_eye = f < 2, mirrored = s >= n;
-    const double *rec = L.fam + 4 * i;
-    d3 apex = mirrored ? load3(rec) : load3(L.sph + 4 * i);
+    const double *rec = L.fam() + 4 * i;
+    d3 apex = mirrored ? load3(rec) : load3(L.sph() + 4 * i);
     double r_chk = mirrored ? rec[3] + TRT_FAMILY_SLACK : rec[3];
-    const double *E = BATCH ? L.eye + frame * (2 * TRT_RAYFAMILY_DOUBLES) + TRT_RAYFAMILY_DOUBLES * (f & 1) : L.eye + TRT_RAYFAMILY_DOUBLES * (f & 1);
+    const double *E = (BATCH ? L.frame(frame) + kLdsCameraDoubles : L.eye()) + TRT_RAYFAMILY_DOUBLES * (f & 1);
     const double rg2_eye = E[5];
     if (of_eye)
     {
@@ -527,15 +538,15 @@
     const bool of_eye = f < 2, mirrored = f >= 2 + n;
     const int code = f - 2 - n;
     const int i = mirrored ? code >> TRT_PATCH_SHIFT : (of_eye ? 0 : f - 2);
-    const double *at_sphere = L.sph + 4 * i, *at_mirror = L.fam + 4 * i;
-    const double *src = of_eye ? L.eye + (BATCH ? frame * (2 * TRT_RAYFAMILY_DOUBLES) : 0) + TRT_RAYFAMILY_DOUBLES * (f & 1) : (mirrored ? at_mirror : at_sphere);
+    const double *at_sphere = L.sph() + 4 * i, *at_mirror = L.fam() + 4 * i;
+    const double *src = of_eye ? (BATCH ? L.frame(frame) + kLdsCameraDoubles : L.eye()) + TRT_RAYFAMILY_DOUBLES * (f & 1) : (mirrored ? at_mirror : at_sphere);
     const d3 base_at = load3(src);
     const int here = trt_cubemap_cell((float)(o.x - base_at.x), (float)(o.y - base_at.y), (float)(o.z - base_at.z), 0.5f * (float)G.patch_m,
                                       (float)(G.patch_m - 1), G.patch_m);
     const int k = mirrored ? code & ((1 << TRT_PATCH_SHIFT) - 1) : (of_eye ? 0 : here);
     fam = !has ? -1 : (f == 0 ? 1 : (!of_eye && !mirrored ? 2 + n + (((f - 2) << TRT_PATCH_SHIFT) | k) : -1));
     const double r_abs = of_eye ? 0.0 : at_mirror[3];
-    const double *pr = L.patch + TRT_PATCH_RECORD * k + (mirrored ? 4 : 0);
+    const double *pr = L.patch() + TRT_PATCH_RECORD * k + (mirrored ? 4 : 0);
     const d3 apex = d3{TRT_PATCH_APEX(base_at.x, r_abs, pr[0]), TRT_PATCH_APEX(base_at.y, r_abs, pr[1]), TRT_PATCH_APEX(base_at.z, r_abs, pr[2])};
     const double rho = pr[3];
     double rchk_eye = src[3], rg2_eye = src[5];
@@ -620,7 +631,7 @@
         r.mat = n + checker_odd(r.ph.p);
         if (r.ph.i >= 0 && r.ph.i < n)
         {
-            raw = sub(r.ph.p, load3(L.sph + 4 * r.ph.i));
+            raw = sub(r.ph.p, load3(L.sph() + 4 * r.ph.i));
             r.mat = r.ph.i;
         }
         r.normal = unit(raw);
@@ -646,13 +657,13 @@
         if (li < nd)
         {
             TRT_MARK_AT(24);
-            sd = load3(L.dir + li * kDirRecord);
-            lcolor = load3(L.dir + li * kDirRecord + 3);
+            sd = load3(L.dir() + li * kDirRecord);
+            lcolor = load3(L.dir() + li * kDirRecord + 3);
             bool use_list = false;
             unsigned long long cell = 0;
             if (grids.enabled)
             {
-                const trt_dirgrid *G = L.dirgrid + li;
+                const trt_dirgrid *G = L.dirgrid() + li;
                 int far;
                 const int c = trt_dirgrid_cell(G, o.x, o.y, o.z, &far);
                 if (lit_lanes && !far)
@@ -662,8 +673,8 @@
             if (COUNT && !use_list)
                 tally.swept++;
             TRT_MARK_AT(8);
-            const Hit sh = trace<true, false, 9>(L, cull, n, o, sd, lit_lanes, lit_word, gp, gn, tally.iters[1], tally.tests[1], L.cull_dir + li * cull.padded, use_list, cell, grids.pool, grids.list_bits,
-                                                 -1, L.dir + li * kDirRecord + 6);
+            const Hit sh = trace<true, false, 9>(L, cull, n, o, sd, lit_lanes, lit_word, gp, gn, tally.iters[1], tally.tests[1], L.cull_dir() + li * cull.padded, use_list, cell, grids.pool, grids.list_bits,
+                                                 -1, L.dir() + li * kDirRecord + 6);
             is_lit = sh.i < 0;
             factor = min1(dot(normal, sd));
             TRT_MARK_AT(13);
@@ -671,7 +682,7 @@
         else
         {
             TRT_MARK_AT(25);
-            const double *pl = L.pt + (li - nd) * 7;
+            const double *pl = L.pt() + (li - nd) * 7;
             const d3 to_light = sub(load3(pl), o);
             const double light_d2 = dot(to_light, to_light);
             const double strength = clampd(pl[6] / light_d2, 0.0, 1.0);
@@ -681,7 +692,7 @@
             unsigned long long cell = 0;
             if (grids.enabled)
             {
-                const trt_pointgrid *G = L.pointgrid + (li - nd);
+                const trt_pointgrid *G = L.pointgrid() + (li - nd);
                 int far;
                 const int c = trt_pointgrid_cell(G, o.x, o.y, o.z, &far);
                 far |= !(__builtin_fabs(dot(sd, sd) - 1.0) <= 9.094947017729282e-13);
@@ -696,7 +707,7 @@
             is_lit = true;
             if (use_list)
             {
-                const trt_pointgrid *G = L.pointgrid + (li - nd);
+                const trt_pointgrid *G = L.pointgrid() + (li - nd);
                 double lo, hi;
                 trt_point_shadow_bounds(G, light_d2, dot(sd, sd), &lo, &hi);
                 bool dark, unsure;
@@ -726,7 +737,7 @@
             TRT_MARK_AT(19);
         }
         if (lit_lanes && is_lit)
-            lit = add(lit, mulc(scale(lcolor, factor), load3(L.mat + mat * 5)));
+            lit = add(lit, mulc(scale(lcolor, factor), load3(L.mat() + mat * 5)));
     }
     return lit;
 }
@@ -794,7 +805,7 @@
 {
     v.jitter = in_device_memory(v.jitter), v.col_x = in_device_memory(v.col_x), v.row_y = in_device_memory(v.row_y);
     v.samples = in_device_memory(v.samples), v.out = in_device_memory(v.out), v.ior = in_device_memory(v.ior);
-    v.counters = in_device_memory(v.counters), v.queue = in_device_memory(v.queue);
+    v.counters = in_device_memory(v.counters), v.queue = in_device_memory(v.queue), v.image = in_device_memory(v.image);
     return v;
 }
 TRT_DEV GridView in_device_memory(GridView v)
@@ -818,6 +829,8 @@
     const d3 gp = load3(s.ground), gn = load3(s.ground + 3);                                       \
     (void)n, (void)nd, (void)nl, (void)total, (void)pixels_here, (void)gp, (void)gn, (void)cull, (void)grids
 
+#define TRT_FRESH_IMAGE const LdsImage L = image_view(DEVICE_IMAGE ? f.image : lds, f)
+
 struct alignas(8) BatchShape
 {
     unsigned frames, units_per_frame, frame_magic, reserved;
@@ -832,21 +845,22 @@
 TRT_DEV LdsImage stage_lds_image_batch(double *lds, const SceneView &s, const CullView &cull, const FrameView &f, const GridView &grids)
 {
     const int frames = (int)load_batch_shape().frames;
-    const ImageParts p = image_layout(lds, s.num_spheres, s.num_dir, s.num_point, cull.padded, f.spp, frames);
-    fill_image(p, s, cull, f, grids);
+    const trt_image_dims dims = image_dims(s, cull, f.spp, grids);
+    fill_image(image_layout(lds, dims), s, cull, f, grids);
+    double *const extra = lds + f.at.frames;
     const double CONSTANT_AS *cams = (const double CONSTANT_AS *)((const char CONSTANT_AS *)__builtin_amdgcn_kernarg_segment_ptr() + kArgBatch);
     const double CONSTANT_AS *eyes = cams + sizeof(BatchView::cam) / sizeof(double);
-    for (int i = threadIdx.x; i < frames * kLdsCameraDoubles; i += blockDim.x)
-    {
-        const int b = i / kLdsCameraDoubles, j = i - b * kLdsCameraDoubles;
+    for (int i = threadIdx.x; i < (frames - 1) * TRT_IMAGE_FRAME_DOUBLES; i += blockDim.x)
+    {
+        const int b = 1 + i / TRT_IMAGE_FRAME_DOUBLES, j = i - (b - 1) * TRT_IMAGE_FRAME_DOUBLES;
         const double CONSTANT_AS *c = cams + b * 15;
-        p.cam[i] = j < 12 ? c[j] : (j == 12 ? -c[12] : c[6 + (j - 13)] * -c[12]);
-    }
-    if (grids.path_enabled)
-        for (int i = threadIdx.x; i < frames * 2 * TRT_RAYFAMILY_DOUBLES; i += blockDim.x)
-            p.eye[i] = eyes[i];
+        if (j < kLdsCameraDoubles)
+            extra[i] = j < 12 ? c[j] : (j == 12 ? -c[12] : c[6 + (j - 13)] * -c[12]);
+        else if (grids.path_enabled)
+            extra[i] = eyes[b * (2 * TRT_RAYFAMILY_DOUBLES) + (j - kLdsCameraDoubles)];
+    }
     __syncthreads();
-    return image_view(p);
+    return image_view(lds, f);
 }
 
 #ifndef TRT_COMPACT_BLOCK
@@ -857,7 +871,7 @@
 
 template <bool COUNT, bool REFRACT = false, bool COMPACT = false, bool PATCHES = false, bool BIG = false, bool DEVICE_IMAGE = false, bool BATCH = false,
           class... BatchArgument>
-__global__ __launch_bounds__(BIG ? kBigBlock : COMPACT ? kCompactBlock : kPersistentBlock, ((COMPACT && !COUNT) || BIG) ? 4 : TRT_ROUNDS_WAVES) void render_rounds_kernel(SceneView s, CullView cull, FrameView f, GridView grids, BatchArgument... batch)
+__global__ __launch_bounds__(BIG ? kBigBlock : COMPACT ? kCompactBlock : kPersistentBlock, COUNT ? TRT_ROUNDS_WAVES : 4) void render_rounds_kernel(SceneView s, CullView cull, FrameView f, GridView grids, BatchArgument... batch)
 {
     static_assert(sizeof...(BatchArgument) == (BATCH ? 1 : 0), "a BATCH launch has one more argument, a BatchView; the others none");
     static_assert(!BATCH || (!COUNT && !REFRACT && !BIG && !DEVICE_IMAGE), "several frames per launch: the plain, patch and decoupled rounds");
@@ -866,9 +880,7 @@
     static_assert(!BIG || (PATCHES && !COUNT && !REFRACT && !COMPACT), "1024-thread workgroups: the shipping patch instantiation only");
     static_assert(!DEVICE_IMAGE || (!REFRACT && !COMPACT && !BIG), "the device-memory image: the plain rounds only");
     extern __shared__ __attribute__((aligned(16))) double lds[];
-    const LdsImage L = BATCH ? stage_lds_image_batch(lds, s, cull, f, grids)
-                       : DEVICE_IMAGE ? image_view(image_layout(const_cast<double *>(f.image), s.num_spheres, s.num_dir, s.num_point, cull.padded, f.spp))
-                                      : stage_lds_image(lds, s, cull, f, grids);
+    const LdsImage L = BATCH ? stage_lds_image_batch(lds, s, cull, f, grids) : DEVICE_IMAGE ? image_view(f.image, f) : stage_lds_image(lds, s, cull, f, grids);
     const int n = s.num_spheres, nd = s.num_dir, nl = s.num_dir + s.num_point;
     const int lane = threadIdx.x & 63;
     const unsigned pixels_here = (unsigned)f.local_rows * (unsigned)f.width;
@@ -912,6 +924,7 @@
         TRT_MARK_AT(22);
         {
             TRT_FRESH_ARGS;
+            TRT_FRESH_IMAGE;
             const unsigned long long need = __ballot(want_unit);
             if (need)
             {
@@ -952,7 +965,7 @@
                             frame += (unsigned)(over - under);
                             mine = (unsigned)(within + (under - over) * (int)total);
                         }
-                        const double *const cam = L.cam + (BATCH ? frame * (unsigned)kLdsCameraDoubles : 0u);
+                        const double *const cam = BATCH ? L.frame((int)frame) : L.cam();
                         unsigned pixel = __umulhi(mine, f.spp_magic);
                         int k = (int)(mine - pixel * (unsigned)f.spp);
                         {
@@ -968,8 +981,9 @@
                             row += (unsigned)(over - under);
                             col += (under - over) * f.width;
                         }
-                        const double sx = f.col_x[col] + L.jit[k];
-                        const double sy = f.row_y[f.tile_first == 0 && f.tile_step == 1 ? (int)row : frame_row_of_magic(f, row)] + L.jit[f.spp + k];
+                        const double2 jitter = ((const double2 *)L.jit())[k];
+                        const double sx = f.col_x[col] + jitter.x;
+                        const double sy = f.row_y[f.tile_first == 0 && f.tile_step == 1 ? (int)row : frame_row_of_magic(f, row)] + jitter.y;
                         d3 dir = d3{0.0, 0.0, 0.0};
                         dir = add(dir, scale(load3(cam + 0), sx));
                         dir = add(dir, scale(load3(cam + 3), sy));
@@ -1001,6 +1015,7 @@
         PathHit hit;
         {
             TRT_FRESH_ARGS;
+            TRT_FRESH_IMAGE;
             hit = path_stage<COUNT, REFRACT, PATCHES, BATCH>(L, cull, grids, n, o, d, fam, alive, alive_lanes, gp, gn, tally, inside, BATCH ? bounces >> kBatchFrameShift : 0);
         }
         if constexpr (COMPACT)
@@ -1011,6 +1026,7 @@
             const double weight_before = weight;
             {
             TRT_FRESH_ARGS;
+            TRT_FRESH_IMAGE;
             if (hit.sky_lanes != 0)
                 sky_t = sky_texel_wave(s.sky, s.sky_dim, hit.back, s.sky_dim_f, path_sky, hit.sky_lanes);
             const unsigned long long hits = hit.hit_lanes;
@@ -1028,7 +1044,7 @@
                     ring_mat[at] = (unsigned short)hit.mat;
                     const d3 nd3 = reflect(d, hit.normal);
                     parked[lane] = nd3.x, parked[64 + lane] = nd3.y, parked[128 + lane] = nd3.z;
-                    weight *= L.mat[hit.mat * 5 + 3];
+                    weight *= L.mat()[hit.mat * 5 + 3];
                     bounces++;
                     end_sample = !((BATCH ? bounces & kBatchBounceMask : bounces) < f.bounce_limit && weight > 0.00001);
                 }
@@ -1042,6 +1058,7 @@
             if (q_head != q_tail && ((int)(q_old - q_head) > 0 || q_tail - q_head >= 64u))
             {
                 TRT_FRESH_ARGS;
+                TRT_FRESH_IMAGE;
                 const unsigned take = q_tail - q_head < 64u ? q_tail - q_head : 64u;
                 const bool has = (unsigned)lane < take;
                 const unsigned at = (q_head + (unsigned)lane) & (kRingTasks - 1);
@@ -1085,7 +1102,7 @@
             old_slot = my_task & (kRingTasks - 1), old_open = my_open, my_open = false;
             if (path_sky)
             {
-                const d3 color = d3{L.b255[sky_t & 0xFF], L.b255[(sky_t >> 8) & 0xFF], L.b255[(sky_t >> 16) & 0xFF]};
+                const d3 color = d3{L.b255()[sky_t & 0xFF], L.b255()[(sky_t >> 8) & 0xFF], L.b255()[(sky_t >> 16) & 0xFF]};
                 sample = add(sample, scale(color, weight));
             }
             if (__any(finish))
@@ -1134,6 +1151,7 @@
                 tally.passes++;
             {
                 TRT_FRESH_ARGS;
+                TRT_FRESH_IMAGE;
                 lit = shadow_stage<COUNT>(L, cull, grids, n, nd, nl, o, h_normal, h_mat, path_hit, hit.hit_lanes, gp, gn, tally);
             }
         }
@@ -1180,9 +1198,10 @@
         if (path_hit)
         {
             TRT_FRESH_ARGS;
+            TRT_FRESH_IMAGE;
             d3 color = d3{clampd(lit.x, 0.0, 1.0), clampd(lit.y, 0.0, 1.0), clampd(lit.z, 0.0, 1.0)};
             color = scale(color, weight);
-            weight *= L.mat[h_mat * 5 + 3];
+            weight *= L.mat()[h_mat * 5 + 3];
             bounces++;
             sample = add(sample, color);
             if ((BATCH ? bounces & kBatchBounceMask : bounces) < f.bounce_limit && weight > 0.00001)
@@ -1199,7 +1218,7 @@
         }
         if (path_sky)
         {
-            const d3 color = d3{L.b255[sky_t & 0xFF], L.b255[(sky_t >> 8) & 0xFF], L.b255[(sky_t >> 16) & 0xFF]};
+            const d3 color = d3{L.b255()[sky_t & 0xFF], L.b255()[(sky_t >> 8) & 0xFF], L.b255()[(sky_t >> 16) & 0xFF]};
             sample = add(sample, scale(color, weight));
         }
         if (__any(end_sample))
@@ -1280,15 +1299,15 @@
     d3 nrm = hit.back;
     if (hit.hit)
     {
-        color = load3(L.mat + hit.mat * 5);
-        refl = L.mat[hit.mat * 5 + 3];
-        spec = L.mat[hit.mat * 5 + 4];
+        color = load3(L.mat() + hit.mat * 5);
+        refl = L.mat()[hit.mat * 5 + 3];
+        spec = L.mat()[hit.mat * 5 + 4];
         nrm = hit.normal;
     }
     else
     {
         const uint32_t t = sky_t;
-        color = d3{L.b255[t & 0xFF], L.b255[(t >> 8) & 0xFF], L.b255[(t >> 16) & 0xFF]};
+        color = d3{L.b255()[t & 0xFF], L.b255()[(t >> 8) & 0xFF], L.b255()[(t >> 16) & 0xFF]};
     }
     obj[i] = hit.hit ? (hit.ph.i < n ? 1 : 2) : 0;
     point[3 * i + 0] = surface.x, point[3 * i + 1] = surface.y, point[3 * i + 2] = surface.z;
```
